# 0x002A/MuCHSALSA

Hardware: AMD Instinct MI355X
Metric: overlap-pairs/s (higher is better)
Workload: dtype int32+f64; 1 GPU; 100k synthetic Nanopore x10 kb, 500k unitig anchors, 10x coverage (BASELINE.json configs[2]); rows=5059558, reads=100000, anchors=499992, edges=981460, edgematches_rank0=25532466, orders_rank0=1029308, parallelism=one job on one GPU, edges_proven_clean_rank0=5372

## Files before the change

### muchsalsa_amd/csrc/msgpu_api.hip

```cpp
#include <hip/hip_runtime.h>

#include <chrono>
#include <cmath>
#include <cstdarg>
#include <cstdio>
#include <cstdlib>
#include <cstring>
#include <condition_variable>
#include <deque>
#include <mutex>
#include <new>
#include <thread>
#include <vector>
#include <algorithm>
#include <sys/mman.h>
#include <unistd.h>

#include "asm_internal.h"
#include "host_pool.h"
#include "msgpu.h"
#include "msgpu_internal.h"

using namespace msgpu;

// ... 74 lines not shown
    if (header_of(p)->registered || !have_device()) return p;
    block_unmap(p);
  }
  void *q = nullptr;
  if (hipHostMalloc(&q, PB_HEADER + (bytes ? bytes : 1), hipHostMallocDefault) != hipSuccess || !q) {
    (void)hipGetLastError();
    return nullptr;
  }
  *static_cast<BlockHeader *>(q) = BlockHeader{PB_MAGIC, q, 0, 0, 0, 1};
  return static_cast<char *>(q) + PB_HEADER;
}
void pinned_block_free(void *p) noexcept {
  if (p) block_unmap(p);
}

void *host_table_alloc(size_t bytes) {
  void *p = block_map(bytes ? bytes : 1);
  if (!p) throw std::bad_alloc();
  return p;
}
void host_table_free(void *q) noexcept {
  if (q) block_unmap(q);
}
void host_table_pin(void *q) noexcept {
  if (q) block_register(q);
}
}


namespace {

struct DevBuf {
  void  *p   = nullptr;
  size_t cap = 0;
  size_t off  = 0;
  size_t hint = 0;
  static inline thread_local double grow_by = 1.0;
  double own_grow_by = 0.0;
  hipError_t ensure(size_t bytes) {
    if (off + bytes <= cap) return hipSuccess;
    const size_t need = off + bytes;
    size_t       want = need + need / 8 + 256;
    const double by = own_grow_by > grow_by ? own_grow_by : grow_by;
    if (by > 1.0) want = off + static_cast<size_t>(double(want - off) * by);
    if (hint > want) want = hint;
    static const bool dbg_alloc = std::getenv("MSGPU_ALLOC_DEBUG") != nullptr;
    if (dbg_alloc) fprintf(stderr, "[alloc] %zu -> %zu bytes (need %zu, kept %zu, hint %zu, grow_by %.2f)\n", cap, want, need, off, hint, grow_by);
    void      *np = nullptr;
    hipError_t e;
    if (p && !off) {
      e   = hipFree(p);
      p   = nullptr;
      cap = 0;
      if (e != hipSuccess) return e;
    }
    e = hipMalloc(&np, want);
    if (e != hipSuccess) return e;
    static const bool poison = std::getenv("MSGPU_POISON") != nullptr;
    if (poison) {
      e = hipMemset(np, 0xA5, want);
      if (e == hipSuccess) e = hipDeviceSynchronize();
      if (e != hipSuccess) {
        (void)hipFree(np);
        return e;
      }
    }
    if (p) {
      e = hipDeviceSynchronize();
      if (e == hipSuccess) e = hipMemcpy(np, p, off, hipMemcpyDeviceToDevice);
      if (e == hipSuccess) e = hipDeviceSynchronize();
      if (e != hipSuccess) {
        (void)hipFree(np);
        return e;
      }
      (void)hipFree(p);
    }
    p   = np;
    cap = want;
    return hipSuccess;
  }
  void release() {
    if (p) (void)hipFree(p);
    p   = nullptr;
    cap = 0;
    off = hint = 0;
  }
  template <class T> T *as() const { return reinterpret_cast<T *>(static_cast<char *>(p) + off); }
  void  *at() const { return static_cast<char *>(p) + off; }
  size_t room() const { return cap > off ? cap - off : 0; }
};

enum State { ST_CREATED = 0, ST_LOADED = 1, ST_EDGES = 2, ST_CHAINED = 3,
             ST_RESULT = 4  };

}

struct msgpu_ctx {
  int          device     = 0;
  hipStream_t  stream     = nullptr;
  hipStream_t  own_stream = nullptr;
  msgpu_params p;
  char         err[512]   = {0};
  State        state      = ST_CREATED;
  uint32_t     shard = 0, nshards = 1;
  uint32_t     win_lo = 0, win_hi = 0xffffffffu;
  uint64_t     base_edges = 0, base_ems = 0, base_orders = 0, base_ids = 0;
  uint64_t    *h_scalars = nullptr;
  uint64_t    *h_scalars_dev = nullptr;
  bool         stage_events = true;
  bool         chain_zeroed = false;
  bool         no_prologue = false;
  bool         prologue_ok = false;
  bool         scalars_clean = false;
  bool         bin_clean = false;
  size_t       bin_zero_words = 0;
  uint32_t     prologue_shard = 0, prologue_nshards = 1;
  uint64_t     prologue_own = 0;
  bool         full_scan_ok = false;
  uint64_t     index_total = 0, own_accum = 0;
  bool         nlists_clean = false;
  bool         cand_zeroed = false;
  uint64_t     prologue_bound = 0;
  uint32_t     prologue_lists[4] = {0, 0, 0, 0};
  uint64_t     readback_seq = 0;
  uint64_t     lost_publications = 0;
  bool         readback_mapped = false;
  hipEvent_t   ev_readback = nullptr;
  hipEvent_t   ev_order = nullptr;
  uint32_t     decl_V = 0, decl_A = 0;
  bool                                  has_deadline = false;
  std::chrono::steady_clock::time_point deadline{};

  uint64_t n_rows = 0, n_alive = 0;
  uint32_t V = 0, A = 0;
  const msgpu_row *d_rows = nullptr;

  uint64_t n_edges = 0, n_ems = 0, n_orders = 0, n_ids = 0, n_visit = 0, total_bound = 0;
  uint32_t n_list[4] = {0, 0, 0, 0};

  DevBuf rows_in, rows_pk, cnt_read, read_off, cursor, bkt_key, bkt_dead, by_read, read_cnt, alive_rank,
      anchor_cnt, anchor_off, anchor_first, anchor_off_gen, bkt2_idx, bkt2_line, by_anchor, read_len, read_first, scalars,
      scan_tmp, vis16, spos2, visits, bin_cursor, bin_start;
  DevBuf bound, cand_off, cand_j, cand_t, scr_v2, scr_start, n_cand, n_edge, lists, edges, edge_cand;
  DevBuf big_key, big_t, big_r2s, big_pfx, pair_tab, chain_chunks, big_off, cand_sums, bucket_visits;
  hipStream_t side_stream = nullptr, side_stream2 = nullptr;
  hipEvent_t  ev_side[2]  = {nullptr, nullptr}, ev_side2 = nullptr;
  uint64_t    n_big_edges = 0, n_big_ems = 0;
  bool   fast_path = true;
  bool   chain_band = true;
  bool   sub_wave  = true;
  bool   use_fork  = true;
  bool   use_prologue = true;
  bool   chain_serial = false;
  uint32_t n_cls[4] = {0, 0, 0, 0};
  uint64_t n_edges_fast = 0;
  uint64_t chain_E = 0;
  DevBuf ems, order_scr, ids_scr, edge_norders, edge_nids, orders, ids, big_list, cls_list, big_elems,
      big_paths;
  DevBuf g_deg, g_off, g_adj, g_cand, g_sane, g_out;
  DevBuf sel_idx, sel_cnt, sel_off, sel_ems;

  DevBuf      alt_edges, alt_ems, alt_orders, alt_ids;
  hipStream_t copy_stream = nullptr;
  hipEvent_t  ev_done[2] = {nullptr, nullptr}, ev_copied[2] = {nullptr, nullptr}, ev_wall[2] = {nullptr, nullptr};
  struct HostBuf {
    void  *p   = nullptr;
    size_t cap = 0;
  } h_edges, h_ems, h_orders, h_ids, h_read_len, h_read_first, h_sel_off, h_sel_ems, h_wire[2];
  hipEvent_t ev_part[2][3] = {{nullptr, nullptr, nullptr}, {nullptr, nullptr, nullptr}};
  std::mutex              gate_m;
  std::condition_variable gate_cv;
  uint64_t                chain_launches = 0;
  DevBuf win_cuts;
  DevBuf wire_dev[2];
  bool   wire_copy = true;

  hipEvent_t ev[10] = {nullptr};
  static constexpr int CK_RING = 256;
  hipEvent_t ck_ev[CK_RING][2] = {};
  uint32_t   ck_head = 0, ck_count = 0;
  bool       have_index_t = false, have_cand_t = false, have_chain_t = false, index_fast = false;
  bool   have_stage_t = false;
  uint32_t index_path = 0;
  bool     index_binned = false;
  bool     use_bin = true;
};

namespace {

int fail(msgpu_ctx *c, int code, const char *fmt, ...) {
  va_list ap;
  va_start(ap, fmt);
  vsnprintf(c->err, sizeof(c->err), fmt, ap);
  va_end(ap);
  return code;
}

#define HIPCHK(c, expr)                                                                                                \
  do {                                                                                                                 \
    hipError_t _e = (expr);                                                                                            \
    if (_e != hipSuccess)                                                                                              \
      return fail((c), _e == hipErrorOutOfMemory ? MSGPU_E_NOMEM : MSGPU_E_HIP, "%s failed: %s (%s:%d)", #expr,        \
                  hipGetErrorString(_e), __FILE__, __LINE__);                                                          \
  } while (0)

#define ENSURE(c, buf, bytes) HIPCHK(c, (c)->buf.ensure(bytes))

template <class T> T *scalar(msgpu_ctx *c, int slot) { return reinterpret_cast<T *>(c->scalars.as<uint64_t>() + slot); }
template <class T> const T *host_scalar(const msgpu_ctx *c, int slot) { return reinterpret_cast<const T *>(c->h_scalars + slot); }
static uint32_t cand_chunks(uint32_t V) { return (V + CAND_CHUNK - 1) / CAND_CHUNK; }
static size_t   cand_sums_bytes(uint32_t V) { return static_cast<size_t>(cand_chunks(V) + 1) * (16 + 256); }
static unsigned long long *cand_chunk_sums(msgpu_ctx *c) { return c->cand_sums.as<unsigned long long>(); }
static uint32_t *cand_hist(msgpu_ctx *c, uint32_t V) { return reinterpret_cast<uint32_t *>(c->cand_sums.as<unsigned long long>() + 2 * static_cast<size_t>(cand_chunks(V) + 1)); }
static CandZero cand_zero(msgpu_ctx *c, uint32_t V) {
  static_assert(SC_BIGCUR == SC_BIGSTATS + 2 && SC_CLS == SC_BIGCUR + 2 && SC_HEADS == SC_CLS + 2, "adjacent scalar slots");
  CandZero z;
  z.n_cand         = c->n_cand.as<uint32_t>();
  z.n_edge         = c->n_edge.as<uint32_t>();
  z.scalar_words   = scalar<uint32_t>(c, SC_BIGSTATS);
  z.n_scalar_words = 12;
  return z;
}

bool past_deadline(const msgpu_ctx *c) { return c->has_deadline && std::chrono::steady_clock::now() >= c->deadline; }
int host_sync(msgpu_ctx *c, hipStream_t st, hipEvent_t ev = nullptr) {
  if (!c->has_deadline) {
    if (ev) HIPCHK(c, hipEventSynchronize(ev));
    else HIPCHK(c, hipStreamSynchronize(st));
    return MSGPU_OK;
  }
  for (uint32_t spins = 0;; ++spins) {
    const hipError_t q = ev ? hipEventQuery(ev) : hipStreamQuery(st);
    if (q == hipSuccess) return MSGPU_OK;
    if (q != hipErrorNotReady) return fail(c, MSGPU_E_HIP, "%s failed: %s", ev ? "hipEventQuery" : "hipStreamQuery", hipGetErrorString(q));
    if (past_deadline(c))
      return fail(c, MSGPU_E_TIMEOUT, "the context's stream did not drain before the deadline (msgpu_set_deadline): work is still queued");
    if (spins < 2000) __builtin_ia32_pause();
    else std::this_thread::sleep_for(std::chrono::microseconds(50));
  }
}

HostPublish arm_readback(msgpu_ctx *c) {
  return c->readback_mapped ? HostPublish{c->h_scalars_dev, ++c->readback_seq} : HostPublish{nullptr, 0};
}
int wait_scalars(msgpu_ctx *c) {
  if (c->readback_mapped) {
    const uint64_t     seq  = c->readback_seq;
    volatile uint64_t *flag = c->h_scalars + SC_COUNT;
    for (uint64_t spins = 1;; ++spins) {
      if (__atomic_load_n(flag, __ATOMIC_ACQUIRE) == seq) return MSGPU_OK;
      __builtin_ia32_pause();
      if ((spins & 0xffff) == 0) {
        const hipError_t q = hipStreamQuery(c->stream);
        if (q == hipSuccess) {
          if (__atomic_load_n(flag, __ATOMIC_ACQUIRE) == seq) return MSGPU_OK;
          break;
        }
        if (q != hipErrorNotReady) break;
        if (past_deadline(c))
          return fail(c, MSGPU_E_TIMEOUT, "table sizes did not come back before the deadline (msgpu_set_deadline): the stream is "
                                          "held up by work queued in front of ours");
      }
    }
    ++c->lost_publications;
    HIPCHK(c, hipMemcpyAsync(c->h_scalars, c->scalars.p, SC_COUNT * sizeof(uint64_t), hipMemcpyDeviceToHost, c->stream));
    return host_sync(c, c->stream);
  }
  return host_sync(c, nullptr, c->ev_readback);
}
int close_readback(msgpu_ctx *c) {
  if (!c->readback_mapped) {
    HIPCHK(c, hipMemcpyAsync(c->h_scalars, c->scalars.p, SC_COUNT * sizeof(uint64_t), hipMemcpyDeviceToHost, c->stream));
    HIPCHK(c, hipEventRecord(c->ev_readback, c->stream));
  }
  return wait_scalars(c);
}
int read_scalars(msgpu_ctx *c, hipEvent_t mark = nullptr) {
  const HostPublish p = arm_readback(c);
  if (p.seq) launch_publish_scalars(c->stream, c->scalars.as<uint64_t>(), p);
  if (mark) HIPCHK(c, hipEventRecord(mark, c->stream));
  return close_readback(c);
}

void release_all(msgpu_ctx *c) {
  DevBuf *all[] = {&c->sel_idx, &c->sel_cnt, &c->sel_off, &c->sel_ems, &c->g_deg, &c->g_off, &c->g_adj, &c->g_cand, &c->g_sane, &c->g_out, &c->rows_in, &c->rows_pk, &c->cnt_read, &c->read_off, &c->cursor, &c->bkt_key,
                   &c->bkt_dead, &c->by_read, &c->read_cnt, &c->alive_rank, &c->anchor_cnt, &c->anchor_off,
                   &c->anchor_first, &c->anchor_off_gen,
                   &c->bkt2_idx, &c->bkt2_line, &c->by_anchor, &c->read_len, &c->read_first, &c->scalars, &c->scan_tmp,
                   &c->bound, &c->cand_off, &c->cand_j, &c->cand_t, &c->scr_v2, &c->scr_start, &c->n_cand, &c->n_edge,
                   &c->lists, &c->edges, &c->edge_cand,
                   &c->big_key, &c->big_t, &c->big_r2s, &c->big_pfx, &c->pair_tab, &c->chain_chunks, &c->big_off, &c->cand_sums, &c->bucket_visits, &c->ems, &c->order_scr, &c->ids_scr,
                   &c->edge_norders, &c->edge_nids, &c->orders, &c->ids, &c->big_list, &c->cls_list, &c->big_elems, &c->big_paths, &c->alt_edges, &c->alt_ems, &c->alt_orders, &c->alt_ids, &c->vis16, &c->visits,
                   &c->spos2, &c->bin_cursor, &c->bin_start, &c->wire_dev[0], &c->wire_dev[1], &c->win_cuts};
  for (DevBuf *b : all) b->release();
}

int build_index_once(msgpu_ctx *c, bool force_generic, bool two_pass, bool bin, uint32_t *ix_flags_out) {
  hipStream_t st = c->stream;
  const uint64_t n = c->n_rows;
  {
    const void *before = c->scalars.p;
    ENSURE(c, scalars, SC_COUNT * sizeof(uint64_t));
    if (c->scalars.p != before) c->scalars_clean = false;
  }
  bool scalars_zeroed = false;
  auto zero_scalars = [&]() -> int {
    if (scalars_zeroed) return MSGPU_OK;
    HIPCHK(c, hipMemsetAsync(c->scalars.p, 0, SC_COUNT * sizeof(uint64_t), st));
    scalars_zeroed  = true;
    c->nlists_clean = true;
    return MSGPU_OK;
  };

  if (c->decl_V && c->decl_A) {
    c->V = c->decl_V;
    c->A = c->decl_A;
  } else {
    if (int rc = zero_scalars()) return rc;
    launch_max_ids(st, c->d_rows, n, scalar<uint32_t>(c, SC_MAXIDS));
    if (int rc = read_scalars(c)) return rc;
    c->V = host_scalar<uint32_t>(c, SC_MAXIDS)[0];
    c->A = host_scalar<uint32_t>(c, SC_MAXIDS)[1];
  }
  const uint32_t V = c->V, A = c->A;

  const size_t nz = n ? n : 1;
  const size_t mva = size_t(V > A ? V : A) + 2;
  constexpr uint32_t BUCKET_CAP = 128;
  const uint32_t reads_per_pass = BIN_NB_MAX << BIN_RPB_SHIFT;
  const uint32_t bpasses = (bin && !force_generic && !two_pass && n && V) ? static_cast<uint32_t>((size_t(V) + reads_per_pass - 1) / reads_per_pass) : 0;
  uint32_t       bcap    = (bpasses && bpasses <= BIN_PASSES_MAX) ? bin_capacity(n, V) : 0;
  if (bcap && !index_sort_bin_prepare(bcap)) bcap = 0;
  const uint32_t bshift  = bcap ? BIN_RPB_SHIFT : 0;
  const uint32_t nb      = bshift ? static_cast<uint32_t>((size_t(std::min(V, reads_per_pass)) + (1u << bshift) - 1) >> bshift) : 0;
  const uint32_t     cap = (!bshift && !two_pass && V && size_t(V) * BUCKET_CAP * sizeof(IRow) <= (size_t(4) << 30)) ? BUCKET_CAP : 0;
  ENSURE(c, cnt_read, (size_t(V) + 1) * 4);
  ENSURE(c, read_off, (size_t(V) + 2) * 4);
  ENSURE(c, cursor, mva * 4);
  if (bshift) {
    const void *before = c->bin_cursor.p;
    ENSURE(c, bin_cursor, (size_t(bpasses) * (nb + 1) + 1) * 4);
    if (c->bin_cursor.p != before) {
      c->bin_clean      = false;
      c->bin_zero_words = 0;
    }
    if (size_t(bpasses) * (nb + 1) + 1 > c->bin_zero_words) c->bin_clean = false;
    ENSURE(c, bin_start, (size_t(nb) + 2) * 4);
    ENSURE(c, bucket_visits, ((size_t(V) >> BIN_RPB_SHIFT) + 2) * 4);
  }
  const bool fused_readback = bshift != 0 && c->readback_mapped;
  if (!(fused_readback && c->scalars_clean))
    if (int rc = zero_scalars()) return rc;
  c->scalars_clean = false;
  ENSURE(c, bkt_key, (bshift ? size_t(nb) * bcap * 2 : cap ? size_t(V) * cap : nz) * sizeof(IRow));
  ENSURE(c, bkt_dead, nz);
  ENSURE(c, by_read, nz * sizeof(IRow));
  ENSURE(c, read_cnt, (size_t(V) + 1) * 4);
  ENSURE(c, alive_rank, nz * 4);
  ENSURE(c, anchor_cnt, (size_t(A) + 1) * 4);
  ENSURE(c, anchor_first, (size_t(A) + 2) * 4);
  ENSURE(c, anchor_off_gen, (size_t(A) + 2) * 4);
  ENSURE(c, anchor_off, (size_t(A) + 2) * 4);
  ENSURE(c, bkt2_idx, nz * 4);
  ENSURE(c, bkt2_line, nz * 4);
  ENSURE(c, by_anchor, nz * sizeof(IRow));
  ENSURE(c, vis16, nz * 16);
  ENSURE(c, spos2, (bshift ? 1 : cap ? size_t(V) * cap : nz) * 8);
  ENSURE(c, visits, (size_t(V) + 1) * 4);
  ENSURE(c, read_len, (size_t(V) + 1) * 4);
  ENSURE(c, read_first, (size_t(V) + 1) * 4);
  {
    uint64_t m = n;
    if (V > m) m = V;
    if (A > m) m = A;
    ENSURE(c, scan_tmp, 3 * (size_t(scan_blocks(m)) + 1) * 8);
  }

  c->prologue_ok           = false;
  const bool want_prologue = c->use_prologue && !force_generic && !c->no_prologue && V != 0 && (c->nshards == 1 || bshift) && c->win_lo == 0 && c->win_hi >= V;
  if (want_prologue) {
    ENSURE(c, n_cand, (size_t(V) + 1) * 4);
    ENSURE(c, n_edge, (size_t(V) + 1) * 4);
    ENSURE(c, cand_sums, cand_sums_bytes(V));
  }
  size_t zero_words_known = 0;
  {
    uint32_t *const zero[8]   = {bshift ? c->bin_cursor.as<uint32_t>() : c->cnt_read.as<uint32_t>(), c->cursor.as<uint32_t>(),
                                 c->read_cnt.as<uint32_t>(), c->anchor_cnt.as<uint32_t>(), nullptr, nullptr, nullptr, nullptr};
    const uint32_t  n_zero[8] = {bshift ? bpasses * (nb + 1) + 1 : V + 1, static_cast<uint32_t>(mva), V + 1, A + 1, 0, 0, 0, 0};
    uint32_t *const ones[2]   = {c->anchor_first.as<uint32_t>(), nullptr};
    const uint32_t  n_ones[2] = {A + 2, 0};
    if (!bshift) launch_index_init8(st, zero, n_zero, ones, n_ones);
    else if (!c->bin_clean) {
      c->bin_zero_words     = std::max<size_t>(c->bin_zero_words, n_zero[0]);
      uint32_t *const z4[4] = {zero[0], nullptr, nullptr, nullptr};
      const uint32_t  n4[4] = {n_zero[0], 0, 0, 0};
      uint32_t *const o2[2] = {nullptr, nullptr};
      const uint32_t  no2[2] = {0, 0};
      launch_index_init(st, z4, n4, o2, no2);
    }
    c->bin_clean = false;
    if (bshift) {
      zero_words_known  = c->bin_zero_words;
      c->bin_zero_words = 0;
    }
  }
  uint32_t *d_flags = scalar<uint32_t>(c, SC_IXFLAGS);
  if (force_generic) {
    const uint32_t f = IXF_FORCE;
    HIPCHK(c, hipMemcpyAsync(d_flags, &f, 4, hipMemcpyHostToDevice, st));
  }

  if (bshift) {
    uint32_t *row_base = c->bin_cursor.as<uint32_t>() + size_t(bpasses) * (nb + 1);
    for (uint32_t p = 0; p < bpasses; ++p) {
      const uint32_t rd_lo = p * reads_per_pass;
      const uint32_t nb_p  = static_cast<uint32_t>((size_t(std::min(V - rd_lo, reads_per_pass)) + (1u << bshift) - 1) >> bshift);
      uint32_t      *cur   = c->bin_cursor.as<uint32_t>() + size_t(p) * (nb + 1);
      BinTail        tail;
      tail.bin_start    = c->bin_start.as<uint32_t>();
      tail.row_base     = row_base;
      tail.read_off_end = p + 1 == bpasses ? c->read_off.as<uint32_t>() + V : nullptr;
      tail.done_heads   = scalar<unsigned long long>(c, SC_HEADS);
      launch_index_bin(st, c->d_rows, n, V, A, d_flags, scalar<uint32_t>(c, SC_ERR), c->anchor_first.as<uint32_t>(), cur,
                       c->bkt_key.as<uint4>(), rd_lo, nb_p, bcap, tail);
      launch_index_sort_bin(st, cur, c->bin_start.as<uint32_t>(), V, rd_lo, nb_p, bcap, c->bkt_key.as<uint4>(),
                            c->by_read.as<IRow>(), c->by_anchor.as<IRow>(), c->vis16.as<uint4>(), c->read_off.as<uint32_t>(),
                            c->read_cnt.as<uint32_t>(), c->read_len.as<int32_t>(), c->read_first.as<uint32_t>(),
                            c->visits.as<uint32_t>(), c->d_rows, d_flags, scalar<uint32_t>(c, SC_ERR), c->bucket_visits.as<uint32_t>());
    }
  } else {
  launch_index_pass1(st, c->d_rows, n, c->cnt_read.as<uint32_t>(), c->anchor_first.as<uint32_t>(), V, A, d_flags,
                     scalar<uint32_t>(c, SC_ERR), c->bkt_key.as<IRow>(), cap, c->spos2.as<uint2>());
  exclusive_scan<uint32_t>(st, c->cnt_read.as<uint32_t>(), V, c->read_off.as<uint32_t>(), c->scan_tmp.as<uint32_t>(),
                           scalar<uint32_t>(c, SC_TOTAL_A));
  if (!cap) launch_scatter_read(st, c->d_rows, n, c->read_off.as<uint32_t>(), c->cursor.as<uint32_t>(), c->bkt_key.as<IRow>());
  launch_sort_read(st, c->read_off.as<uint32_t>(), c->cnt_read.as<uint32_t>(), V, c->bkt_key.as<IRow>(),
                   c->by_read.as<IRow>(), c->read_cnt.as<uint32_t>(),
                   c->alive_rank.as<uint32_t>(), c->anchor_cnt.as<uint32_t>(), c->bkt_dead.as<uint8_t>(), d_flags,
                   c->by_anchor.as<IRow>(), cap, c->d_rows, c->read_len.as<int32_t>(), c->read_first.as<uint32_t>(),
                   scalar<uint32_t>(c, SC_ERR), c->spos2.as<uint2>(), c->vis16.as<uint4>(), c->visits.as<uint32_t>());
  }
  if (bshift) {
    ENSURE(c, cand_off, (size_t(V) + 2) * 8);
    ENSURE(c, lists, (size_t(V) + 1) * (3 * sizeof(CandDesc) + 4));
// ... 69 lines not shown
  c->own_accum    = fused_readback ? 0 : *host_scalar<uint64_t>(c, SC_OWN);
  if (fused_readback && ixf == 0 && err == 0) {
    c->scalars_clean = c->bin_clean = true;
    c->bin_zero_words = zero_words_known;
  }
  if (want_prologue && ixf == 0 && err == 0) {
    c->prologue_ok      = true;
    c->cand_zeroed      = true;
    c->prologue_bound   = *host_scalar<uint64_t>(c, SC_TOTAL_A);
    c->prologue_shard   = bshift ? c->shard : 0;
    c->prologue_nshards = bshift ? c->nshards : 1;
    c->prologue_own     = (bshift && c->nshards > 1) ? *host_scalar<uint64_t>(c, SC_OWN) : c->prologue_bound;
    for (int k = 0; k < 4; ++k) c->prologue_lists[k] = host_scalar<uint32_t>(c, SC_NLISTS)[k];
  }
  uint32_t       n_alive = *host_scalar<uint32_t>(c, SC_NALIVE);
  if (err & 2u)
    return fail(c, MSGPU_E_IDS, "a row has an id outside the declared id space (%u reads, %u anchors)", V, A);
  c->index_binned = bshift != 0;
  if (bshift && ixf != 0) {
    c->prologue_ok = c->cand_zeroed = false;
    *ix_flags_out  = ixf | IXF_BINFAIL;
    return MSGPU_OK;
  }
  if (ixf & IXF_OVERFLOW) {
    *ix_flags_out = ixf;
    return MSGPU_OK;
  }
  if ((ixf & ~IXF_DUPS) != 0 && !(err & 1u)) {
    exclusive_scan<uint32_t>(st, c->anchor_cnt.as<uint32_t>(), A, c->anchor_off_gen.as<uint32_t>(),
                             c->scan_tmp.as<uint32_t>(), scalar<uint32_t>(c, SC_NALIVE));
    launch_select_anchor_off(st, d_flags, c->anchor_first.as<uint32_t>(), c->anchor_off_gen.as<uint32_t>(), A,
                             c->anchor_off.as<uint32_t>(), scalar<uint32_t>(c, SC_NALIVE), static_cast<uint32_t>(n));
    HIPCHK(c, hipMemsetAsync(c->cursor.p, 0, mva * 4, st));
    launch_scatter_anchor(st, c->d_rows, n, c->alive_rank.as<uint32_t>(), c->anchor_off.as<uint32_t>(),
                          c->cursor.as<uint32_t>(), c->bkt2_idx.as<uint32_t>(), c->bkt2_line.as<uint32_t>(), d_flags);
    launch_rank_anchor(st, c->anchor_off.as<uint32_t>(), n, scalar<uint32_t>(c, SC_NALIVE), c->bkt2_idx.as<uint32_t>(),
                       c->bkt2_line.as<uint32_t>(), c->d_rows, c->alive_rank.as<uint32_t>(), c->by_anchor.as<IRow>(),
                       d_flags, c->read_off.as<uint32_t>(), c->by_read.as<IRow>(), c->vis16.as<uint4>());
    HIPCHK(c, hipGetLastError());
    if (int rc = read_scalars(c, c->ev[1])) return rc;
    n_alive = *host_scalar<uint32_t>(c, SC_NALIVE);
  }
  c->n_alive    = n_alive;
  *ix_flags_out = ixf;
  if (err & 1u)
    return fail(c, MSGPU_E_IDS,
                "read ids are not dense Registry ids in first-line order (Registry.cpp:36-45): use msgpu_parse_paf ids");
  return MSGPU_OK;
}

int build_index(msgpu_ctx *c) {
  if (c->stage_events) HIPCHK(c, hipEventRecord(c->ev[0], c->stream));
  uint32_t ixf = 0;
  bool     two_pass = false;
  int      rc  = build_index_once(c, false, two_pass, c->use_bin, &ixf);
  if (rc != MSGPU_OK) return rc;
  const bool binned = c->use_bin && !(ixf & IXF_BINFAIL) && c->index_binned;
  if (ixf & IXF_BINFAIL) {
    ixf = 0;
    rc  = build_index_once(c, false, two_pass, false, &ixf);
    if (rc != MSGPU_OK) return rc;
  }
  if (ixf & IXF_OVERFLOW) {
    two_pass = true;
    rc       = build_index_once(c, false, two_pass, false, &ixf);
    if (rc != MSGPU_OK) return rc;
  }
  if ((ixf & IXF_DUPS) && (ixf & ~IXF_DUPS) == 0) {
    rc = build_index_once(c, true, two_pass, false, &ixf);
    if (rc != MSGPU_OK) return rc;
  }
  c->index_fast   = (ixf & ~IXF_DUPS) == 0;
  c->index_path   = (binned ? MSGPU_INDEX_BIN : two_pass ? MSGPU_INDEX_TWO_PASS : MSGPU_INDEX_ATOMIC) | (c->index_fast ? 0u : MSGPU_INDEX_GENERIC);
  c->have_index_t = c->stage_events;
  c->state        = ST_LOADED;
  return MSGPU_OK;
}

}

extern "C" {

void msgpu_default_params(msgpu_params *p) {
  if (!p) return;
  p->min_matches = 400;
  p->th_length   = 500;
  p->th_matches  = 500;
  p->th_overlap  = 100;
  p->wiggle_room = 300;
  p->ratio_pct   = 15;
  p->alt_frac    = 0.75;
}

const char *msgpu_strerror(int code) {
  switch (code) {
  case MSGPU_OK: return "ok";
  case MSGPU_E_IO: return "can't open blast file";
  case MSGPU_E_FORMAT: return "invalid BLAST file";
  case MSGPU_E_NUMBER: return "invalid integer field in BLAST file";
  case MSGPU_E_NOMEM: return "out of memory";
  case MSGPU_E_ARG: return "invalid argument (unexpected nullptr)";
  case MSGPU_E_HIP: return "HIP runtime error";
  case MSGPU_E_STATE: return "entry points called out of order";
  case MSGPU_E_IDS: return "read ids are not in Registry (first-line) order";
  case MSGPU_E_NODEVICE: return "no HIP device (libmsgpu has no CPU fallback)";
  case MSGPU_E_LAYOUT: return "path cannot be assembled (the reference would terminate or hang on it)";
  case MSGPU_E_TIMEOUT: return "a deadline passed while device work was still queued";
  default: return "unknown error";
  }
}

int msgpu_create(int device, const msgpu_params *params, msgpu_ctx **out) {
  if (!out) return MSGPU_E_ARG;
  *out = nullptr;
  int        ndev = 0;
  hipError_t e    = hipGetDeviceCount(&ndev);
  if (e != hipSuccess || ndev <= 0) return MSGPU_E_NODEVICE;
  if (device < 0 || device >= ndev) return MSGPU_E_ARG;
  msgpu_ctx *c = new (std::nothrow) msgpu_ctx();
  if (!c) return MSGPU_E_NOMEM;
  c->device = device;
  if (params)
    c->p = *params;
  else
    msgpu_default_params(&c->p);
  if (hipSetDevice(device) != hipSuccess || hipStreamCreateWithFlags(&c->own_stream, hipStreamNonBlocking) != hipSuccess) {
    delete c;
    return MSGPU_E_HIP;
  }
  c->stream = c->own_stream;
  if (hipHostMalloc(reinterpret_cast<void **>(&c->h_scalars), (SC_COUNT + 1) * sizeof(uint64_t),
                    hipHostMallocMapped | hipHostMallocCoherent) != hipSuccess) {
    c->h_scalars = nullptr;
    msgpu_destroy(c);
    return MSGPU_E_NOMEM;
  }
  memset(c->h_scalars, 0, (SC_COUNT + 1) * sizeof(uint64_t));
  if (hipHostGetDevicePointer(reinterpret_cast<void **>(&c->h_scalars_dev), c->h_scalars, 0) != hipSuccess) c->h_scalars_dev = nullptr;
  c->readback_mapped = c->h_scalars_dev && !getenv("MSGPU_SYNC_READBACK");
  {
    const char *nf = getenv("MSGPU_NO_FASTPATH");
    c->fast_path   = !(nf && nf[0] == '1');
    const char *nb = getenv("MSGPU_NO_BAND");
    c->chain_band  = c->fast_path && !(nb && nb[0] == '1');
    const char *ns = getenv("MSGPU_NO_SUBWAVE");
    c->sub_wave    = !(ns && ns[0] == '1');
    const char *nw = getenv("MSGPU_NO_WIRE_COPY");
    c->wire_copy   = !(nw && nw[0] == '1');
    const char *nbin = getenv("MSGPU_NO_BIN");
    c->use_bin       = !(nbin && nbin[0] == '1');
    c->use_prologue = !getenv("MSGPU_NO_PROLOGUE");
    c->use_fork     = !getenv("MSGPU_NO_FORK");
    c->chain_serial = getenv("MSGPU_CHAIN_SERIAL") != nullptr;
  }
  for (auto &ev : c->ev)
    if (hipEventCreate(&ev) != hipSuccess) {
      msgpu_destroy(c);
      return MSGPU_E_HIP;
    }
  int prio_least = 0, prio_greatest = 0;
  if (hipDeviceGetStreamPriorityRange(&prio_least, &prio_greatest) != hipSuccess) prio_least = prio_greatest = 0;
  if (hipStreamCreateWithPriority(&c->side_stream, hipStreamNonBlocking, prio_greatest) != hipSuccess ||
      hipStreamCreateWithPriority(&c->side_stream2, hipStreamNonBlocking, prio_greatest) != hipSuccess ||
      hipEventCreateWithFlags(&c->ev_side2, hipEventDisableTiming) != hipSuccess ||
      hipEventCreateWithFlags(&c->ev_part[0][0], hipEventDisableTiming) != hipSuccess ||
      hipEventCreateWithFlags(&c->ev_part[0][1], hipEventDisableTiming) != hipSuccess ||
      hipEventCreateWithFlags(&c->ev_part[0][2], hipEventDisableTiming) != hipSuccess ||
      hipEventCreateWithFlags(&c->ev_part[1][0], hipEventDisableTiming) != hipSuccess ||
      hipEventCreateWithFlags(&c->ev_part[1][1], hipEventDisableTiming) != hipSuccess ||
      hipEventCreateWithFlags(&c->ev_part[1][2], hipEventDisableTiming) != hipSuccess ||
      hipEventCreateWithFlags(&c->ev_side[0], hipEventDisableTiming) != hipSuccess ||
      hipEventCreateWithFlags(&c->ev_side[1], hipEventDisableTiming) != hipSuccess ||
      hipEventCreateWithFlags(&c->ev_readback, hipEventDisableTiming) != hipSuccess ||
      hipEventCreateWithFlags(&c->ev_order, hipEventDisableTiming) != hipSuccess) {
    msgpu_destroy(c);
    return MSGPU_E_HIP;
  }
  if (hipStreamCreateWithFlags(&c->copy_stream, hipStreamNonBlocking) != hipSuccess) {
    msgpu_destroy(c);
    return MSGPU_E_HIP;
  }
  for (int k = 0; k < 2; ++k)
    if (hipEventCreateWithFlags(&c->ev_done[k], hipEventDisableTiming) != hipSuccess ||
        hipEventCreateWithFlags(&c->ev_copied[k], hipEventDisableTiming) != hipSuccess) {
      msgpu_destroy(c);
      return MSGPU_E_HIP;
    }
  *out = c;
  return MSGPU_OK;
}

void msgpu_destroy(msgpu_ctx *c) {
  if (!c) return;
  (void)hipSetDevice(c->device);
  if (c->stream) (void)hipStreamSynchronize(c->stream);
  release_all(c);
  for (auto &ev : c->ev)
    if (ev) (void)hipEventDestroy(ev);
  for (auto &ev : c->ev_side)
    if (ev) (void)hipEventDestroy(ev);
  if (c->ev_readback) (void)hipEventDestroy(c->ev_readback);
  if (c->ev_order) (void)hipEventDestroy(c->ev_order);
  if (c->ev_side2) (void)hipEventDestroy(c->ev_side2);
  for (auto &per_set : c->ev_part)
    for (hipEvent_t e : per_set)
      if (e) (void)hipEventDestroy(e);
  if (c->side_stream2) {
    (void)hipStreamSynchronize(c->side_stream2);
    (void)hipStreamDestroy(c->side_stream2);
  }
  for (auto &pair : c->ck_ev)
    for (auto &ev : pair)
      if (ev) (void)hipEventDestroy(ev);
  if (c->side_stream) {
    (void)hipStreamSynchronize(c->side_stream);
    (void)hipStreamDestroy(c->side_stream);
  }
  if (c->copy_stream) {
    (void)hipStreamSynchronize(c->copy_stream);
    (void)hipStreamDestroy(c->copy_stream);
  }
  for (int k = 0; k < 2; ++k) {
    if (c->ev_done[k]) (void)hipEventDestroy(c->ev_done[k]);
    if (c->ev_copied[k]) (void)hipEventDestroy(c->ev_copied[k]);
  }
  for (msgpu_ctx::HostBuf *h : {&c->h_edges, &c->h_ems, &c->h_orders, &c->h_ids, &c->h_read_len, &c->h_read_first, &c->h_sel_off,
                               &c->h_sel_ems, &c->h_wire[0], &c->h_wire[1]})
    if (h->p) pinned_block_free(h->p);
  if (c->own_stream) (void)hipStreamDestroy(c->own_stream);
  if (c->h_scalars) (void)hipHostFree(c->h_scalars);
  delete c;
}

const char *msgpu_last_error(const msgpu_ctx *c) { return c ? c->err : "null context"; }

int msgpu_set_stream(msgpu_ctx *c, void *hip_stream) {
  if (!c) return MSGPU_E_ARG;
  HIPCHK(c, hipStreamSynchronize(c->stream));
  c->stream = hip_stream ? static_cast<hipStream_t>(hip_stream) : c->own_stream;
  return MSGPU_OK;
}

void *msgpu_get_stream(const msgpu_ctx *c) { return c ? static_cast<void *>(c->stream) : nullptr; }

int msgpu_stream_wait(msgpu_ctx *c, void *hip_stream) {
  if (!c) return MSGPU_E_ARG;
  hipStream_t other = static_cast<hipStream_t>(hip_stream);
  if (other == c->stream) return MSGPU_OK;
  HIPCHK(c, hipSetDevice(c->device));
  HIPCHK(c, hipEventRecord(c->ev_order, other));
  HIPCHK(c, hipStreamWaitEvent(c->stream, c->ev_order, 0));
  return MSGPU_OK;
}
int msgpu_stream_release(msgpu_ctx *c, void *hip_stream) {
  if (!c) return MSGPU_E_ARG;
  hipStream_t other = static_cast<hipStream_t>(hip_stream);
  if (other == c->stream) return MSGPU_OK;
  HIPCHK(c, hipSetDevice(c->device));
  HIPCHK(c, hipEventRecord(c->ev_order, c->stream));
  HIPCHK(c, hipStreamWaitEvent(other, c->ev_order, 0));
  return MSGPU_OK;
}

int msgpu_set_shard(msgpu_ctx *c, uint32_t shard, uint32_t n_shards) {
  if (!c) return MSGPU_E_ARG;
  if (n_shards == 0 || shard >= n_shards) return fail(c, MSGPU_E_ARG, "shard %u of %u is out of range", shard, n_shards);
  c->shard   = shard;
  c->nshards = n_shards;
  if (c->state > ST_LOADED) c->state = ST_LOADED;
  return MSGPU_OK;
}

int msgpu_set_id_space(msgpu_ctx *c, uint32_t n_reads, uint32_t n_anchors) {
  if (!c) return MSGPU_E_ARG;
  if ((n_reads == 0) != (n_anchors == 0)) return fail(c, MSGPU_E_ARG, "declare both id counts, or 0 and 0 to find them");
  c->decl_V = n_reads;
  c->decl_A = n_anchors;
  return MSGPU_OK;
}

int msgpu_load_rows(msgpu_ctx *c, const msgpu_row *rows, size_t n_rows) {
  if (!c) return MSGPU_E_ARG;
  if (n_rows && !rows) return fail(c, MSGPU_E_ARG, "Unexpected nullptr.");
  if (n_rows > (1ull << 30)) return fail(c, MSGPU_E_ARG, "row table too large (%zu rows, at most 2^30)", n_rows);
  HIPCHK(c, hipSetDevice(c->device));
  c->state = ST_CREATED;
  ENSURE(c, rows_in, (n_rows ? n_rows : 1) * sizeof(msgpu_row));
  if (n_rows)
    HIPCHK(c, hipMemcpyAsync(c->rows_in.p, rows, n_rows * sizeof(msgpu_row), hipMemcpyHostToDevice, c->stream));
  c->d_rows = c->rows_in.as<msgpu_row>();
  c->n_rows = n_rows;
  return build_index(c);
}

int msgpu_load_rows_packed(msgpu_ctx *c, const msgpu_packed_rows *p) {
  if (!c) return MSGPU_E_ARG;
  if (!p || (p->n_rows && (!p->rows || !p->run_start || !p->run_delta || !p->n_runs)) || (p->n_reads && !p->read_len))
    return fail(c, MSGPU_E_ARG, "Unexpected nullptr.");
  if (p->n_rows > (1ull << 30)) return fail(c, MSGPU_E_ARG, "row table too large (%llu rows, at most 2^30)", (unsigned long long)p->n_rows);
  HIPCHK(c, hipSetDevice(c->device));
  c->state = ST_CREATED;
  const size_t n = static_cast<size_t>(p->n_rows);
  const size_t off_len = (n * sizeof(msgpu_row28) + 255) / 256 * 256, off_rs = off_len + (size_t(p->n_reads) * 4 + 255) / 256 * 256,
               off_rd = off_rs + (size_t(p->n_runs) * 4 + 255) / 256 * 256, total = off_rd + size_t(p->n_runs) * 4 + 256;
  ENSURE(c, rows_pk, total);
  ENSURE(c, rows_in, (n ? n : 1) * sizeof(msgpu_row));
// ... 3 lines not shown
    if (p->n_reads) HIPCHK(c, hipMemcpyAsync(d + off_len, p->read_len, size_t(p->n_reads) * 4, hipMemcpyHostToDevice, c->stream));
    HIPCHK(c, hipMemcpyAsync(d + off_rs, p->run_start, size_t(p->n_runs) * 4, hipMemcpyHostToDevice, c->stream));
    HIPCHK(c, hipMemcpyAsync(d + off_rd, p->run_delta, size_t(p->n_runs) * 4, hipMemcpyHostToDevice, c->stream));
    launch_expand_rows(c->stream, d, n, reinterpret_cast<const int32_t *>(d + off_len), p->n_reads, reinterpret_cast<const uint32_t *>(d + off_rs),
                       reinterpret_cast<const uint32_t *>(d + off_rd), p->n_runs, c->rows_in.as<msgpu_row>(),
                       reinterpret_cast<uint32_t *>(d + off_rd + size_t(p->n_runs) * 4));
    HIPCHK(c, hipGetLastError());
  }
  c->d_rows = c->rows_in.as<msgpu_row>();
  c->n_rows = n;
  return build_index(c);
}

int msgpu_load_rows_device(msgpu_ctx *c, const void *d_rows, size_t n_rows) {
  if (!c) return MSGPU_E_ARG;
  if (n_rows && !d_rows) return fail(c, MSGPU_E_ARG, "Unexpected nullptr.");
  if (n_rows > (1ull << 30)) return fail(c, MSGPU_E_ARG, "row table too large (%zu rows, at most 2^30)", n_rows);
  HIPCHK(c, hipSetDevice(c->device));
  c->state  = ST_CREATED;
  c->d_rows = static_cast<const msgpu_row *>(d_rows);
  c->n_rows = n_rows;
  return build_index(c);
}

static size_t chunk_words(uint64_t n_edges) { return 2 * static_cast<size_t>(n_edges / COMPACT_CHUNK + 2); }

int msgpu_calculate_edges(msgpu_ctx *c) {
  if (!c) return MSGPU_E_ARG;
  if (c->state < ST_LOADED) return fail(c, MSGPU_E_STATE, "msgpu_calculate_edges before msgpu_load_rows");
  HIPCHK(c, hipSetDevice(c->device));
  hipStream_t    st = c->stream;
  const uint32_t V  = c->V;
  c->state          = ST_LOADED;
  if (c->stage_events) HIPCHK(c, hipEventRecord(c->ev[2], st));

  ENSURE(c, bound, (size_t(V) + 1) * 4);
  ENSURE(c, cand_off, (size_t(V) + 2) * 8);
  ENSURE(c, lists, (size_t(V) + 1) * (3 * sizeof(CandDesc) + 4));
  ENSURE(c, n_cand, (size_t(V) + 1) * 4);
  ENSURE(c, n_edge, (size_t(V) + 1) * 4);
  ENSURE(c, cand_sums, cand_sums_bytes(V));
  CandDesc *l0 = c->lists.as<CandDesc>(), *l1 = l0 + V + 1, *l2 = l1 + V + 1;
  uint32_t *l3 = reinterpret_cast<uint32_t *>(l2 + V + 1);

  const bool all_reads = c->index_fast && c->nshards == 1 && c->win_lo == 0 && c->win_hi >= V;
  const bool use_prologue = c->index_fast && c->win_lo == 0 && c->win_hi >= V && c->prologue_ok && c->prologue_shard == c->shard &&
                            c->prologue_nshards == c->nshards;
  const bool zeroed    = use_prologue && c->cand_zeroed;
  c->cand_zeroed       = false;
  const uint32_t *bound     = all_reads ? c->visits.as<uint32_t>() : c->bound.as<uint32_t>();
  uint64_t total_bound, own_bound;
  if (use_prologue) {
    total_bound = c->prologue_bound;
    own_bound   = c->prologue_own;
    for (int k = 0; k < 4; ++k) c->n_list[k] = c->prologue_lists[k];
    if (!zeroed) {
      const CandZero  z         = cand_zero(c, V);
      uint32_t *const zero[4]   = {z.n_cand, z.n_edge, z.scalar_words, nullptr};
      const uint32_t  n_zero[4] = {V + 1, V + 1, z.n_scalar_words, 0};
      uint32_t *const ones[2]   = {nullptr, nullptr};
      const uint32_t  n_ones[2] = {0, 0};
      launch_index_init(st, zero, n_zero, ones, n_ones);
    }
  } else if (c->full_scan_ok && c->index_fast && c->nshards == 1) {
    if (!c->nlists_clean) HIPCHK(c, hipMemsetAsync(scalar<uint32_t>(c, SC_NLISTS), 0, 16, st));
    c->nlists_clean = false;
    launch_classify_reads(st, c->read_off.as<uint32_t>(), c->read_cnt.as<uint32_t>(), c->visits.as<uint32_t>(),
                          c->cand_off.as<uint64_t>(), V, 0, 1, c->win_lo, c->win_hi, l0, l1, l2, l3,
                          scalar<uint32_t>(c, SC_NLISTS), cand_zero(c, V), scalar<unsigned long long>(c, SC_OWN));
    HIPCHK(c, hipGetLastError());
    if (int rc = read_scalars(c)) return rc;
    total_bound  = c->index_total;
    const uint64_t own_now = *host_scalar<uint64_t>(c, SC_OWN);
    own_bound    = own_now - c->own_accum;
    c->own_accum = own_now;
    for (int k = 0; k < 4; ++k) c->n_list[k] = host_scalar<uint32_t>(c, SC_NLISTS)[k];
  } else {
    if (!c->nlists_clean) HIPCHK(c, hipMemsetAsync(scalar<uint32_t>(c, SC_NLISTS), 0, 16, st));
    c->full_scan_ok = false;
    if (!all_reads)
      launch_bound(st, c->read_off.as<uint32_t>(), c->read_cnt.as<uint32_t>(), c->vis16.as<uint4>(), V, c->shard,
                   c->nshards, c->win_lo, c->win_hi, c->bound.as<uint32_t>());
    exclusive_scan<uint64_t>(st, bound, V, c->cand_off.as<uint64_t>(), c->scan_tmp.as<uint64_t>(),
                             scalar<uint64_t>(c, SC_TOTAL_A));
    c->nlists_clean = false;
    launch_classify_reads(st, c->read_off.as<uint32_t>(), c->read_cnt.as<uint32_t>(), bound,
                          c->cand_off.as<uint64_t>(), V, c->shard, c->nshards, c->win_lo, c->win_hi, l0, l1, l2, l3,
                          scalar<uint32_t>(c, SC_NLISTS), cand_zero(c, V));
    HIPCHK(c, hipGetLastError());
    if (int rc = read_scalars(c)) return rc;
    total_bound = own_bound = *host_scalar<uint64_t>(c, SC_TOTAL_A);
    for (int k = 0; k < 4; ++k) c->n_list[k] = host_scalar<uint32_t>(c, SC_NLISTS)[k];
  }
  c->total_bound = own_bound;

  const size_t tb = total_bound ? total_bound : 1;
  ENSURE(c, cand_j, tb * 4);
  ENSURE(c, cand_t, tb * 4);
  ENSURE(c, scr_v2, tb * 4);
  ENSURE(c, scr_start, tb * 4);

  CandArgs a;
  a.read_off       = c->read_off.as<uint32_t>();
  a.read_cnt       = c->read_cnt.as<uint32_t>();
  a.anchor_off     = c->anchor_off.as<uint32_t>();
  a.by_read        = c->by_read.as<IRow>();
  a.by_anchor      = c->by_anchor.as<IRow>();
  a.vis            = c->vis16.as<uint4>();
  a.cand_off       = c->cand_off.as<uint64_t>();
  a.cand_j         = c->cand_j.as<uint32_t>();
  a.cand_t         = c->cand_t.as<uint32_t>();
  a.edge_scr_v2    = c->scr_v2.as<uint32_t>();
  a.edge_scr_start = c->scr_start.as<uint32_t>();
  a.n_cand         = c->n_cand.as<uint32_t>();
  a.n_edge         = c->n_edge.as<uint32_t>();
  a.th_overlap     = c->p.th_overlap;
  a.big_stats      = scalar<unsigned long long>(c, SC_BIGSTATS);
  const bool fork = (c->n_list[1] || c->n_list[2]) && c->n_list[0] && c->use_fork;
  if (fork) {
    HIPCHK(c, hipEventRecord(c->ev_side[0], st));
    if (c->n_list[2]) {
      HIPCHK(c, hipStreamWaitEvent(c->side_stream, c->ev_side[0], 0));
      launch_candidates(c->side_stream, a, 2, l2, c->n_list[2]);
    }
    launch_candidates(st, a, 0, l0, c->n_list[0]);
    if (c->n_list[1]) {
      HIPCHK(c, hipStreamWaitEvent(c->side_stream2, c->ev_side[0], 0));
      launch_candidates(c->side_stream2, a, 1, l1, c->n_list[1]);
      HIPCHK(c, hipEventRecord(c->ev_side2, c->side_stream2));
      HIPCHK(c, hipStreamWaitEvent(st, c->ev_side2, 0));
    }
    if (c->n_list[2]) {
      HIPCHK(c, hipEventRecord(c->ev_side[1], c->side_stream));
      HIPCHK(c, hipStreamWaitEvent(st, c->ev_side[1], 0));
    }
  } else {
    launch_candidates(st, a, 2, l2, c->n_list[2]);
    launch_candidates(st, a, 1, l1, c->n_list[1]);
    launch_candidates(st, a, 0, l0, c->n_list[0]);
  }
  if (c->n_list[3]) {
    ENSURE(c, big_key, tb * 8);
    ENSURE(c, big_t, tb * 4);
    ENSURE(c, big_r2s, tb * 4);
    ENSURE(c, big_pfx, (c->n_rows ? c->n_rows : 1) * 4);
    launch_candidates_big(st, a, l3, c->n_list[3], c->big_key.as<uint64_t>(), c->big_t.as<uint32_t>(),
                          c->big_r2s.as<uint32_t>(), c->big_pfx.as<uint32_t>());
  }
  HIPCHK(c, hipGetLastError());
  auto capacities = [&](uint64_t *cap_edges, uint64_t *cap_big) {
    uint64_t ce = c->edges.room() / sizeof(msgpu_edge);
    if (c->edge_cand.cap / 8 < ce) ce = c->edge_cand.cap / 8;
    if (c->cls_list.cap / 4 < ce) ce = c->cls_list.cap / 4;
    uint64_t cb = c->big_list.cap / 4;
    if (c->big_off.cap / 8 < cb) cb = c->big_off.cap / 8;
    if (c->chain_chunks.cap / 8 < chunk_words(ce)) ce = 0;
    *cap_edges = ce;
    *cap_big   = cb;
  };
  auto emit = [&](uint64_t cap_edges, uint64_t cap_big, bool publish) {
    EmitArgs k;
    k.n_edge         = c->n_edge.as<uint32_t>();
    k.n_cand         = c->n_cand.as<uint32_t>();
    k.cand_off       = c->cand_off.as<uint64_t>();
    k.edge_scr_v2    = c->scr_v2.as<uint32_t>();
    k.edge_scr_start = c->scr_start.as<uint32_t>();
    k.V              = V;
    k.hist           = cand_hist(c, V);
    k.chunk_sums     = cand_chunk_sums(c);
    k.n_chunks       = cand_chunks(V);
    k.edges          = c->edges.as<msgpu_edge>();
    k.edge_cand      = c->edge_cand.as<uint64_t>();
    k.list           = c->cls_list.as<uint32_t>();
    k.big_list       = c->big_list.as<uint32_t>();
    k.big_off        = c->big_off.as<uint64_t>();
    k.big_cursor     = scalar<unsigned long long>(c, SC_BIGCUR);
    k.big_stats      = scalar<unsigned long long>(c, SC_BIGSTATS);
    k.cap_edges      = cap_edges;
    k.cap_big        = cap_big;
    k.chain_chunk_sums    = c->chain_chunks.as<unsigned long long>();
    k.n_chain_chunk_words = cap_edges ? static_cast<uint32_t>(chunk_words(cap_edges)) : 0u;
    k.scalars        = c->scalars.as<uint64_t>();
    k.pub            = publish ? arm_readback(c) : HostPublish{nullptr, 0};
    k.nlists         = scalar<unsigned long long>(c, SC_NLISTS);
    launch_emit_edges(st, k, publish);
  };
  uint64_t cap_edges = 0, cap_big = 0;
  capacities(&cap_edges, &cap_big);
  emit(cap_edges, cap_big, true);
  c->nlists_clean = true;
  HIPCHK(c, hipGetLastError());
  if (int rc = close_readback(c)) return rc;
  const uint64_t *tot = host_scalar<uint64_t>(c, SC_TOTAL_A), *big = host_scalar<uint64_t>(c, SC_BIGSTATS);
  c->n_big_edges = big[0];
  c->n_big_ems   = big[1];
  for (int k = 0; k < 4; ++k) c->n_cls[k] = host_scalar<uint32_t>(c, SC_CLS)[k];
  c->n_ems   = tot[0];
  c->n_edges = tot[1];
  c->n_visit = c->total_bound;
  if (c->n_edges >= 0xfffffff0ull) return fail(c, MSGPU_E_ARG, "edge table too large (%llu)", (unsigned long long)c->n_edges);
  if (c->n_edges > cap_edges || c->n_big_edges >= cap_big) {
    ENSURE(c, edges, (c->n_edges ? c->n_edges : 1) * sizeof(msgpu_edge));
    ENSURE(c, edge_cand, (c->n_edges ? c->n_edges : 1) * 8);
    ENSURE(c, cls_list, (c->n_edges + 1) * 4);
    ENSURE(c, big_list, (c->n_big_edges + 1) * 4);
    ENSURE(c, big_off, (c->n_big_edges + 1) * 8);
    ENSURE(c, chain_chunks, chunk_words(c->edges.room() / sizeof(msgpu_edge)) * 8);
    capacities(&cap_edges, &cap_big);
    emit(cap_edges, cap_big, false);
  }
  c->chain_zeroed = true;
  HIPCHK(c, hipGetLastError());
  if (c->stage_events) HIPCHK(c, hipEventRecord(c->ev[3], st));
  c->have_cand_t = c->stage_events;
  c->n_orders    = 0;
  c->n_ids       = 0;
  c->state       = ST_EDGES;
  return MSGPU_OK;
}

int msgpu_chaining_and_overlaps(msgpu_ctx *c) {
  if (!c) return MSGPU_E_ARG;
  if (c->state < ST_EDGES || c->state == ST_RESULT)
    return fail(c, MSGPU_E_STATE, "msgpu_chaining_and_overlaps before msgpu_calculate_edges");
  HIPCHK(c, hipSetDevice(c->device));
  hipStream_t    st = c->stream;
  const uint64_t E = c->n_edges, M = c->n_ems;
  for (int k = 0; k < 2; ++k)
    if (!c->ck_ev[c->ck_head][k]) HIPCHK(c, hipEventCreate(&c->ck_ev[c->ck_head][k]));
  const hipEvent_t ck_begin = c->ck_ev[c->ck_head][0], ck_end = c->ck_ev[c->ck_head][1];
  if (c->stage_events) HIPCHK(c, hipEventRecord(c->ev[4], st));

  ENSURE(c, ems, (M ? M : 1) * sizeof(msgpu_edgematch));
  ENSURE(c, order_scr, (M ? M : 1) * sizeof(msgpu_order));
  ENSURE(c, ids_scr, (M ? M : 1) * 4);
  ENSURE(c, edge_norders, (E + 4) * 4);
  ENSURE(c, edge_nids, (E + 4) * 4);
  ENSURE(c, chain_chunks, chunk_words(E) * 8);

  ChainArgs a;
  a.edges        = c->edges.as<msgpu_edge>();
  a.edge_cand    = c->edge_cand.as<uint64_t>();
  a.n_edges      = E;
  a.cand_j       = c->cand_j.as<uint32_t>();
  a.cand_t       = c->cand_t.as<uint32_t>();
  a.read_off     = c->read_off.as<uint32_t>();
  a.read_cnt     = c->read_cnt.as<uint32_t>();
  a.read_len     = c->read_len.as<int32_t>();
  a.by_read      = c->by_read.as<IRow>();
  a.by_anchor    = c->by_anchor.as<IRow>();
  a.ems          = c->ems.as<msgpu_edgematch>();
  a.order_scr    = c->order_scr.as<msgpu_order>();
  a.ids_scr      = c->ids_scr.as<uint32_t>();
  a.edge_norders = c->edge_norders.as<uint32_t>();
  a.edge_nids    = c->edge_nids.as<uint32_t>();
  a.err          = scalar<uint32_t>(c, SC_ERR);
  if (!c->pair_tab.p) {
    ENSURE(c, pair_tab, PAIR_TAB_WORDS * sizeof(uint32_t));
    launch_fill_pair_tab(st, c->pair_tab.as<uint32_t>());
  }
  a.pair_tab     = c->pair_tab.as<uint32_t>();
  a.pair_tab64   = c->pair_tab.as<uint32_t>() + 4 * PAIR_TAB_STRIDE;
  a.pair_tab_sub = c->pair_tab.as<uint32_t>() + 4 * PAIR_TAB_STRIDE + 2 * PAIR_TAB_STRIDE;
  if (!c->chain_zeroed)
    HIPCHK(c, hipMemsetAsync(c->chain_chunks.p, 0, chunk_words(E) * 8, st));
  c->chain_zeroed = false;
  a.chunk_sums   = c->chain_chunks.as<unsigned long long>();
  a.fast_path    = (c->fast_path ? CHAIN_FAST_SHORTCUT : 0) | (c->chain_band ? CHAIN_FAST_BAND : 0);
  c->chain_E     = E;
  a.fast_margin  = static_cast<long long>(std::min<uint64_t>(c->p.wiggle_room, uint64_t(1) << 40)) - 3;
  a.wiggle       = static_cast<double>(c->p.wiggle_room);
  a.ratio_pct    = c->p.ratio_pct;
  a.alt_frac     = c->p.alt_frac;
  a.out_edge_base = static_cast<uint32_t>(c->base_edges);

  const uint32_t n_big = static_cast<uint32_t>(c->n_big_edges);
  if (n_big) {
    ENSURE(c, big_elems, (c->n_big_ems ? c->n_big_ems : 1) * big_elem_bytes());
    ENSURE(c, big_paths, (c->n_big_ems ? c->n_big_ems : 1) * 2 * big_path_bytes());
  }
  if (n_big) HIPCHK(c, hipEventRecord(c->ev_side[0], st));
  auto launch_big = [&]() -> int {
    if (!n_big) return MSGPU_OK;
    HIPCHK(c, hipStreamWaitEvent(c->side_stream, c->ev_side[0], 0));
    launch_chain_big(c->side_stream, a, c->big_list.as<uint32_t>(), c->big_off.as<uint64_t>(), n_big,
                     c->big_elems.p, c->big_paths.p);
    HIPCHK(c, hipEventRecord(c->ev_side[1], c->side_stream));
    return MSGPU_OK;
  };
  {
    std::lock_guard<std::mutex> g(c->gate_m);
    ++c->chain_launches;
  }
  c->gate_cv.notify_all();
  if (int rc = launch_big()) return rc;
  HIPCHK(c, hipEventRecord(ck_begin, st));
  if (c->sub_wave && E) {
    const uint32_t *list = c->cls_list.as<uint32_t>();
    const uint32_t *l64 = list, *l32 = l64 + c->n_cls[2], *l16 = l32 + c->n_cls[1], *l8 = l16 + c->n_cls[0];
    const bool serial = c->chain_serial;
    const bool any_sub = c->n_cls[0] || c->n_cls[1] || c->n_cls[3];
    const bool beside  = !serial && any_sub && c->n_cls[2];
    if (beside) HIPCHK(c, hipStreamWaitEvent(c->side_stream2, ck_begin, 0));
    launch_chain(st, a, l64, c->n_cls[2]);
    if (serial) {
      launch_chain_sub(st, a, 32, l32, c->n_cls[1]);
      launch_chain_sub(st, a, 16, l16, c->n_cls[0]);
      launch_chain_sub(st, a, 8, l8, c->n_cls[3]);
    } else if (any_sub) {
      launch_chain_sub_all(beside ? c->side_stream2 : st, a, l32, c->n_cls[1], l16, c->n_cls[0], l8, c->n_cls[3]);
    }
    if (beside) {
      HIPCHK(c, hipEventRecord(c->ev_side2, c->side_stream2));
      HIPCHK(c, hipStreamWaitEvent(st, c->ev_side2, 0));
    }
  } else {
    launch_chain(st, a, nullptr, 0);
  }
  HIPCHK(c, hipEventRecord(ck_end, st));
  c->ck_head = (c->ck_head + 1) % msgpu_ctx::CK_RING;
  if (c->ck_count < msgpu_ctx::CK_RING) ++c->ck_count;
  HIPCHK(c, hipGetLastError());
  if (n_big) HIPCHK(c, hipStreamWaitEvent(st, c->ev_side[1], 0));

  if (c->stage_events) HIPCHK(c, hipEventRecord(c->ev[7], st));
  auto compact = [&](bool publish) {
    CompactArgs k;
    k.edges        = c->edges.as<msgpu_edge>();
    k.n_edges      = E;
    k.edge_norders = c->edge_norders.as<uint32_t>();
    k.edge_nids    = c->edge_nids.as<uint32_t>();
    k.chunk_sums   = c->chain_chunks.as<unsigned long long>();
    k.n_chunks     = static_cast<uint32_t>((E + COMPACT_CHUNK - 1) / COMPACT_CHUNK);
    k.scalars      = c->scalars.as<uint64_t>();
    k.pub          = publish ? arm_readback(c) : HostPublish{nullptr, 0};
    k.order_scr    = c->order_scr.as<msgpu_order>();
    k.ids_scr      = c->ids_scr.as<uint32_t>();
    k.orders       = c->orders.as<msgpu_order>();
    k.ids          = c->ids.as<uint32_t>();
    k.out_em_base    = c->base_ems;
    k.out_order_base = c->base_orders;
    k.out_ids_base   = c->base_ids;
    k.out_edge_base  = static_cast<uint32_t>(c->base_edges);
    k.cap_orders     = c->orders.room() / sizeof(msgpu_order);
    k.cap_ids        = c->ids.room() / 4;
    launch_compact(st, k);
  };
  const uint64_t cap_orders = c->orders.room() / sizeof(msgpu_order), cap_ids = c->ids.room() / 4;
  compact(true);
  HIPCHK(c, hipGetLastError());
  if (int rc = close_readback(c)) return rc;
  c->n_edges_fast     = *host_scalar<uint64_t>(c, SC_TOTAL_C);
  const uint64_t *tot = host_scalar<uint64_t>(c, SC_TOTAL_A);
  c->n_orders = tot[0];
  c->n_ids    = tot[1];
  if (c->n_orders > cap_orders || c->n_ids > cap_ids) {
    ENSURE(c, orders, (c->n_orders ? c->n_orders : 1) * sizeof(msgpu_order));
    ENSURE(c, ids, (c->n_ids ? c->n_ids : 1) * 4);
    compact(false);
  }
  HIPCHK(c, hipGetLastError());
  if (c->stage_events) HIPCHK(c, hipEventRecord(c->ev[8], st));
  c->have_chain_t = true;
  c->have_stage_t = c->stage_events;
  c->state        = ST_CHAINED;
  return MSGPU_OK;
}

int msgpu_set_stage_events(msgpu_ctx *c, int on) {
  if (!c) return MSGPU_E_ARG;
  c->stage_events = on != 0;
  return MSGPU_OK;
}

int msgpu_get_counts(msgpu_ctx *c, msgpu_counts *out) {
  if (!c || !out) return MSGPU_E_ARG;
  memset(out, 0, sizeof(*out));
  out->n_rows_in       = c->n_rows;
  out->n_rows_alive    = c->n_alive;
  out->n_reads         = c->V;
  out->n_anchors       = c->A;
  out->n_edges         = c->state >= ST_EDGES ? c->n_edges : 0;
  out->n_ems           = c->state >= ST_EDGES ? c->n_ems : 0;
  out->n_orders        = c->state >= ST_CHAINED ? c->n_orders : 0;
  out->n_ids           = c->state >= ST_CHAINED ? c->n_ids : 0;
  out->n_pairs_scanned = c->state >= ST_EDGES ? c->n_visit : 0;
  out->n_edges_fastpath = c->state >= ST_CHAINED ? c->n_edges_fast : 0;
  out->n_lost_publications = c->lost_publications;
  out->index_path          = c->index_path;
  return MSGPU_OK;
}

int msgpu_chain_band_width(void) { return MSGPU_CHAIN_BAND; }

int msgpu_get_chain_band_counts(msgpu_ctx *c, uint64_t *n_banded, uint64_t *n_fallback) {
  if (!c || !n_banded || !n_fallback) return MSGPU_E_ARG;
  *n_banded = *n_fallback = 0;
  if (c->state < ST_CHAINED || !c->chain_chunks.p) return MSGPU_OK;
  HIPCHK(c, hipSetDevice(c->device));
  const size_t n_chunks = static_cast<size_t>((c->chain_E + COMPACT_CHUNK - 1) / COMPACT_CHUNK);
  const size_t fb_word  = 2 * static_cast<size_t>(c->chain_E / COMPACT_CHUNK + 1);
  std::vector<unsigned long long> w(fb_word + 1);
  HIPCHK(c, hipStreamSynchronize(c->stream));
  HIPCHK(c, hipMemcpy(w.data(), c->chain_chunks.p, w.size() * 8, hipMemcpyDeviceToHost));
  for (size_t k = 0; k < n_chunks; ++k) *n_banded += (w[2 * k] >> 16) & 0xffffull;
  *n_fallback = w[fb_word];
  return MSGPU_OK;
}

int msgpu_get_timings(msgpu_ctx *c, msgpu_timings *out) {
  if (!c || !out) return MSGPU_E_ARG;
  memset(out, 0, sizeof(*out));
  HIPCHK(c, hipStreamSynchronize(c->stream));
  if (c->have_index_t) HIPCHK(c, hipEventElapsedTime(&out->index_ms, c->ev[0], c->ev[1]));
  if (c->have_cand_t) HIPCHK(c, hipEventElapsedTime(&out->candidates_ms, c->ev[2], c->ev[3]));
  if (c->have_chain_t) {
    if (c->have_stage_t) {
      HIPCHK(c, hipEventElapsedTime(&out->chain_ms, c->ev[4], c->ev[7]));
      HIPCHK(c, hipEventElapsedTime(&out->compact_ms, c->ev[7], c->ev[8]));
    }
    double   sum = 0;
    uint32_t n   = 0;
    for (uint32_t i = 0; i < c->ck_count; ++i) {
      const uint32_t slot = (c->ck_head + msgpu_ctx::CK_RING - 1 - i) % msgpu_ctx::CK_RING;
      float          ms   = 0;
      HIPCHK(c, hipEventElapsedTime(&ms, c->ck_ev[slot][0], c->ck_ev[slot][1]));
      sum += ms;
      ++n;
    }
    out->chain_kernel_ms       = n ? static_cast<float>(sum / n) : 0.f;
    out->chain_kernel_launches = n;
    c->ck_count                = 0;
  }
  return MSGPU_OK;
}

static int copy_tables(msgpu_ctx *c, void *edges, void *ems, void *orders, void *ids, hipMemcpyKind kind) {
  if (!c) return MSGPU_E_ARG;
  if (c->state < ST_EDGES) return fail(c, MSGPU_E_STATE, "no tables yet");
  if ((ems || orders || ids) && c->state < ST_CHAINED)
    return fail(c, MSGPU_E_STATE, "EdgeMatch/order tables exist only after msgpu_chaining_and_overlaps");
  HIPCHK(c, hipSetDevice(c->device));
  hipStream_t st = c->stream;
  if (edges && c->n_edges) HIPCHK(c, hipMemcpyAsync(edges, c->edges.at(), c->n_edges * sizeof(msgpu_edge), kind, st));
  if (ems && c->n_ems) HIPCHK(c, hipMemcpyAsync(ems, c->ems.at(), c->n_ems * sizeof(msgpu_edgematch), kind, st));
  if (orders && c->n_orders) HIPCHK(c, hipMemcpyAsync(orders, c->orders.at(), c->n_orders * sizeof(msgpu_order), kind, st));
  if (ids && c->n_ids) HIPCHK(c, hipMemcpyAsync(ids, c->ids.at(), c->n_ids * 4, kind, st));
  if (kind == hipMemcpyDeviceToHost) HIPCHK(c, hipStreamSynchronize(st));
  return MSGPU_OK;
}

int msgpu_copy_tables(msgpu_ctx *c, msgpu_edge *edges, msgpu_edgematch *ems, msgpu_order *orders, uint32_t *ids) {
  return copy_tables(c, edges, ems, orders, ids, hipMemcpyDeviceToHost);
}
int msgpu_copy_tables_device(msgpu_ctx *c, void *d_edges, void *d_ems, void *d_orders, void *d_ids) {
  return copy_tables(c, d_edges, d_ems, d_orders, d_ids, hipMemcpyDeviceToDevice);
}

int msgpu_copy_reads(msgpu_ctx *c, int32_t *read_len, uint32_t *read_first_line) {
  if (!c) return MSGPU_E_ARG;
  if (c->state < ST_LOADED) return fail(c, MSGPU_E_STATE, "no rows loaded");
  HIPCHK(c, hipSetDevice(c->device));
  if (read_len && c->V)
// ... 679 lines not shown
```

### muchsalsa_amd/csrc/msgpu_internal.h

```cpp
#ifndef MSGPU_INTERNAL_H
#define MSGPU_INTERNAL_H

#include <hip/hip_runtime.h>
#include <stdint.h>

#include "msgpu.h"

namespace msgpu {

struct IRow {
  int32_t  n_lo, n_hi, i_lo, i_hi;
  uint32_t score, line, other, pf;
};
static_assert(sizeof(IRow) == 32, "IRow must be 32 bytes");
constexpr uint32_t PF_POS_MASK = 0x3fffffffu;
constexpr uint32_t PF_DIR      = 1u << 30;
constexpr uint32_t PF_PRIM     = 1u << 31;

enum { SC_MAXIDS = 0 , SC_ERR = 1, SC_TOTAL_A = 2, SC_TOTAL_B = 3, SC_TOTAL_C = 4, SC_NLISTS = 5 ,
       SC_NBIG = 7, SC_NALIVE = 8, SC_IXFLAGS = 9, SC_BIGSTATS = 10 , SC_BIGCUR = 12 ,
       SC_CLS = 14 ,
       SC_HEADS = 16 , SC_DONE = 17 ,
       SC_OWN = 18 , SC_COUNT = 19 };
static_assert(SC_COUNT <= 64, "one wavefront publishes the whole scalar block (publish_to_host)");
struct HostPublish {
  uint64_t *host;
  uint64_t  seq;
};

struct CandDesc {
  uint32_t r, rb, n1, bound;
  uint64_t co, pad;
};
static_assert(sizeof(CandDesc) == 32, "CandDesc must be 32 bytes");

struct CandArgs {
  const uint32_t *read_off, *read_cnt, *anchor_off;
  const IRow     *by_read, *by_anchor;
  const uint4    *vis;
  const uint64_t *cand_off;
  uint32_t       *cand_j;
  uint32_t       *cand_t;
  uint32_t       *edge_scr_v2;
  uint32_t       *edge_scr_start;
  uint32_t       *n_cand, *n_edge;
  unsigned long long *big_stats;
  uint32_t        th_overlap;
};
constexpr uint32_t CAND_CHUNK = 256;
struct CandZero {
  uint32_t *n_cand, *n_edge;
  uint32_t *scalar_words;
  uint32_t  n_scalar_words;
};
struct EmitArgs {
  const uint32_t *n_edge, *n_cand;
  const uint64_t *cand_off;
  const uint32_t *edge_scr_v2, *edge_scr_start;
  uint32_t        V;
  const uint32_t *hist;
  const unsigned long long *chunk_sums;
  uint32_t        n_chunks;
  msgpu_edge     *edges;
  uint64_t       *edge_cand;
  uint32_t       *list;
  uint32_t       *big_list;
  uint64_t       *big_off;
  unsigned long long *big_cursor;
  const unsigned long long *big_stats;
  uint64_t        cap_edges, cap_big;
  unsigned long long *chain_chunk_sums;
  uint32_t        n_chain_chunk_words;
  uint64_t       *scalars;
  HostPublish     pub;
  unsigned long long *nlists;
};

struct ChainArgs {
  msgpu_edge      *edges;
  const uint64_t  *edge_cand;
  uint64_t         n_edges;
  const uint32_t  *cand_j, *cand_t;
  const uint32_t  *read_off, *read_cnt;
  const int32_t   *read_len;
  const IRow      *by_read, *by_anchor;
  msgpu_edgematch *ems;
  msgpu_order     *order_scr;
  uint32_t        *ids_scr;
  uint32_t        *edge_norders, *edge_nids;
  uint32_t        *err;
  const uint32_t  *pair_tab;
  const uint32_t  *pair_tab64;
  const uint32_t  *pair_tab_sub;
  unsigned long long *chunk_sums;
  int              fast_path;
  long long        fast_margin;
  double           wiggle, ratio_pct, alt_frac;
  uint32_t         out_edge_base;
};

constexpr uint32_t COMPACT_CHUNK = 1024;
struct CompactArgs {
  msgpu_edge        *edges;
  uint64_t           n_edges;
  const uint32_t    *edge_norders, *edge_nids;
  const unsigned long long *chunk_sums;
  uint32_t           n_chunks;
  uint64_t          *scalars;
  HostPublish        pub;
  const msgpu_order *order_scr;
  const uint32_t    *ids_scr;
  msgpu_order       *orders;
  uint32_t          *ids;
  uint64_t           out_em_base, out_order_base, out_ids_base;
  uint32_t           out_edge_base;
  uint64_t           cap_orders, cap_ids;
};

constexpr uint32_t MAX_WORLD = 64;
struct MergeBase {
  uint64_t edges, orders, ids;
  uint32_t read_id, anchor_id;
};
struct MergeArgs {
  const uint8_t *gathered;
  uint64_t       slab_bytes, off_edges, off_orders, off_ids;
  uint32_t       world;
  MergeBase      base[MAX_WORLD + 1];
  msgpu_edge    *edges;
  msgpu_order   *orders;
  uint32_t      *ids;
};

struct PackWireArgs {
  const msgpu_edge  *edges;
  const msgpu_order *orders;
  const uint32_t    *ids;
  uint64_t           n_edges, n_orders, n_ids;
  uint8_t           *w_edges, *w_orders;
  uint32_t          *w_ids;
  uint64_t           base_ems = 0, base_orders = 0, base_ids = 0;
  uint32_t           base_edges = 0;
};
inline uint64_t wire_edges_bytes(uint64_t n) { return 17 * n + 8; }
inline uint64_t wire_orders_bytes(uint64_t n) { return 33 * n + 4; }
inline uint64_t wire_ids_bytes(uint64_t n, uint32_t id_bytes) { return id_bytes == 3 ? (3 * n + 3) / 4 * 4 : 4 * n; }
struct WindowCutArgs {
  uint32_t n;
  float    frac[255];
};
void launch_window_cuts(hipStream_t st, const uint64_t *cum, uint32_t V, const WindowCutArgs &a, uint64_t *out);
void launch_pack_wire(hipStream_t st, const PackWireArgs &a);
void unpack_wire_host(const uint8_t *w_edges, const uint8_t *w_orders, const uint32_t *w_ids, uint32_t id_bytes, uint64_t n_edges,
                      uint64_t n_orders, uint64_t n_ids, uint64_t base_edges, uint64_t base_ems, uint64_t base_orders,
                      uint64_t base_ids, msgpu_edge *edges, msgpu_order *orders, uint32_t *ids, unsigned threads, unsigned tables = 7);
void launch_merge_wire(hipStream_t st, const MergeArgs &a, bool ids3);

template <class T> void exclusive_scan(hipStream_t st, const uint32_t *in, uint64_t n, T *out, T *block_sums, T *d_total);
uint32_t scan_blocks(uint64_t n);

void launch_max_ids(hipStream_t st, const msgpu_row *rows, uint64_t n, uint32_t *max_ids);
void launch_expand_rows(hipStream_t st, const void *pk, uint64_t n, const int32_t *read_len, uint32_t n_reads, const uint32_t *run_start,
                        const uint32_t *run_delta, uint32_t n_runs, msgpu_row *out, uint32_t *err);
constexpr uint32_t IXF_UNSORTED = 1u;
constexpr uint32_t IXF_SPARSE   = 2u;
constexpr uint32_t IXF_DUPS     = 4u;
constexpr uint32_t IXF_FORCE    = 8u;
constexpr uint32_t IXF_OVERFLOW = 16u;
constexpr uint32_t IXF_BIGSCAF  = 32u;
constexpr uint32_t IXF_BINFAIL  = 64u;
constexpr uint32_t BIN_NB_MAX    = 8192;
constexpr uint32_t BIN_RPB_SHIFT = 4;
constexpr uint32_t BIN_PASSES_MAX = 8;
struct BinTail {
  uint32_t *bin_start;
  uint32_t *row_base;
  uint32_t *read_off_end;
  unsigned long long *done_heads;
};
struct IndexEpilogueArgs {
  const uint32_t *read_first;
  uint32_t        V, A, n_rows;
  uint32_t       *err, *flags;
  const uint32_t *anchor_first, *anchor_off_gen;
  uint32_t       *anchor_off, *n_alive;
  uint32_t       *heads, *row_base;
  const uint32_t *visits, *bucket_visits;
  uint32_t        n_buckets;
  uint64_t       *cand_off;
  uint64_t       *total;
  int             classify;
  const uint32_t *read_off, *read_cnt;
  uint32_t        shard, nshards;
  CandDesc       *list0, *list1, *list2;
  uint32_t       *list3, *n_lists;
  unsigned long long *own_total;
  CandZero        z;
  uint32_t       *done;
  uint64_t       *scalars;
  HostPublish     pub;
  uint64_t        zero_mask;
};
void launch_index_epilogue(hipStream_t st, const IndexEpilogueArgs &a);
uint32_t bin_capacity(uint64_t n, uint32_t V);
bool index_sort_bin_prepare(uint32_t cap);
void launch_index_bin(hipStream_t st, const msgpu_row *rows, uint64_t n, uint32_t V, uint32_t A, uint32_t *flags, uint32_t *err,
                      uint32_t *anchor_first, uint32_t *cursor, uint4 *bin_rec, uint32_t rd_lo, uint32_t nb, uint32_t cap,
                      const BinTail &tail);
void launch_index_sort_bin(hipStream_t st, uint32_t *cursor, const uint32_t *bin_start, uint32_t V, uint32_t rd_lo, uint32_t nb,
                           uint32_t cap, const uint4 *bin_rec, IRow *by_read, IRow *by_anchor, uint4 *vis, uint32_t *read_off,
                           uint32_t *read_cnt, int32_t *read_len, uint32_t *read_first, uint32_t *visits, const msgpu_row *rows,
                           uint32_t *flags, uint32_t *err, uint32_t *bucket_visits);
void launch_publish_scalars(hipStream_t st, const uint64_t *src, const HostPublish &p);
void launch_index_init(hipStream_t st, uint32_t *const zero[4], const uint32_t n_zero[4], uint32_t *const ones[2],
                       const uint32_t n_ones[2]);
void launch_index_init8(hipStream_t st, uint32_t *const zero[8], const uint32_t n_zero[8], uint32_t *const ones[2],
                        const uint32_t n_ones[2]);
void launch_index_pass1(hipStream_t st, const msgpu_row *rows, uint64_t n, uint32_t *cnt_read, uint32_t *anchor_first,
                        uint32_t V, uint32_t A, uint32_t *flags, uint32_t *err, IRow *bkt_row, uint32_t cap, uint2 *spos);
void launch_scatter_read(hipStream_t st, const msgpu_row *rows, uint64_t n, const uint32_t *read_off, uint32_t *cursor,
                         IRow *bkt_row);
void launch_sort_read(hipStream_t st, const uint32_t *read_off, const uint32_t *cnt_read, uint32_t V, const IRow *bkt_row,
                      IRow *by_read, uint32_t *read_cnt, uint32_t *alive_rank,
                      uint32_t *anchor_cnt, uint8_t *bkt_dead, uint32_t *flags, IRow *by_anchor, uint32_t cap,
                      const msgpu_row *rows, int32_t *read_len, uint32_t *read_first, uint32_t *err,
                      const uint2 *spos, uint4 *vis, uint32_t *visits);
void launch_index_finish(hipStream_t st, const uint32_t *read_first, uint32_t V, uint32_t *err, const uint32_t *flags,
                         const uint32_t *fast_off, const uint32_t *gen_off, uint32_t A, uint32_t *anchor_off, uint32_t *d_n_alive,
                         uint32_t n_rows);
void launch_select_anchor_off(hipStream_t st, const uint32_t *flags, const uint32_t *fast_off, const uint32_t *gen_off,
                              uint32_t A, uint32_t *anchor_off, uint32_t *d_n_alive, uint32_t n_rows);
void launch_scatter_anchor(hipStream_t st, const msgpu_row *rows, uint64_t n, const uint32_t *alive_rank,
                           const uint32_t *anchor_off, uint32_t *cursor, uint32_t *bkt_idx, uint32_t *bkt_line,
                           const uint32_t *flags);
void launch_rank_anchor(hipStream_t st, const uint32_t *anchor_off, uint64_t n_rows, const uint32_t *d_n_alive,
                        const uint32_t *bkt_idx, const uint32_t *bkt_line, const msgpu_row *rows,
                        const uint32_t *alive_rank, IRow *by_anchor, const uint32_t *flags, const uint32_t *read_off,
                        IRow *by_read, uint4 *vis);
void launch_bound(hipStream_t st, const uint32_t *read_off, const uint32_t *read_cnt, const uint4 *vis, uint32_t V,
                  uint32_t shard, uint32_t nshards, uint32_t lo, uint32_t hi, uint32_t *bound);
void launch_classify_reads(hipStream_t st, const uint32_t *read_off, const uint32_t *read_cnt, const uint32_t *bound,
                           const uint64_t *cand_off, uint32_t V, uint32_t shard, uint32_t nshards, uint32_t lo,
                           uint32_t hi, CandDesc *l0, CandDesc *l1, CandDesc *l2, uint32_t *l3, uint32_t *n_lists, const CandZero &z,
                           unsigned long long *own_total = nullptr);
void launch_candidates(hipStream_t st, const CandArgs &a, int cls, const CandDesc *list, uint32_t n_list);
void launch_candidates_big(hipStream_t st, const CandArgs &a, const uint32_t *list, uint32_t n_list, uint64_t *big_key,
                           uint32_t *big_t, uint32_t *big_r2s, uint32_t *big_pfx);
void launch_emit_edges(hipStream_t st, const EmitArgs &a, bool reduce);
constexpr uint32_t PAIR_TAB_STRIDE = 2016 + 128;
#ifndef MSGPU_CHAIN_BAND
#define MSGPU_CHAIN_BAND 12
#endif
static_assert(MSGPU_CHAIN_BAND >= 1 && MSGPU_CHAIN_BAND <= 62, "band width");
constexpr int chain_band_pairs(int n) { return MSGPU_CHAIN_BAND * (MSGPU_CHAIN_BAND + 1) / 2 + (n - 1 - MSGPU_CHAIN_BAND) * MSGPU_CHAIN_BAND; }
static_assert(chain_band_pairs(64) <= 2016, "the band table fits the stride of the others");
constexpr uint32_t PAIR_TAB_BAND64_OFF = 4 * PAIR_TAB_STRIDE + 2 * PAIR_TAB_STRIDE + 3 * 2 * PAIR_TAB_STRIDE;
constexpr uint32_t PAIR_TAB_WORDS      = PAIR_TAB_BAND64_OFF + 2 * PAIR_TAB_STRIDE;
constexpr int CHAIN_FAST_SHORTCUT = 1, CHAIN_FAST_BAND = 2;
void launch_fill_pair_tab(hipStream_t st, uint32_t *tab);
void launch_chain(hipStream_t st, const ChainArgs &a, const uint32_t *list, uint32_t n_list);
void launch_chain_sub(hipStream_t st, const ChainArgs &a, int width, const uint32_t *list, uint32_t n_list);
struct ChainSubLists {
  const uint32_t *list32, *list16, *list8;
  uint32_t        n32, n16, n8, nb32, nb16;
};
void launch_chain_sub_all(hipStream_t st, const ChainArgs &a, const uint32_t *l32, uint32_t n32, const uint32_t *l16, uint32_t n16,
                          const uint32_t *l8, uint32_t n8);
size_t big_elem_bytes();
size_t big_path_bytes();
void launch_chain_big(hipStream_t st, const ChainArgs &a, const uint32_t *big_list, const uint64_t *big_off,
                      uint32_t n_big, void *elems, void *paths);
void launch_merge_gathered(hipStream_t st, const MergeArgs &a);
void launch_degree(hipStream_t st, const msgpu_edge *edges, uint64_t n_edges, uint32_t *deg);
void launch_fill_adj(hipStream_t st, const msgpu_edge *edges, uint64_t n_edges, const uint64_t *adj_off,
                     uint32_t *cursor, uint32_t *adj);
void launch_mark_contained(hipStream_t st, const msgpu_order *orders, uint64_t n_orders, uint32_t *cand,
                           uint32_t *n_cand);
void launch_check_contraction(hipStream_t st, const msgpu_edge *edges, uint64_t n_edges, const msgpu_order *orders,
                              const uint64_t *adj_off, const uint32_t *adj, const uint32_t *cand,
                              const uint32_t *n_cand, uint64_t n_orders, double wiggle, uint8_t *sane);
void launch_pick_contraction(hipStream_t st, const msgpu_edge *edges, uint64_t n_edges, const uint8_t *sane,
                             int64_t *out);
void launch_compact(hipStream_t st, const CompactArgs &a);
void launch_em_counts(hipStream_t st, const msgpu_edge *edges, const uint32_t *sel, uint64_t n, uint32_t *cnt);
void launch_em_gather(hipStream_t st, const msgpu_edge *edges, const msgpu_edgematch *ems, const uint32_t *sel, uint64_t n,
                      const uint64_t *off, msgpu_edgematch *out);

const uint8_t *seq_store_bases(const msgpu_seqctx *c, int kind, uint64_t *n_bases);
void launch_edit_distance_pairs(hipStream_t st, const uint8_t *d_a, const uint8_t *d_b, const msgpu_align_pair *d_pairs, uint32_t n,
                                uint32_t band, uint32_t *d_out);
enum { ES_CNT_LDS = 0, ES_CNT_SLAB, ES_CNT_D0, ES_CNT_CAPPED, ES_CNT_MAXD, ES_CNT_BROKEN, ES_CNT_COUNT = 8 };
void       launch_edit_script_lengths(hipStream_t st, const uint32_t *d_dist, uint32_t n, uint32_t band, uint32_t *d_len);
uint32_t   edit_script_slots();
uint64_t   edit_script_slab_words(uint32_t slots, uint32_t band);
uint32_t   edit_script_lds_max_d();
hipError_t launch_edit_script_pairs(hipStream_t st, const uint8_t *d_a, const uint8_t *d_b, const msgpu_align_pair *d_pairs, uint32_t n,
                                    uint32_t band, const uint32_t *d_dist, const uint64_t *d_off, uint32_t *d_list, uint32_t *d_cnt,
                                    uint32_t *d_slab, uint32_t slots, uint32_t *d_words);

}

#endif
```

### muchsalsa_amd/csrc/msgpu_kernels.hip

```cpp
#include <hip/hip_runtime.h>
#include <stdint.h>
#include <stdlib.h>

#include <type_traits>
#include <utility>

#include "msgpu.h"
#include "msgpu_internal.h"
#include "msgpu_device.h"

namespace msgpu {


constexpr int SCAN_ITEMS = 8;
uint32_t      scan_blocks(uint64_t n);

template <class T> __global__ __launch_bounds__(256) void k_scan_reduce(const uint32_t *in, uint64_t n, T *block_sums) {
  __shared__ T s[4];
  uint64_t     base = static_cast<uint64_t>(blockIdx.x) * 256 * SCAN_ITEMS;
  T            sum  = 0;
  for (int i = 0; i < SCAN_ITEMS; ++i) {
    uint64_t idx = base + static_cast<uint64_t>(i) * 256 + threadIdx.x;
    if (idx < n) sum += in[idx];
  }
// ... 1133 lines not shown
    nc_r             = r < a.V ? a.n_cand[r] : 0u;
  }
  for (uint32_t i = blockIdx.x * 1024 + threadIdx.x; i < a.n_chain_chunk_words; i += gridDim.x * 1024) a.chain_chunk_sums[i] = 0;
  unsigned long long t[4] = {0, 0, 0, 0};
  for (uint32_t c = threadIdx.x; c < a.n_chunks; c += 1024) {
    const unsigned long long nc = a.chunk_sums[2 * c], ne = a.chunk_sums[2 * c + 1];
    if (c < chunk) {
      t[0] += nc;
      t[1] += ne;
    }
    t[2] += nc;
    t[3] += ne;
  }
#pragma unroll
  for (int k = 0; k < 4; ++k) {
    for (int d = 32; d > 0; d >>= 1) t[k] += __shfl_xor(t[k], d);
    if (lane == 0) s_red[wave][k] = t[k];
  }
  {
    uint32_t hb = 0, ht = 0;
    for (uint32_t c0 = wave; c0 < a.n_chunks; c0 += 64) {
      uint32_t v[4];
#pragma unroll
      for (int u = 0; u < 4; ++u) {
        const uint32_t c = c0 + 16 * u;
        v[u]             = c < a.n_chunks ? a.hist[static_cast<size_t>(c) * 64 + lane] : 0u;
      }
#pragma unroll
      for (int u = 0; u < 4; ++u) {
        hb += c0 + 16 * u < chunk ? v[u] : 0u;
        ht += v[u];
      }
    }
    s_hb[wave][lane] = hb;
    s_ht[wave][lane] = ht;
  }
  __syncthreads();
  if (wave == 1) {
#pragma unroll
    for (int k = 0; k < 4; ++k) {
      unsigned long long v = lane < 16 ? s_red[lane][k] : 0ull;
      for (int d = 8; d > 0; d >>= 1) v += __shfl_xor(v, d);
      if (lane == 0) s_tot[k] = v;
    }
  }
  uint32_t c8 = 0, c16 = 0, c32 = 0, c64 = 0;
  if (wave == 0) {
    uint32_t before = 0, total = 0;
#pragma unroll
    for (int w = 0; w < 16; ++w) {
      before += s_hb[w][lane];
      total += s_ht[w][lane];
    }
    uint32_t inc = total;
    for (int d = 1; d < 64; d <<= 1) {
      const uint32_t o = __shfl_down(inc, d);
      if (lane + d < 64) inc += o;
    }
    s_pos[lane] = inc - total + before;
    c8 = lane < 8 ? total : 0, c16 = (lane >= 8 && lane < 16) ? total : 0, c32 = (lane >= 16 && lane < 32) ? total : 0, c64 = lane >= 32 ? total : 0;
    for (int d = 32; d > 0; d >>= 1) {
      c8 += __shfl_xor(c8, d);
      c16 += __shfl_xor(c16, d);
      c32 += __shfl_xor(c32, d);
      c64 += __shfl_xor(c64, d);
    }
  }
  __syncthreads();
  const unsigned long long base_m = s_tot[0], base_e = s_tot[1], tot_m = s_tot[2], tot_e = s_tot[3];
  if (chunk == 0 && threadIdx.x < 64) {
    const unsigned long long cls_lo = static_cast<unsigned long long>(c16) | (static_cast<unsigned long long>(c32) << 32);
    const unsigned long long cls_hi = static_cast<unsigned long long>(c64) | (static_cast<unsigned long long>(c8) << 32);
    if (lane == 0) {
      a.scalars[SC_TOTAL_A] = tot_m;
      a.scalars[SC_TOTAL_B] = tot_e;
      a.scalars[SC_CLS]     = cls_lo;
      a.scalars[SC_CLS + 1] = cls_hi;
    }
    publish_to_host(a.pub, lane, lane == SC_TOTAL_A ? tot_m : lane == SC_TOTAL_B ? tot_e : lane == SC_CLS ? cls_lo : lane == SC_CLS + 1 ? cls_hi
                                 : lane < SC_COUNT ? a.scalars[lane] : 0ull);
    if (lane == 0 && a.nlists) a.nlists[0] = a.nlists[1] = 0;
  }
  if (tot_e > a.cap_edges || a.big_stats[0] >= a.cap_big) return;
  uint32_t ie = 0, im = 0;
  if (threadIdx.x < CAND_CHUNK) {
    ie               = wave_incl_scan(ne_r);
    im               = wave_incl_scan(nc_r);
    if (lane == 63) {
      s_w[0][wave] = ie;
      s_w[1][wave] = im;
    }
  }
  __syncthreads();
  if (threadIdx.x < CAND_CHUNK) {
    uint32_t be = ie - ne_r, bm = im - nc_r;
    for (int w = 0; w < wave; ++w) {
      be += s_w[0][w];
      bm += s_w[1][w];
    }
    s_ne[threadIdx.x] = ne_r;
    s_nc[threadIdx.x] = nc_r;
    s_eb[threadIdx.x] = be;
    s_mb[threadIdx.x] = bm;
  }
  __syncthreads();
  constexpr int ROUNDS = CAND_CHUNK / 64;
  const int     sub = threadIdx.x & 15;
  uint32_t      ne_r4[ROUNDS], nc_r4[ROUNDS], st_r[ROUNDS], en_r[ROUNDS], v2_r[ROUNDS];
  uint64_t      co_r[ROUNDS];
#pragma unroll
  for (int round = 0; round < ROUNDS; ++round) {
    const uint32_t lr = round * 64 + (threadIdx.x >> 4), r = chunk * CAND_CHUNK + lr;
    ne_r4[round] = s_ne[lr];
    nc_r4[round] = s_nc[lr];
    co_r[round]  = ne_r4[round] ? a.cand_off[r] : 0ull;
  }
#pragma unroll
  for (int round = 0; round < ROUNDS; ++round) {
    const uint32_t e = sub;
    st_r[round] = en_r[round] = v2_r[round] = 0;
    if (e < ne_r4[round]) {
      st_r[round] = a.edge_scr_start[co_r[round] + e];
      en_r[round] = (e + 1 < ne_r4[round]) ? a.edge_scr_start[co_r[round] + e + 1] : nc_r4[round];
      v2_r[round] = a.edge_scr_v2[co_r[round] + e];
    }
  }
#pragma unroll
  for (int round = 0; round < ROUNDS; ++round) {
    const uint32_t lr = round * 64 + (threadIdx.x >> 4), r = chunk * CAND_CHUNK + lr;
    const uint32_t ne = ne_r4[round];
    if (ne == 0) continue;
    const uint32_t nc = nc_r4[round];
    const uint64_t eb = base_e + s_eb[lr], mb = base_m + s_mb[lr], co = co_r[round];
    for (uint32_t e = sub; e < ne; e += 16) {
      const bool     first = e == static_cast<uint32_t>(sub);
      const uint32_t st = first ? st_r[round] : a.edge_scr_start[co + e];
      const uint32_t en = first ? en_r[round] : ((e + 1 < ne) ? a.edge_scr_start[co + e + 1] : nc);
      msgpu_edge     ed;
      ed.v1        = r;
      ed.v2        = first ? v2_r[round] : a.edge_scr_v2[co + e];
      ed.em_off    = mb + st;
      ed.order_off = 0;
      ed.em_cnt    = en - st;
      ed.order_cnt = 0;
      ed.shadow    = 0;
      ed.pad       = 0;
      a.edges[eb + e]     = ed;
      a.edge_cand[eb + e] = co + st;
      if (ed.em_cnt > 64) {
        const unsigned long long i = atomicAdd(&a.big_cursor[0], 1ull);
        a.big_list[i] = static_cast<uint32_t>(eb + e);
        a.big_off[i]  = atomicAdd(&a.big_cursor[1], static_cast<unsigned long long>(ed.em_cnt));
      } else if (ed.em_cnt) {
        a.list[atomicAdd(&s_pos[ed.em_cnt - 1], 1u)] = static_cast<uint32_t>(eb + e);
      }
    }
  }
}
void launch_emit_edges(hipStream_t st, const EmitArgs &a, bool reduce) {
  if (reduce && a.n_chunks)
    hipLaunchKernelGGL(k_cand_reduce, dim3(a.n_chunks), dim3(1024), 0, st, a.n_edge, a.n_cand, a.cand_off, a.edge_scr_start, a.V,
                       const_cast<unsigned long long *>(a.chunk_sums), const_cast<uint32_t *>(a.hist));
  hipLaunchKernelGGL(k_emit_edges, dim3(a.n_chunks ? a.n_chunks : 1), dim3(1024), 0, st, a);
}


__device__ __forceinline__ void chunk_add(unsigned long long *chunk_sums, uint64_t e, bool clean, uint32_t n_orders, uint32_t n_ids, bool banded = false) {
  static_assert(COMPACT_CHUNK < (1u << 16), "two 16-bit edge counts in the low half of a chunk sum");
  unsigned long long *c = chunk_sums + 2 * (e / COMPACT_CHUNK);
  __hip_atomic_fetch_add(c, (clean ? 1ull : 0ull) | (banded ? 1ull << 16 : 0ull) | (static_cast<unsigned long long>(n_orders) << 32), __ATOMIC_RELAXED, __HIP_MEMORY_SCOPE_AGENT);
  __hip_atomic_fetch_add(c + 1, static_cast<unsigned long long>(n_ids), __ATOMIC_RELAXED, __HIP_MEMORY_SCOPE_AGENT);
}
__device__ __forceinline__ void band_fallback_add(unsigned long long *chunk_sums, uint64_t n_edges) {
  __hip_atomic_fetch_add(chunk_sums + 2 * (n_edges / COMPACT_CHUNK + 1), 1ull, __ATOMIC_RELAXED, __HIP_MEMORY_SCOPE_AGENT);
}

struct PathRec {
  uint64_t mask;
  uint64_t score;
  uint32_t primary;
  uint32_t pad;
};

struct __attribute__((aligned(16))) ChainElem {
  double clo1, chi1;
  double clo2, chi2;
  int    rlo1, rhi1, rlo2, rhi2;
};

struct NanoMasks {
  unsigned long long pos, neg, ovl, abort_;
};
template <bool WF, int SORTED >
__device__ __forceinline__ NanoMasks nano_check(double k_clo, double k_chi, double l_clo, double l_chi, int k_rlo,
                                                int k_rhi, int l_rlo, int l_rhi, double &d) {
  typedef unsigned long long M;
  const bool lt_lo_b = k_clo < l_clo;
  const M    lt_lo = __ballot(lt_lo_b), lt_hi = __ballot(k_chi < l_chi);
  const M    gt_lo = __ballot(k_clo > l_clo), gt_hi = __ballot(k_chi > l_chi);
  NanoMasks  f;
  const double x = k_chi - l_clo;
  const double y = l_chi - k_clo;
  double       t = lt_lo_b ? x : y;
  if (WF) {
    f.ovl = __ballot(t >= 0.0);
    d     = fabs(t) + 1;
  } else {
    f.ovl = __ballot(k_clo <= l_chi) & __ballot(l_clo <= k_chi);
    t     = __builtin_amdgcn_inverse_ballot_w64(f.ovl) ? t : -t;
    d = t + 1;
  }
  if (WF) {
    f.pos = lt_lo & lt_hi;
    f.neg = gt_lo & gt_hi;
  } else {
    f.pos = lt_lo & (lt_hi | ~f.ovl);
    f.neg = (f.ovl & gt_lo & gt_hi) | ~(f.ovl | lt_lo);
  }
  if (SORTED == 1) {
    const M rovl = __ballot(l_rlo <= k_rhi);
    const M u2   = __ballot(k_rlo < l_rlo) & __ballot(k_rhi < l_rhi);
    f.abort_     = rovl & (f.neg | (f.pos & ~u2));
  } else if (SORTED == 2) {
    const M rovl = __ballot(k_rlo <= l_rhi);
    const M um2  = __ballot(k_rlo > l_rlo) & __ballot(k_rhi > l_rhi);
    f.abort_     = rovl & (f.pos | (f.neg & ~um2));
  } else {
    const M rovl = __ballot(k_rlo <= l_rhi) & __ballot(l_rlo <= k_rhi);
    const M u2   = __ballot(k_rlo < l_rlo) & __ballot(k_rhi < l_rhi);
    const M um2  = __ballot(k_rlo > l_rlo) & __ballot(k_rhi > l_rhi);
    f.abort_     = rovl & ((f.neg & ~um2) | (f.pos & ~u2));
  }
  return f;
}

__device__ __forceinline__ int paths_of_direction(unsigned long long act, bool direction, int lane, double pop,
                                                  uint64_t pm, bool em_prim, uint32_t j1, uint32_t q2, uint32_t n1,
                                                  uint32_t n2, double alt_frac, PathRec *paths) {
  if (act == 0) return 0;
  const bool mine = (act >> lane) & 1ull;
  const double best = group_max_f64<64>(mine ? pop : -1.0);
  double maxv;
  int    maxi;
  if (best > 0.0) {
    maxv = best;
    maxi = __builtin_ctzll(__ballot(mine && pop == best));
  } else {
    maxv = 0.0;
    maxi = __builtin_ctzll(act);
  }
  maxi = __builtin_amdgcn_readfirstlane(maxi);
  const unsigned long long prim_lanes = __ballot(mine && em_prim);
  int                      np         = 0;
  const uint64_t           m          = rl_u64(pm, maxi);
  bool                     hp         = (m & prim_lanes) != 0;
  hp |= __popcll(m) > 2;
  if (lane == 0) {
    paths[0].mask    = m;
    paths[0].score   = static_cast<uint64_t>(maxv);
    paths[0].primary = hp;
  }
  np = 1;
  const double       thr  = maxv * alt_frac;
  uint64_t           used = m;
  unsigned long long cand = __ballot(mine && pop > thr);
  while (true) {
    cand &= __ballot((pm & used) == 0);
    if (!cand) break;
    const int      p  = __builtin_ctzll(cand);
    const uint64_t mp = rl_u64(pm, p);
    const double   sp = rl_f64(pop, p);
    if (lane == 0) {
      paths[np].mask    = mp;
      paths[np].score   = static_cast<uint64_t>(sp);
      paths[np].primary = (mp & prim_lanes) != 0;
    }
    ++np;
    used |= mp;
    cand &= ~(1ull << p);
  }
  if (np == 1 && hp) {
    const int first = __builtin_ctzll(m), last = 63 - __builtin_clzll(m);
    const uint32_t qe = direction ? q2 : (n2 - 1 - q2);
    const uint32_t jf = rl_u32(j1, first), jl = rl_u32(j1, last), qf = rl_u32(qe, first), ql = rl_u32(qe, last);
    bool           demote;
    if ((jf != 0 && qf != 0) || (jl != n1 - 1 && ql != n2 - 1)) {
      demote = true;
    } else {
      const bool     on   = (m >> lane) & 1ull;
      const uint64_t below = m & ((1ull << lane) - 1);
      const int      prev  = below ? 63 - __builtin_clzll(below) : lane;
      const uint32_t pj = __shfl(j1, prev), pq = __shfl(qe, prev);
      const bool     firstt = below == 0;
      const uint32_t i_t    = firstt ? 0u : pj + 1u;
      const uint32_t jj_t   = firstt ? 0u : pq + 1u;
      const bool     viol   = on && qe < jj_t;
      const unsigned long long vmask = __ballot(viol);
      const int      fv   = vmask ? __builtin_ctzll(vmask) : 64;
      const bool     i1   = j1 > i_t;
      const bool     i2   = lane < fv ? (qe > jj_t) : (lane == fv ? (n2 > jj_t) : false);
      demote              = __ballot(on && i1 && i2) != 0;
    }
    if (demote && lane == 0) paths[0].primary = 0;
  }
  return np;
}

// ... 371 lines not shown
      } else if (L1 < L2 && R1 > R2) {
        have = true;
        fl   = 0;
        lo   = L2 - L1;
        ro   = R1 - R2;
      }
      if (!have) continue;
      const uint32_t cnt = static_cast<uint32_t>(__popcll(mask));
      if ((mask >> lane) & 1ull) {
        const uint32_t pos = static_cast<uint32_t>(__popcll(mask & ((1ull << lane) - 1)));
        a.ids_scr[ed.em_off + n_ids + pos] = anchor;
      }
      if (lane == 0) {
        msgpu_order o;
        o.edge_idx     = static_cast<uint32_t>(e);
        o.flags        = fl | (dir ? MSGPU_ORD_DIR : 0u) | (pv[pi].primary ? MSGPU_ORD_PRIMARY : 0u);
        o.left_offset  = lo;
        o.right_offset = ro;
        o.score        = pv[pi].score;
        o.ids_off      = n_ids;
        o.ids_cnt      = cnt;
        o.start        = (fl & MSGPU_ORD_START_V1) ? v1 : v2;
        o.end          = (fl & MSGPU_ORD_START_V1) ? v2 : v1;
        o.base         = v1;
        o.pad[0]       = 0;
        o.pad[1]       = 0;
        a.order_scr[ed.em_off + n_orders] = o;
      }
      ++n_orders;
      n_ids += cnt;
    }
  }
  if (lane == 0) {
    a.edge_norders[e] = n_orders;
    a.edge_nids[e]    = n_ids;
    a.edges[e].shadow = shadow ? 1 : 0;
    chunk_add(a.chunk_sums, e, clean, n_orders, n_ids, banded);
  }
}


struct __attribute__((aligned(16))) SubPath {
  uint32_t mask, primary;
  uint64_t score;
};

__device__ __forceinline__ double shfl_f64(double v, int src) {
  const long long b  = __double_as_longlong(v);
  const uint32_t  lo = __shfl(static_cast<uint32_t>(b), src), hi = __shfl(static_cast<uint32_t>(b >> 32), src);
  return __longlong_as_double(static_cast<long long>((static_cast<unsigned long long>(hi) << 32) | lo));
}

template <int W> __device__ __forceinline__ uint32_t group_bits(unsigned long long m, int gbase) {
  return static_cast<uint32_t>(m >> gbase) & (W == 32 ? 0xffffffffu : ((1u << W) - 1u));
}

template <int W> __device__ __forceinline__ int longest_prefix(unsigned long long m) {
#pragma unroll
  for (int d = 32; d >= W; d >>= 1) m |= m >> d;
  return __popc(static_cast<uint32_t>(m) & (W == 32 ? 0xffffffffu : ((1u << W) - 1u)));
}

template <int K> __device__ __forceinline__ uint32_t row_bcast(uint32_t v) {
  static_assert(K >= 0 && K < 16, "row lane");
  return static_cast<uint32_t>(__builtin_amdgcn_mov_dpp(static_cast<int>(v), 0x150 + K, 0xf, 0xf, false));
}

template <int W, int K> __device__ __forceinline__ uint32_t group_bcast(uint32_t v) {
  static_assert(K >= 0 && K < W, "group lane");
  if constexpr (W == 16) {
    return row_bcast<K>(v);
  } else if constexpr (W == 8) {
    const int lo = __builtin_amdgcn_mov_dpp(static_cast<int>(v), 0x150 + K, 0xf, 0x3, false);
    return static_cast<uint32_t>(__builtin_amdgcn_update_dpp(lo, static_cast<int>(v), 0x150 + 8 + K, 0xf, 0xc, false));
  } else if constexpr (K < 16) {
    const int r = static_cast<int>(row_bcast<K>(v));
    return static_cast<uint32_t>(__builtin_amdgcn_update_dpp(r, r, 0x142, 0xa, 0xf, false));
  } else {
    const uint32_t r  = row_bcast<K - 16>(v);
    const uint32_t ro = static_cast<uint32_t>(__builtin_amdgcn_mov_dpp(static_cast<int>(v), 0x150 + K - 16, 0xa, 0xf, false));
    return __builtin_amdgcn_permlane16_swap(r, ro, false, false)[1];
  }
}
template <int W, int K> __device__ __forceinline__ double group_bcast_f64(double v) {
  const unsigned long long b  = __builtin_bit_cast(unsigned long long, v);
  const uint32_t           lo = group_bcast<W, K>(static_cast<uint32_t>(b));
  const uint32_t           hi = group_bcast<W, K>(static_cast<uint32_t>(b >> 32));
  return __builtin_bit_cast(double, (static_cast<unsigned long long>(hi) << 32) | lo);
}

template <typename F, int... K> __device__ __forceinline__ void unroll_while(F &&f, std::integer_sequence<int, K...>) {
  (void)(f(std::integral_constant<int, K>{}) && ...);
}

template <int W>
__device__ __forceinline__ uint32_t paths_of_direction_sub(uint32_t act, bool direction, int sl, int gbase, double pop,
                                                           uint32_t pm, bool em_prim, uint32_t j1, uint32_t q2,
                                                           uint32_t n1, uint32_t n2, double alt_frac, SubPath *paths) {
  const bool live = act != 0;
  const bool mine = (act >> sl) & 1u;
  const double best = group_max_f64<W>(mine ? pop : -1.0);
  double maxv = 0.0;
  int    maxi = live ? __builtin_ctz(act) : 0;
  if (best > 0.0) {
    maxv = best;
    const uint32_t at = group_bits<W>(__ballot(mine && pop == best), gbase);
    maxi = at ? __builtin_ctz(at) : 0;
  }
  const uint32_t prim_lanes = group_bits<W>(__ballot(mine && em_prim), gbase);
  const uint32_t m          = __shfl(pm, gbase + maxi);
  const bool     hp         = ((m & prim_lanes) != 0) | (__popc(m) > 2);
  if (live && sl == 0) paths[0] = SubPath{m, hp ? 1u : 0u, static_cast<uint64_t>(maxv)};
  uint32_t np = live ? 1u : 0u;
  const double thr  = maxv * alt_frac;
  uint32_t     used = m;
  uint32_t     cand = group_bits<W>(__ballot(mine && pop > thr), gbase);
  while (true) {
    cand &= group_bits<W>(__ballot((pm & used) == 0), gbase);
    if (__ballot(cand != 0) == 0) break;
    const bool     has = cand != 0;
    const int      p   = has ? __builtin_ctz(cand) : 0;
    const uint32_t mp  = __shfl(pm, gbase + p);
    const double   sp  = shfl_f64(pop, gbase + p);
    if (has && sl == 0) paths[np] = SubPath{mp, (mp & prim_lanes) != 0 ? 1u : 0u, static_cast<uint64_t>(sp)};
    if (has) {
      ++np;
      used |= mp;
      cand &= ~(1u << p);
    }
  }
  const bool     single = live && np == 1 && hp;
  const uint32_t ms     = m ? m : 1u;
  const int      first = __builtin_ctz(ms), last = 31 - __builtin_clz(ms);
  const uint32_t qe = direction ? q2 : (n2 - 1 - q2);
  const uint32_t jf = __shfl(j1, gbase + first), jl = __shfl(j1, gbase + last);
  const uint32_t qf = __shfl(qe, gbase + first), ql = __shfl(qe, gbase + last);
  const bool     ends   = (jf != 0 && qf != 0) || (jl != n1 - 1 && ql != n2 - 1);
  const bool     on     = (m >> sl) & 1u;
  const uint32_t below  = m & ((1u << sl) - 1u);
  const int      prev   = below ? 31 - __builtin_clz(below) : sl;
  const uint32_t pj = __shfl(j1, gbase + prev), pq = __shfl(qe, gbase + prev);
  const bool     firstt = below == 0;
  const uint32_t i_t = firstt ? 0u : pj + 1u, jj_t = firstt ? 0u : pq + 1u;
  const bool     viol  = on && qe < jj_t;
  const uint32_t vmask = group_bits<W>(__ballot(viol), gbase);
  const int      fv    = vmask ? __builtin_ctz(vmask) : 64;
  const bool     i1    = j1 > i_t;
  const bool     i2    = sl < fv ? (qe > jj_t) : (sl == fv ? (n2 > jj_t) : false);
  const bool     inter = group_bits<W>(__ballot(on && i1 && i2), gbase) != 0;
  if (single && (ends || inter) && sl == 0) paths[0].primary = 0;
  return np;
}

template <int W>
__device__ __forceinline__ void chain_sub_body(const ChainArgs &a, const uint32_t *list, uint32_t n_list, uint32_t block,
                                               unsigned char (*s_wavebuf)[sizeof(ChainElem) * 64], uint32_t (*s_cm)[64],
                                               double (*s_keep)[64][4], uint32_t (*s_anchor)[64]) {
  constexpr int G = 64 / W;
  static_assert(W == 8 || W == 16 || W == 32, "group width");
  static_assert(sizeof(ChainElem) * 64 >= sizeof(SubPath) * 2 * 64, "the path lists overlay the element table");
  const int      wave = threadIdx.x >> 6, lane = threadIdx.x & 63;
  const int      g = lane / W, sl = lane % W, gbase = g * W;
  const uint32_t slot    = (block * 4 + wave) * G + g;
  const bool     valid_g = slot < n_list;
  if (__ballot(valid_g) == 0) return;
  const uint32_t   e  = valid_g ? list[slot] : list[0];
  const msgpu_edge ed = a.edges[e];
  const uint32_t   n  = (valid_g && ed.em_cnt <= static_cast<uint32_t>(W)) ? ed.em_cnt : 0u;
  const uint64_t   cp = a.edge_cand[e];
  const bool       act = sl < static_cast<int>(n);
  const uint32_t   v1 = ed.v1, v2 = ed.v2;
  const uint32_t   n1 = a.read_cnt[v1], n2 = a.read_cnt[v2];
  const int        len1 = a.read_len[v1], len2 = a.read_len[v2];
  ChainElem       *el = reinterpret_cast<ChainElem *>(s_wavebuf[wave]);
  uint32_t        *cm = s_cm[wave];

  uint32_t  j1 = 0, q2 = 0, anchor = 0;
  double    clo1 = 0, clo2 = 0, ovr1 = 0, ovr2 = 0, em_score = 0;
  bool      em_dir = false, em_prim = false;
  ChainElem x{};
  cm[lane] = 0;
  if (act) {
    j1               = a.cand_j[cp + sl];
    const uint32_t t = a.cand_t[cp + sl];
    const IRow m1 = load_irow(&a.by_read[a.read_off[v1] + j1]);
    const IRow m2 = load_irow(&a.by_anchor[t]);
    anchor        = m1.other;
    q2            = m2.pf & PF_POS_MASK;
    const int  ov_lo = max(m1.i_lo, m2.i_lo), ov_hi = min(m1.i_hi, m2.i_hi);
    const bool d1 = (m1.pf & PF_DIR) != 0, d2 = (m2.pf & PF_DIR) != 0;
    em_dir           = d1 == d2;
    em_prim          = (m1.pf & PF_PRIM) && (m2.pf & PF_PRIM);
    const bool   o1  = m1.line > m2.line;
    const IRow  &om = o1 ? m1 : m2, &im = o1 ? m2 : m1;
    const double ol  = static_cast<double>(om.i_hi - om.i_lo + 1);
    const double il  = static_cast<double>(im.i_hi - im.i_lo + 1);
    const double cl  = static_cast<double>(ov_hi - ov_lo + 1);
    const double os  = static_cast<double>(om.score) * cl / ol;
    const double is_ = static_cast<double>(im.score) * cl / il;
    em_score         = os + is_;
    {
      uint4 *q = reinterpret_cast<uint4 *>(&a.ems[ed.em_off + sl]);
      q[0]     = make_uint4(static_cast<uint32_t>(ov_lo), static_cast<uint32_t>(ov_hi),
                            static_cast<uint32_t>(__double_as_longlong(em_score)),
                            static_cast<uint32_t>(__double_as_longlong(em_score) >> 32));
      q[1]     = make_uint4(anchor, om.line, (em_dir ? 1u : 0u) | (em_prim ? 2u : 0u), e + a.out_edge_base);
    }
    {
      const double rr1 = static_cast<double>(m1.i_hi - m1.i_lo + 1) / static_cast<double>(m1.n_hi - m1.n_lo + 1);
      const double rr2 = static_cast<double>(m2.i_hi - m2.i_lo + 1) / static_cast<double>(m2.n_hi - m2.n_lo + 1);
      const bool   l1  = m1.i_lo < m2.i_lo, l2 = m2.i_lo < m1.i_lo;
      const bool   h1  = m1.i_hi > m2.i_hi, h2 = m2.i_hi > m1.i_hi;
      const double qL  = static_cast<double>(l1 ? m2.i_lo - m1.i_lo : m1.i_lo - m2.i_lo) / (l1 ? rr1 : rr2);
      const double qR  = static_cast<double>(h1 ? m1.i_hi - m2.i_hi : m2.i_hi - m1.i_hi) / (h1 ? rr1 : rr2);
      double ncl1 = l1 ? qL : 0.0, ncr1 = h1 ? qR : 0.0, ncl2 = l2 ? qL : 0.0, ncr2 = h2 ? qR : 0.0;
      if (!d1) {
        const double tmp = ncl1;
        ncl1             = ncr1;
        ncr1             = tmp;
      }
      if (!d2) {
        const double tmp = ncl2;
        ncl2             = ncr2;
        ncr2             = tmp;
      }
      x.rlo1 = m1.n_lo;
      x.rhi1 = m1.n_hi;
      x.clo1 = static_cast<double>(m1.n_lo) + ncl1;
      x.chi1 = static_cast<double>(m1.n_hi) - ncr1;
      ovr1   = static_cast<double>(len1 - m1.n_hi) + ncr1;
      x.rlo2 = m2.n_lo;
      x.rhi2 = m2.n_hi;
      x.clo2 = static_cast<double>(m2.n_lo) + ncl2;
      x.chi2 = static_cast<double>(m2.n_hi) - ncr2;
      ovr2   = static_cast<double>(len2 - m2.n_hi) + ncr2;
    }
    clo1     = x.clo1;
    clo2     = x.clo2;
    el[lane] = x;
  }
  {
    double *kp = s_keep[wave][lane];
    kp[0] = clo1, kp[1] = clo2, kp[2] = ovr1, kp[3] = ovr2;
    s_anchor[wave][lane] = anchor;
  }
  const uint32_t m_plus  = group_bits<W>(__ballot(act && em_dir), gbase);
  const uint32_t m_minus = group_bits<W>(__ballot(act && !em_dir), gbase);
  __builtin_amdgcn_fence(__ATOMIC_RELEASE, "wavefront");
  __builtin_amdgcn_wave_barrier();

  bool clean = false;
  {
    const bool      try_clean = (m_plus == 0 || m_minus == 0) && n >= 2 && (a.fast_path & CHAIN_FAST_SHORTCUT);
    const bool      plus      = m_minus == 0;
    const ChainElem Pv        = el[sl > 0 ? lane - 1 : lane];
    bool            good      = true;
    if (act && sl > 0) {
      good = (Pv.clo1 < x.clo1) & (Pv.chi1 < x.chi1) & (Pv.rlo1 < x.rlo1) & (Pv.rhi1 < x.rhi1);
      good &= plus ? ((Pv.clo2 < x.clo2) & (Pv.chi2 < x.chi2) & (Pv.rlo2 < x.rlo2) & (Pv.rhi2 < x.rhi2))
                   : ((Pv.clo2 > x.clo2) & (Pv.chi2 > x.chi2) & (Pv.rlo2 > x.rlo2) & (Pv.rhi2 > x.rhi2));
    }
    const double av = plus ? x.clo1 - x.clo2 : x.clo1 + x.chi2;
    const double bv = plus ? x.chi1 - x.chi2 : x.chi1 + x.clo2;
    good &= (av > -1.0e9) & (av < 1.0e9) & (bv > -1.0e9) & (bv < 1.0e9) & (em_score > 1.0e-6);
    const bool maybe = try_clean && group_bits<W>(__ballot(act && !good), gbase) == 0;
    if (__ballot(maybe)) {
      int a_hi = act ? static_cast<int>(ceil(av)) : -2147483647 - 1;
      int a_lo = act ? static_cast<int>(floor(av)) : 2147483647;
      int b_hi = act ? static_cast<int>(ceil(bv)) : -2147483647 - 1;
      int b_lo = act ? static_cast<int>(floor(bv)) : 2147483647;
#pragma unroll
      for (int d = W / 2; d > 0; d >>= 1) {
        a_hi = max(a_hi, __shfl_xor(a_hi, d));
        a_lo = min(a_lo, __shfl_xor(a_lo, d));
        b_hi = max(b_hi, __shfl_xor(b_hi, d));
        b_lo = min(b_lo, __shfl_xor(b_lo, d));
      }
      clean = maybe && static_cast<long long>(a_hi) - b_lo <= a.fast_margin && static_cast<long long>(b_hi) - a_lo <= a.fast_margin;
    }
  }

  const int P = clean ? 0 : static_cast<int>(n * (n - 1) / 2);
  const int nP   = longest_prefix<W>(__ballot(act && !clean));
  const int Pmax = nP * (nP - 1) / 2;
  const bool               one_dir = __ballot(m_plus != 0 && m_minus != 0) == 0;
  const unsigned long long KD_one  = __ballot(m_minus == 0);
  static_assert(sizeof(ChainElem) == 48, "the pair table holds byte offsets of 48-byte elements");
  const __amdgpu_buffer_rsrc_t tab_rsrc = __builtin_amdgcn_make_buffer_rsrc(
      const_cast<uint32_t *>(a.pair_tab_sub) + (W == 32 ? 0 : W == 16 ? 1 : 2) * PAIR_TAB_STRIDE * 2, 0, PAIR_TAB_STRIDE * 8, 0x00020000);
  const uint32_t tab_lane = static_cast<uint32_t>(sl) * 8u;
  auto           load_pairs = [&](int p0) __attribute__((always_inline)) -> uint2 {
    typedef int v2i __attribute__((ext_vector_type(2)));
    const v2i   v = __builtin_amdgcn_raw_buffer_load_b64(tab_rsrc, tab_lane, p0 * 8, 0);
    return make_uint2(static_cast<uint32_t>(v.x), static_cast<uint32_t>(v.y));
  };
  const int            Pl  = P - sl;
  const unsigned char *elg = reinterpret_cast<const unsigned char *>(el + gbase);
  unsigned char       *cmg = reinterpret_cast<unsigned char *>(cm + gbase);
  double          wiggle  = a.wiggle;
  asm volatile("" : "+v"(wiggle));
  bool wf_lane = true;
  if (act) {
    const int prev_rlo1 = el[sl > 0 ? lane - 1 : lane].rlo1;
    wf_lane = (x.clo1 <= x.chi1) & (x.clo2 <= x.chi2) & (x.rlo1 <= x.rhi1) & (sl == 0 || prev_rlo1 <= x.rlo1);
  }
  const bool wf = __ballot(!wf_lane) == 0;
  auto sweep_step = [&](int p0, const uint2 kl, auto wft, auto dirt) __attribute__((always_inline)) {
    typedef decltype(wft)  WFT;
    typedef decltype(dirt) DIRT;
    constexpr int          DIR = DIRT::value;
    unsigned long long     bits;
    const bool             in_range = p0 < Pl;
    {
      typedef unsigned long long M;
      M valid = __ballot(in_range), KD = KD_one;
      if (DIR == 2) {
        const int  k = static_cast<int>(kl.y & 0xffu), l = static_cast<int>(kl.y >> 18);
        const bool kd = (m_plus >> k) & 1u, ld = (m_plus >> l) & 1u;
        valid &= __ballot(kd == ld);
        KD    = __ballot(kd);
      }
      const ChainElem K = *reinterpret_cast<const ChainElem *>(elg + (kl.x & 0xffffu));
      const ChainElem L = *reinterpret_cast<const ChainElem *>(elg + (kl.x >> 16));
      double          d1, d2;
      const NanoMasks f1 = nano_check<WFT::value, WFT::value>(K.clo1, K.chi1, L.clo1, L.chi1, K.rlo1, K.rhi1, L.rlo1, L.rhi1, d1);
      const NanoMasks f2 = nano_check<WFT::value, false>(K.clo2, K.chi2, L.clo2, L.chi2, K.rlo2, K.rhi2, L.rlo2, L.rhi2, d2);
      M p2, n2m;
      if (DIR == 0) {
        p2  = f2.pos;
        n2m = f2.neg;
      } else if (DIR == 1) {
        p2  = f2.neg;
        n2m = f2.pos;
      } else {
        const M fl = KD & (f2.pos ^ f2.neg);
        p2         = f2.neg ^ fl;
        n2m        = f2.pos ^ fl;
      }
      const M codir = (f1.pos & p2) | (f1.neg & n2m);
      const M mixed = f1.ovl ^ f2.ovl;
      M       cl    = codir & ~(f1.abort_ | f2.abort_);
      cl &= valid;
      const double df = fabs(d1 - d2);
      const M near_ = __ballot(df <= wiggle), sum_ok = __ballot(d1 + d2 <= wiggle);
      M       ok    = cl & ((near_ & ~mixed) | (sum_ok & mixed));
      const M need_div = cl & ~(mixed | near_);
      if (need_div) {
        bool pass = false;
        if (__builtin_amdgcn_inverse_ballot_w64(need_div)) pass = df * 100 / fmax(d1, d2) <= a.ratio_pct;
        ok |= __ballot(pass);
      }
      bits = ok;
    }
    const uint32_t run = (kl.y >> 8) & 0xffu;
    if (run != 0 && in_range) {
      uint32_t *row = reinterpret_cast<uint32_t *>(cmg + (kl.y >> 16));
      __hip_atomic_fetch_or(row, __builtin_amdgcn_ubfe(static_cast<uint32_t>(bits >> lane), 0u, run) << (kl.y & 31u),
                            __ATOMIC_RELAXED, __HIP_MEMORY_SCOPE_WORKGROUP);
    }
  };
  auto sweep = [&](auto wft, auto dirt) __attribute__((always_inline)) {
    uint2 ka = load_pairs(0);
    for (int p0 = 0; p0 < Pmax; p0 += 2 * W) {
      const uint2 kb = load_pairs(p0 + W);
      sweep_step(p0, ka, wft, dirt);
      if (p0 + W >= Pmax) break;
      ka = load_pairs(p0 + 2 * W);
      sweep_step(p0 + W, kb, wft, dirt);
    }
  };
  auto sweep_dir = [&](auto wft) __attribute__((always_inline)) {
    if (!one_dir) sweep(wft, std::integral_constant<int, 2>{});
    else if (KD_one == ~0ull) sweep(wft, std::integral_constant<int, 0>{});
    else if (KD_one == 0) sweep(wft, std::integral_constant<int, 1>{});
    else sweep(wft, std::integral_constant<int, 3>{});
  };
  if (wf) sweep_dir(std::true_type{});
  else sweep_dir(std::false_type{});
  __builtin_amdgcn_fence(__ATOMIC_RELEASE, "wavefront");
  __builtin_amdgcn_wave_barrier();
  const uint32_t mycm = clean ? (act ? (1u << sl) - 1u : 0u) : cm[lane];

  const int nmax = longest_prefix<W>(__ballot(act));
  double    pop  = em_score;
  uint32_t  pm   = 1u << sl;
  {
    uint32_t pred = static_cast<uint32_t>(sl);
    uint32_t rev  = __builtin_bitreverse32(mycm);
    auto     dp_step = [&](double cand, int k) __attribute__((always_inline)) {
      unsigned long long comp, saved;
      asm volatile("v_add_co_u32 %0, %1, %0, %0" : "+v"(rev), "=s"(comp));
      const unsigned long long upd = comp & __ballot(cand > pop);
      asm volatile("s_and_saveexec_b64 %[sv], %[m]\n\t"
                   "v_mov_b64 %[pop], %[cand]\n\t"
                   "v_mov_b32 %[pred], %[k]\n\t"
                   "s_mov_b64 exec, %[sv]"
                   : [pop] "+v"(pop), [pred] "+v"(pred), [sv] "=&s"(saved)
                   : [m] "s"(upd), [cand] "v"(cand), [k] "s"(k)
                   : "scc");
    };
    unroll_while(
        [&](auto kc) __attribute__((always_inline)) {
          constexpr int k = decltype(kc)::value;
          if (k + 1 >= nmax) return false;
          dp_step(group_bcast_f64<W, k>(pop) + em_score, k);
          return true;
        },
        std::make_integer_sequence<int, W - 1>{});
    uint32_t ptr = pred;
    for (int span = 1; span < nmax; span <<= 1) {
      if constexpr (W == 32) {
        const uint32_t o  = __shfl(pm, gbase + static_cast<int>(ptr));
        const uint32_t p2 = __shfl(ptr, gbase + static_cast<int>(ptr));
        pm |= o;
        ptr = p2;
      } else {
        const uint32_t o = __shfl(pm | (ptr << 16), gbase + static_cast<int>(ptr));
        pm |= o & 0xffffu;
        ptr = o >> 16;
      }
    }
  }

  SubPath *pmn = reinterpret_cast<SubPath *>(s_wavebuf[wave]) + gbase, *ppl = pmn + 64;
  uint32_t n_m = 0, n_p = 0;
#pragma clang loop unroll(disable)
  for (int trip = 0; trip < 2; ++trip) {
    const bool     dir  = trip != 0 || m_minus == 0;
    const uint32_t actd = trip == 0 ? (m_minus ? m_minus : m_plus) : (m_minus ? m_plus : 0u);
    const uint32_t np   = paths_of_direction_sub<W>(actd, dir, sl, gbase, pop, pm, em_prim, j1, q2, n1, n2, a.alt_frac, dir ? ppl : pmn);
    if (actd) (dir ? n_p : n_m) = np;
    if (__ballot(m_minus != 0 && m_plus != 0) == 0) break;
  }
  __builtin_amdgcn_fence(__ATOMIC_RELEASE, "wavefront");
  __builtin_amdgcn_wave_barrier();

  bool     k_m = false, k_p = false;
  uint32_t prim_m = 0, prim_p = 0, len_m = 0, len_p = 0;
  if (sl < static_cast<int>(n_m)) {
    prim_m = pmn[sl].primary;
    len_m  = static_cast<uint32_t>(__popc(pmn[sl].mask));
    k_m    = true;
  }
  if (sl < static_cast<int>(n_p)) {
    prim_p = ppl[sl].primary;
    len_p  = static_cast<uint32_t>(__popc(ppl[sl].mask));
    k_p    = true;
  }
  const bool has_primary = group_bits<W>(__ballot((k_m && prim_m) || (k_p && prim_p)), gbase) != 0;
  if (has_primary) {
    k_m = k_m && prim_m;
    k_p = k_p && prim_p;
  }
  const bool has_multi = group_bits<W>(__ballot((k_m && len_m > 1) || (k_p && len_p > 1)), gbase) != 0;
  if (has_multi) {
    k_m = k_m && len_m > 1;
    k_p = k_p && len_p > 1;
  }
  const uint32_t keep_m = group_bits<W>(__ballot(k_m), gbase), keep_p = group_bits<W>(__ballot(k_p), gbase);
  const int      combined = __popc(keep_m) + __popc(keep_p);
  bool           shadow   = true;
  if (combined == 1) shadow = !(keep_m ? pmn[__builtin_ctz(keep_m)].primary : ppl[__builtin_ctz(keep_p)].primary);

  uint32_t n_orders = 0, n_ids = 0;
  {
    uint32_t km = keep_m, kp = keep_p;
    while (__ballot((km | kp) != 0)) {
      const bool     dir  = km == 0;
      const uint32_t keep = dir ? kp : km;
      const bool     has  = keep != 0;
      const int      pi   = has ? __builtin_ctz(keep) : 0;
      km &= km - 1u;
      kp = dir ? (keep & (keep - 1u)) : kp;
      const SubPath  rec  = (dir ? ppl : pmn)[pi];
      const uint32_t mask = (has && rec.mask) ? rec.mask : 1u;
      const int      f = __builtin_ctz(mask), l = 31 - __builtin_clz(mask);
      const double  *kf = s_keep[wave][gbase + f], *kl = s_keep[wave][gbase + l];
      const double   L1 = kf[0], R1 = kl[2];
      const double   L2 = dir ? kf[1] : kf[3], R2 = dir ? kl[3] : kl[1];
      bool     have = false;
      uint32_t fl   = 0;
      double   lo = 0, ro = 0;
      if (L1 <= L2 && R1 <= R2) {
        have = true;
        fl   = MSGPU_ORD_START_V1 | MSGPU_ORD_CONTAINED;
        lo   = L2 - L1;
        ro   = R2 - R1;
      } else if (L1 >= L2 && R1 >= R2) {
        have = true;
        fl   = MSGPU_ORD_CONTAINED;
        lo   = L1 - L2;
        ro   = R1 - R2;
      } else if (L1 > L2 && R1 < R2) {
        have = true;
        fl   = MSGPU_ORD_START_V1;
        lo   = L1 - L2;
        ro   = R2 - R1;
      } else if (L1 < L2 && R1 > R2) {
        have = true;
        fl   = 0;
        lo   = L2 - L1;
        ro   = R1 - R2;
      }
      const bool emit = has && have;
      if (emit) {
        const uint32_t cnt = static_cast<uint32_t>(__popc(mask));
        if ((mask >> sl) & 1u) a.ids_scr[ed.em_off + n_ids + static_cast<uint32_t>(__popc(mask & ((1u << sl) - 1u)))] = s_anchor[wave][lane];
        if (sl == 0) {
          msgpu_order o;
          o.edge_idx     = e;
          o.flags        = fl | (dir ? MSGPU_ORD_DIR : 0u) | (rec.primary ? MSGPU_ORD_PRIMARY : 0u);
          o.left_offset  = lo;
          o.right_offset = ro;
          o.score        = rec.score;
          o.ids_off      = n_ids;
          o.ids_cnt      = cnt;
          o.start        = (fl & MSGPU_ORD_START_V1) ? v1 : v2;
          o.end          = (fl & MSGPU_ORD_START_V1) ? v2 : v1;
          o.base         = v1;
          o.pad[0]       = 0;
          o.pad[1]       = 0;
          a.order_scr[ed.em_off + n_orders] = o;
        }
        ++n_orders;
        n_ids += cnt;
      }
    }
  }
  if (n && sl == 0) {
    a.edge_norders[e] = n_orders;
    a.edge_nids[e]    = n_ids;
    a.edges[e].shadow = shadow ? 1 : 0;
    chunk_add(a.chunk_sums, e, clean, n_orders, n_ids);
  }
}

template <int W>
__global__ __launch_bounds__(256) __attribute__((amdgpu_waves_per_eu(W == 32 ? 7 : 6, W == 32 ? 7 : 6))) void k_chain_sub(ChainArgs a, const uint32_t *list, uint32_t n_list) {
  __shared__ __attribute__((aligned(16))) unsigned char s_wavebuf[4][sizeof(ChainElem) * 64];
  __shared__ uint32_t                                  s_cm[4][64];
  __shared__ __attribute__((aligned(16))) double       s_keep[4][64][4];
  __shared__ uint32_t                                  s_anchor[4][64];
  chain_sub_body<W>(a, list, n_list, blockIdx.x, s_wavebuf, s_cm, s_keep, s_anchor);
}
#ifndef MSGPU_SUB_WAVES
#define MSGPU_SUB_WAVES 7
#endif
__global__ __launch_bounds__(256) __attribute__((amdgpu_waves_per_eu(MSGPU_SUB_WAVES, MSGPU_SUB_WAVES))) void k_chain_sub_all(ChainArgs a, ChainSubLists l) {
  __shared__ __attribute__((aligned(16))) unsigned char s_wavebuf[4][sizeof(ChainElem) * 64];
  __shared__ uint32_t                                  s_cm[4][64];
  __shared__ __attribute__((aligned(16))) double       s_keep[4][64][4];
  __shared__ uint32_t                                  s_anchor[4][64];
  uint32_t b = blockIdx.x;
  if (b < l.nb32) {
    chain_sub_body<32>(a, l.list32, l.n32, b, s_wavebuf, s_cm, s_keep, s_anchor);
  } else if ((b -= l.nb32) < l.nb16) {
    chain_sub_body<16>(a, l.list16, l.n16, b, s_wavebuf, s_cm, s_keep, s_anchor);
  } else {
    chain_sub_body<8>(a, l.list8, l.n8, b - l.nb16, s_wavebuf, s_cm, s_keep, s_anchor);
  }
}
template __global__ void k_chain_sub<8>(ChainArgs, const uint32_t *, uint32_t);
template __global__ void k_chain_sub<16>(ChainArgs, const uint32_t *, uint32_t);
template __global__ void k_chain_sub<32>(ChainArgs, const uint32_t *, uint32_t);


struct BigElem {
  int      rlo1, rhi1, rlo2, rhi2;
  double   clo1, chi1, clo2, chi2, ovr1, ovr2, score;
  uint32_t anchor, j1, q2, flags;
  double   pop;
  uint32_t pred, used;
};

struct BigPath {
  uint32_t end, first, len, primary;
  uint64_t score;
};

struct BigHot {
  int    rlo1, rhi1, rlo2, rhi2;
  double clo1, chi1, clo2, chi2;
};
template <class EK, class EL>
__device__ __forceinline__ bool big_compat(const EK &K, const EL &L, bool direction, double wiggle, double ratio_pct) {
  int    o1 = 0, o2 = 0;
  double d1 = 0, d2 = 0;
  bool   abort_ = false;
  {
    if (K.clo1 <= L.chi1 && L.clo1 <= K.chi1) {
      if (K.clo1 < L.clo1 && K.chi1 < L.chi1) {
        o1 = 2;
        d1 = K.chi1 - L.clo1 + 1;
      }
      if (K.clo1 > L.clo1 && K.chi1 > L.chi1) {
        o1 = -2;
        d1 = L.chi1 - K.clo1 + 1;
      }
    } else if (K.clo1 < L.clo1) {
      o1 = 1;
      d1 = L.clo1 - K.chi1 + 1;
    } else {
      o1 = -1;
      d1 = K.clo1 - L.chi1 + 1;
    }
    int uco = 0;
    if (K.rlo1 <= L.rhi1 && L.rlo1 <= K.rhi1) {
      if (K.rlo1 < L.rlo1 && K.rhi1 < L.rhi1) uco = 2;
      if (K.rlo1 > L.rlo1 && K.rhi1 > L.rhi1) uco = -2;
      if ((o1 < 0 && uco >= 0) || (o1 > 0 && uco <= 0)) abort_ = true;
    }
  }
  {
    if (K.clo2 <= L.chi2 && L.clo2 <= K.chi2) {
      if (K.clo2 < L.clo2 && K.chi2 < L.chi2) {
        o2 = 2;
        d2 = K.chi2 - L.clo2 + 1;
      }
      if (K.clo2 > L.clo2 && K.chi2 > L.chi2) {
        o2 = -2;
        d2 = L.chi2 - K.clo2 + 1;
      }
    } else if (K.clo2 < L.clo2) {
      o2 = 1;
      d2 = L.clo2 - K.chi2 + 1;
    } else {
      o2 = -1;
      d2 = K.clo2 - L.chi2 + 1;
    }
    int uco = 0;
    if (K.rlo2 <= L.rhi2 && L.rlo2 <= K.rhi2) {
      if (K.rlo2 < L.rlo2 && K.rhi2 < L.rhi2) uco = 2;
      if (K.rlo2 > L.rlo2 && K.rhi2 > L.rhi2) uco = -2;
      if ((o2 < 0 && uco >= 0) || (o2 > 0 && uco <= 0)) abort_ = true;
    }
  }
  if (abort_) return false;
  if (!direction) o2 = -o2;
  if (o1 == o2 && o1 != 0) {
    const double mx = std_max(d1, d2);
    const double df = mx - std_min(d1, d2);
    return (df <= wiggle) || (df * 100 / mx <= ratio_pct);
  }
  if ((o1 < 0 && o2 < 0) || (o1 > 0 && o2 > 0)) return d1 + d2 <= wiggle;
  return false;
}

constexpr uint32_t BIG_REG_CAP = 256;
__global__ __launch_bounds__(64) void k_chain_big(ChainArgs a, const uint32_t *big_list, const uint64_t *big_off,
                                                  uint32_t n_big, BigElem *elems,
                                                  BigPath *paths ) {
  if (blockIdx.x >= n_big) return;
  const int        lane = threadIdx.x;
  const uint64_t   e    = big_list[blockIdx.x];
  const msgpu_edge ed   = a.edges[e];
  const uint32_t   n    = ed.em_cnt;
  const uint64_t   cp   = a.edge_cand[e];
  const uint32_t   v1 = ed.v1, v2 = ed.v2;
  const uint32_t   n1 = a.read_cnt[v1], n2 = a.read_cnt[v2];
  const int        len1 = a.read_len[v1], len2 = a.read_len[v2];
  BigElem         *E  = elems + big_off[blockIdx.x];
  BigPath         *Pm = paths + 2 * big_off[blockIdx.x], *Pp = Pm + n;
  __shared__ double   s_pop[BIG_REG_CAP];
  __shared__ uint32_t s_pred[BIG_REG_CAP], s_used[BIG_REG_CAP], s_flags[BIG_REG_CAP];
  const bool fast = n <= BIG_REG_CAP;
  auto POP   = [&](uint32_t i) -> double & { return fast ? s_pop[i] : E[i].pop; };
  auto PRED  = [&](uint32_t i) -> uint32_t & { return fast ? s_pred[i] : E[i].pred; };
  auto USED  = [&](uint32_t i) -> uint32_t & { return fast ? s_used[i] : E[i].used; };
  auto FLAGS = [&](uint32_t i) -> uint32_t { return fast ? s_flags[i] : E[i].flags; };

  for (uint32_t i = lane; i < n; i += 64) {
    const uint32_t j1 = a.cand_j[cp + i], t = a.cand_t[cp + i];
    const IRow     m1 = load_irow(&a.by_read[a.read_off[v1] + j1]);
    const IRow     m2 = load_irow(&a.by_anchor[t]);
    const int      ov_lo = max(m1.i_lo, m2.i_lo), ov_hi = min(m1.i_hi, m2.i_hi);
    const bool     d1 = (m1.pf & PF_DIR) != 0, d2 = (m2.pf & PF_DIR) != 0;
    const bool     em_dir = d1 == d2, em_prim = (m1.pf & PF_PRIM) && (m2.pf & PF_PRIM);
    const bool     o1 = m1.line > m2.line;
    const IRow    &om = o1 ? m1 : m2, &im = o1 ? m2 : m1;
    const double   ol = static_cast<double>(om.i_hi - om.i_lo + 1);
    const double   il = static_cast<double>(im.i_hi - im.i_lo + 1);
    const double   cl = static_cast<double>(ov_hi - ov_lo + 1);
    const double   os = static_cast<double>(om.score) * cl / ol;
    const double   is_ = static_cast<double>(im.score) * cl / il;
    BigElem        x;
    x.score  = os + is_;
    x.anchor = m1.other;
    x.j1     = j1;
    x.q2     = m2.pf & PF_POS_MASK;
    x.flags  = (em_dir ? 1u : 0u) | (em_prim ? 2u : 0u);
    msgpu_edgematch em;
    em.ov_lo     = ov_lo;
    em.ov_hi     = ov_hi;
    em.score     = x.score;
    em.anchor_id = x.anchor;
    em.line      = om.line;
    em.flags     = x.flags;
    em.edge_idx  = static_cast<uint32_t>(e) + a.out_edge_base;
    a.ems[ed.em_off + i] = em;
    {
      const double rr  = static_cast<double>(m1.i_hi - m1.i_lo + 1) / static_cast<double>(m1.n_hi - m1.n_lo + 1);
      double       ncl = static_cast<double>(ov_lo - m1.i_lo) / rr;
      double       ncr = static_cast<double>(m1.i_hi - ov_hi) / rr;
      if (!d1) {
        double tmp = ncl;
        ncl        = ncr;
        ncr        = tmp;
      }
      x.rlo1 = m1.n_lo;
      x.rhi1 = m1.n_hi;
      x.clo1 = static_cast<double>(m1.n_lo) + ncl;
      x.chi1 = static_cast<double>(m1.n_hi) - ncr;
      x.ovr1 = static_cast<double>(len1 - m1.n_hi) + ncr;
// ... 147 lines not shown
          bool     disjoint = true;
          uint32_t len = 0, first = p;
          bool     prim = false;
          for (uint32_t c = p; c != 0xffffffffu; c = PRED(c)) {
            if (USED(c)) {
              disjoint = false;
              break;
            }
            prim |= (FLAGS(c) & 2u) != 0;
            first = c;
            ++len;
          }
          if (!disjoint) continue;
          for (uint32_t c = p; c != 0xffffffffu; c = PRED(c)) USED(c) = 1;
          P[np].end     = p;
          P[np].first   = first;
          P[np].len     = len;
          P[np].primary = prim ? 1u : 0u;
          P[np].score   = static_cast<uint64_t>(POP(p));
          ++np;
        }
        if (np == 1 && P[0].primary) {
          const uint32_t f = P[0].first, l = P[0].end;
          auto           qe = [&](uint32_t i) { return direction ? E[i].q2 : (n2 - 1 - E[i].q2); };
          bool           demote;
          if ((E[f].j1 != 0 && qe(f) != 0) || (E[l].j1 != n1 - 1 && qe(l) != n2 - 1)) {
            demote = true;
          } else {
            uint32_t *tmp = a.ids_scr + ed.em_off;
            uint32_t  len = P[0].len, w = len;
            for (uint32_t c = l; c != 0xffffffffu; c = PRED(c)) tmp[--w] = c;
            long long i = 0, jj = 0;
            bool      is_shadow = false;
            for (uint32_t t = 0; t < len && !is_shadow; ++t) {
              const uint32_t  c  = tmp[t];
              const long long rs = static_cast<long long>(E[c].j1);
              bool            inter = rs > i;
              i                     = rs + 1;
              long long re          = static_cast<long long>(qe(c));
              if (re < jj) re = static_cast<long long>(n2);
              inter &= re > jj;
              jj        = re + 1;
              is_shadow = inter;
            }
            demote = is_shadow;
          }
          if (demote) P[0].primary = 0;
        }
      }
    }
    np_dir[pass] = np;
    __threadfence_block();
    __syncthreads();
  }

  if (lane == 0) {
    const uint32_t n_m = np_dir[0], n_p = np_dir[1];
    bool           has_primary = false;
    for (uint32_t i = 0; i < n_p; ++i) has_primary |= Pp[i].primary != 0;
    for (uint32_t i = 0; i < n_m; ++i) has_primary |= Pm[i].primary != 0;
    auto keep1 = [&](const BigPath &p) { return !has_primary || p.primary; };
    bool has_multi = false;
    for (uint32_t i = 0; i < n_p; ++i) has_multi |= keep1(Pp[i]) && Pp[i].len > 1;
    for (uint32_t i = 0; i < n_m; ++i) has_multi |= keep1(Pm[i]) && Pm[i].len > 1;
    auto     keep = [&](const BigPath &p) { return keep1(p) && (!has_multi || p.len > 1); };
    uint32_t combined = 0;
    for (uint32_t i = 0; i < n_m; ++i) combined += keep(Pm[i]) ? 1u : 0u;
    for (uint32_t i = 0; i < n_p; ++i) combined += keep(Pp[i]) ? 1u : 0u;
    bool shadow;
    if (combined > 1) {
      shadow = true;
    } else {
      const BigPath *first = nullptr;
      for (uint32_t i = 0; i < n_m && !first; ++i)
        if (keep(Pm[i])) first = &Pm[i];
      for (uint32_t i = 0; i < n_p && !first; ++i)
        if (keep(Pp[i])) first = &Pp[i];
      shadow = first ? !first->primary : false;
    }
    uint32_t n_orders = 0, n_ids = 0;
    for (int pass = 0; pass < 2; ++pass) {
      const BigPath *pv  = pass == 0 ? Pm : Pp;
      const uint32_t npv = pass == 0 ? n_m : n_p;
      const bool     dir = pass == 1;
      for (uint32_t pi = 0; pi < npv; ++pi) {
        if (!keep(pv[pi])) continue;
        const uint32_t f = pv[pi].first, l = pv[pi].end;
        const double   L1 = E[f].clo1, R1 = E[l].ovr1;
        double         L2 = E[f].clo2, R2 = E[l].ovr2;
        if (!dir) {
          L2 = E[f].ovr2;
          R2 = E[l].clo2;
        }
        bool     have = false;
        uint32_t fl   = 0;
        double   lo = 0, ro = 0;
        if (L1 <= L2 && R1 <= R2) {
          have = true;
          fl   = MSGPU_ORD_START_V1 | MSGPU_ORD_CONTAINED;
          lo   = L2 - L1;
          ro   = R2 - R1;
        } else if (L1 >= L2 && R1 >= R2) {
          have = true;
          fl   = MSGPU_ORD_CONTAINED;
          lo   = L1 - L2;
          ro   = R1 - R2;
        } else if (L1 > L2 && R1 < R2) {
          have = true;
          fl   = MSGPU_ORD_START_V1;
          lo   = L1 - L2;
          ro   = R2 - R1;
        } else if (L1 < L2 && R1 > R2) {
          have = true;
          fl   = 0;
          lo   = L2 - L1;
          ro   = R1 - R2;
        }
        if (!have) continue;
        const uint32_t cnt = pv[pi].len;
        uint32_t       w   = cnt;
        for (uint32_t c = l; c != 0xffffffffu; c = PRED(c)) a.ids_scr[ed.em_off + n_ids + --w] = E[c].anchor;
        msgpu_order o;
        o.edge_idx     = static_cast<uint32_t>(e);
        o.flags        = fl | (dir ? MSGPU_ORD_DIR : 0u) | (pv[pi].primary ? MSGPU_ORD_PRIMARY : 0u);
        o.left_offset  = lo;
        o.right_offset = ro;
        o.score        = pv[pi].score;
        o.ids_off      = n_ids;
        o.ids_cnt      = cnt;
        o.start        = (fl & MSGPU_ORD_START_V1) ? v1 : v2;
        o.end          = (fl & MSGPU_ORD_START_V1) ? v2 : v1;
        o.base         = v1;
        o.pad[0]       = 0;
        o.pad[1]       = 0;
        a.order_scr[ed.em_off + n_orders] = o;
        ++n_orders;
        n_ids += cnt;
      }
    }
    a.edge_norders[e] = n_orders;
    a.edge_nids[e]    = n_ids;
    a.edges[e].shadow = shadow ? 1 : 0;
    chunk_add(a.chunk_sums, e, false, n_orders, n_ids);
  }
}

__device__ __forceinline__ void tab64_entry(uint32_t *tab, int p, int k, int l, int run) {
  (void)run;
  tab[4 * PAIR_TAB_STRIDE + 2 * p]     = static_cast<uint32_t>(k * 48);
  tab[4 * PAIR_TAB_STRIDE + 2 * p + 1] = static_cast<uint32_t>(l * 48);
}
__device__ __forceinline__ void tabsub_entry(uint32_t *tab, int t, int p, int k, int l, int run) {
  uint32_t *e = tab + 4 * PAIR_TAB_STRIDE + 2 * PAIR_TAB_STRIDE + (static_cast<size_t>(t - 1) * PAIR_TAB_STRIDE + p) * 2;
  e[0]        = static_cast<uint32_t>(k * 48) | (static_cast<uint32_t>(l * 48) << 16);
  e[1]        = static_cast<uint32_t>(k) | (static_cast<uint32_t>(run) << 8) | (static_cast<uint32_t>(l * 4) << 16);
}
__device__ __forceinline__ void band64_entry(uint32_t *tab, int p) {
  constexpr int B = MSGPU_CHAIN_BAND, TRI = B * (B + 1) / 2;
  int k = 0, l = 1;
  if (p < TRI) {
    l = static_cast<int>((1.0f + __fsqrt_rn(1.0f + 8.0f * static_cast<float>(p))) * 0.5f);
    if (l * (l - 1) / 2 > p) --l;
    if ((l + 1) * l / 2 <= p) ++l;
    k = p - l * (l - 1) / 2;
  } else {
    const int q = p - TRI;
    l = B + 1 + q / B;
    k = l - B + q % B;
    if (l >= 64) {
      k = 0;
      l = 1;
    }
  }
  tab[PAIR_TAB_BAND64_OFF + 2 * p]     = static_cast<uint32_t>(k * 48);
  tab[PAIR_TAB_BAND64_OFF + 2 * p + 1] = static_cast<uint32_t>(l * 48);
}
__global__ __launch_bounds__(256) void k_fill_pair_tab(uint32_t *tab) {
  const int i = blockIdx.x * 256 + threadIdx.x;
  if (i >= 4 * static_cast<int>(PAIR_TAB_STRIDE)) return;
  const int t = i / static_cast<int>(PAIR_TAB_STRIDE), p = i % static_cast<int>(PAIR_TAB_STRIDE), W = 64 >> t;
  if (t == 0) band64_entry(tab, p);
  if (p >= 2016) {
    tab[i] = 1u << 8;
    if (t == 0) tab64_entry(tab, p, 0, 1, 0);
    else tabsub_entry(tab, t, p, 0, 1, 0);
    return;
  }
  int l = static_cast<int>((1.0f + __fsqrt_rn(1.0f + 8.0f * static_cast<float>(p))) * 0.5f);
  if (l * (l - 1) / 2 > p) --l;
  if ((l + 1) * l / 2 <= p) ++l;
  const int k = p - l * (l - 1) / 2, lane = p % W;
  const int run = (k == 0 || lane == 0) ? min(l - k, W - lane) : 0;
  tab[i] = static_cast<uint32_t>(k | (l << 8) | (run << 16)) | (static_cast<uint32_t>(64 - run - k) << 24);
  if (t == 0) tab64_entry(tab, p, k, l, run);
  else tabsub_entry(tab, t, p, k, l, run);
}

__global__ __launch_bounds__(1024) __attribute__((amdgpu_waves_per_eu(8, 8))) void k_compact(CompactArgs a) {
  __shared__ unsigned long long s_red[16][5], s_tot[5], s_em[COMPACT_CHUNK];
  __shared__ uint32_t           s_ob[COMPACT_CHUNK], s_ib[COMPACT_CHUNK], s_no[COMPACT_CHUNK], s_w[2][16];
  static_assert(COMPACT_CHUNK == 1024, "an edge per thread");
  const int      lane = threadIdx.x & 63, wave = threadIdx.x >> 6;
  const uint32_t chunk = blockIdx.x;
  const uint64_t my_e  = static_cast<uint64_t>(chunk) * COMPACT_CHUNK + threadIdx.x;
  const uint32_t my_no = my_e < a.n_edges ? a.edge_norders[my_e] : 0u, my_ni = my_e < a.n_edges ? a.edge_nids[my_e] : 0u;
  const uint64_t my_em = my_e < a.n_edges ? a.edges[my_e].em_off : 0ull;
  unsigned long long t[5] = {0, 0, 0, 0, 0};
  for (uint32_t c = threadIdx.x; c < a.n_chunks; c += 1024) {
    const unsigned long long w0 = a.chunk_sums[2 * c], w1 = a.chunk_sums[2 * c + 1];
    const unsigned long long no = w0 >> 32, nf = w0 & 0xffffull;
    if (c < chunk) {
      t[0] += no;
      t[1] += w1;
    }
    t[2] += no;
    t[3] += w1;
    t[4] += nf;
  }
#pragma unroll
  for (int k = 0; k < 5; ++k) {
    for (int d = 32; d > 0; d >>= 1) t[k] += __shfl_xor(t[k], d);
    if (lane == 0) s_red[wave][k] = t[k];
  }
  __syncthreads();
  if (wave == 0) {
#pragma unroll
    for (int k = 0; k < 5; ++k) {
      unsigned long long v = lane < 16 ? s_red[lane][k] : 0ull;
      for (int d = 8; d > 0; d >>= 1) v += __shfl_xor(v, d);
      if (lane == 0) s_tot[k] = v;
    }
  }
  __syncthreads();
  const unsigned long long base_o = s_tot[0], base_i = s_tot[1], tot_o = s_tot[2], tot_i = s_tot[3], tot_f = s_tot[4];
  if (chunk == 0 && a.scalars && threadIdx.x < 64) {
    if (lane == 0) {
      a.scalars[SC_TOTAL_A] = tot_o;
      a.scalars[SC_TOTAL_B] = tot_i;
      a.scalars[SC_TOTAL_C] = tot_f;
    }
    publish_to_host(a.pub, lane, lane == SC_TOTAL_A ? tot_o : lane == SC_TOTAL_B ? tot_i : lane == SC_TOTAL_C ? tot_f : lane < SC_COUNT ? a.scalars[lane] : 0ull);
  }
  if (tot_o > a.cap_orders || tot_i > a.cap_ids) return;
  const uint64_t e0 = static_cast<uint64_t>(chunk) * COMPACT_CHUNK;
  if (e0 >= a.n_edges) return;
  {
    const uint32_t no = my_no, ni = my_ni;
    const uint64_t em = my_em;
    const uint32_t io = wave_incl_scan(no), ii = wave_incl_scan(ni);
    if (lane == 63) {
      s_w[0][wave] = io;
      s_w[1][wave] = ii;
    }
    __syncthreads();
    uint32_t bo = io - no, bi = ii - ni;
    for (int w = 0; w < wave; ++w) {
      bo += s_w[0][w];
      bi += s_w[1][w];
    }
    s_ob[threadIdx.x] = bo;
    s_ib[threadIdx.x] = bi;
    s_no[threadIdx.x] = no;
    s_em[threadIdx.x] = em;
  }
  __syncthreads();
  constexpr int ROUNDS = COMPACT_CHUNK / 256;
  const int     sub = lane & 3;
#pragma unroll 1
  for (int round = 0; round < ROUNDS; ++round) {
    const uint32_t le   = round * 256 + wave * 16 + (lane >> 2);
    const uint64_t e    = e0 + le;
    const bool     have = e < a.n_edges;
    const uint32_t no   = have ? s_no[le] : 0u;
    const uint64_t em_off = s_em[le];
    uint64_t       oo = 0, io = 0;
    if (have) {
      oo = base_o + s_ob[le];
      io = base_i + s_ib[le];
      if (sub == 0) {
        a.edges[e].order_off = oo + a.out_order_base;
        a.edges[e].order_cnt = static_cast<uint16_t>(no);
        a.edges[e].em_off    = em_off + a.out_em_base;
      }
    }
    uint32_t max_no = no;
    for (int d = 32; d >= 4; d >>= 1) max_no = max(max_no, static_cast<uint32_t>(__shfl_xor(static_cast<int>(max_no), d)));
    for (uint32_t i = 0; i < max_no; ++i) {
      const bool on = i < no;
      uint4      w  = make_uint4(0, 0, 0, 0);
      if (on) w = reinterpret_cast<const uint4 *>(&a.order_scr[em_off + i])[sub];
      const int      q2  = (lane & ~3) + 2;
      const uint32_t rel = static_cast<uint32_t>(__shfl(static_cast<int>(w.x), q2));
      const uint32_t cnt = static_cast<uint32_t>(__shfl(static_cast<int>(w.z), q2));
      if (sub == 2) {
        const uint64_t gio = io + a.out_ids_base;
        w.x = static_cast<uint32_t>(gio);
        w.y = static_cast<uint32_t>(gio >> 32);
      }
      if (sub == 0) w.x += a.out_edge_base;
      if (on) {
        reinterpret_cast<uint4 *>(&a.orders[oo + i])[sub] = w;
        for (uint32_t q = sub; q < cnt; q += 4) a.ids[io + q] = a.ids_scr[em_off + rel + q];
        io += cnt;
      }
    }
  }
}
// ... 161 lines not shown
  if (i0 < nO) {
    __syncthreads();
    const uint64_t quads = min<uint64_t>(256, nO - i0) * 4;
    uint4         *dst   = reinterpret_cast<uint4 *>(a.orders + i0);
    for (uint32_t q = threadIdx.x; q < quads; q += 256) dst[q] = s_rec[q];
  }
  if (i < nI) {
    uint32_t r = 0;
    while (i >= a.base[r + 1].ids) ++r;
    const uint64_t  k   = i - a.base[r].ids;
    const uint32_t *src = reinterpret_cast<const uint32_t *>(a.gathered + r * a.slab_bytes + a.off_ids);
    uint32_t        id;
    if (IDS3) {
      const uint32_t *w = src + 3 * (k >> 2);
      const uint32_t  j = static_cast<uint32_t>(k & 3);
      id = j == 0 ? (w[0] & 0xffffffu) : j == 1 ? ((w[0] >> 24) | ((w[1] & 0xffffu) << 8))
           : j == 2 ? ((w[1] >> 16) | ((w[2] & 0xffu) << 16)) : (w[2] >> 8);
    } else {
      id = src[k];
    }
    a.ids[i] = id + a.base[r].anchor_id;
  }
}


static inline dim3 grid1(uint64_t n, uint32_t per_block) { return dim3(static_cast<uint32_t>((n + per_block - 1) / per_block)); }

void launch_max_ids(hipStream_t st, const msgpu_row *rows, uint64_t n, uint32_t *max_ids) {
  if (n) {
    uint64_t nb = (n + 255) / 256;
    hipLaunchKernelGGL(k_max_ids, dim3(static_cast<uint32_t>(nb < 2048 ? nb : 2048)), dim3(256), 0, st, rows, n, max_ids);
  }
}
void launch_index_init(hipStream_t st, uint32_t *const zero[4], const uint32_t n_zero[4], uint32_t *const ones[2],
                       const uint32_t n_ones[2]) {
  uint32_t *const z8[8] = {zero[0], zero[1], zero[2], zero[3], nullptr, nullptr, nullptr, nullptr};
  const uint32_t  n8[8] = {n_zero[0], n_zero[1], n_zero[2], n_zero[3], 0, 0, 0, 0};
  launch_index_init8(st, z8, n8, ones, n_ones);
}
void launch_index_init8(hipStream_t st, uint32_t *const zero[8], const uint32_t n_zero[8], uint32_t *const ones[2],
                        const uint32_t n_ones[2]) {
  IndexInitArgs a;
  uint32_t      most = 1;
  for (int k = 0; k < 8; ++k) {
    a.zero[k]   = zero[k];
    a.n_zero[k] = zero[k] ? n_zero[k] : 0;
    most        = a.n_zero[k] > most ? a.n_zero[k] : most;
  }
  for (int k = 0; k < 2; ++k) {
    a.ones[k]   = ones[k];
    a.n_ones[k] = n_ones[k];
    most        = n_ones[k] > most ? n_ones[k] : most;
  }
  uint32_t nb = (most + 255) / 256;
  hipLaunchKernelGGL(k_index_init, dim3(nb < 1024 ? nb : 1024), dim3(256), 0, st, a);
}
void launch_index_pass1(hipStream_t st, const msgpu_row *rows, uint64_t n, uint32_t *cnt_read, uint32_t *anchor_first,
                        uint32_t V, uint32_t A, uint32_t *flags, uint32_t *err, IRow *bkt_row, uint32_t cap,
                        uint2 *spos) {
  if (n)
    hipLaunchKernelGGL(k_index_pass1, grid1(n, 256), dim3(256), 0, st, rows, n, cnt_read, anchor_first, flags, V, A, err,
                       bkt_row, cap, spos);
  hipLaunchKernelGGL(k_check_anchor_first, grid1(static_cast<uint64_t>(A) + 1, 256), dim3(256), 0, st, anchor_first, A,
                     static_cast<uint32_t>(n), flags);
}
void launch_scatter_read(hipStream_t st, const msgpu_row *rows, uint64_t n, const uint32_t *read_off, uint32_t *cursor,
                         IRow *bkt_row) {
  if (n)
    hipLaunchKernelGGL(k_scatter_read, grid1(n, 256), dim3(256), 0, st, rows, n, read_off, cursor, bkt_row);
}
void launch_sort_read(hipStream_t st, const uint32_t *read_off, const uint32_t *cnt_read, uint32_t V, const IRow *bkt_row,
                      IRow *by_read, uint32_t *read_cnt, uint32_t *alive_rank,
                      uint32_t *anchor_cnt, uint8_t *bkt_dead, uint32_t *flags, IRow *by_anchor, uint32_t cap,
                      const msgpu_row *rows, int32_t *read_len, uint32_t *read_first, uint32_t *err,
                      const uint2 *spos, uint4 *vis, uint32_t *visits) {
  if (V)
    hipLaunchKernelGGL(k_sort_read, grid1(V, 4), dim3(256), 0, st, read_off, cnt_read, V, bkt_row, by_read,
                       read_cnt, alive_rank, anchor_cnt, bkt_dead, flags, by_anchor, cap, rows, read_len, read_first, err,
                       spos, vis, visits);
}
void launch_index_finish(hipStream_t st, const uint32_t *read_first, uint32_t V, uint32_t *err, const uint32_t *flags,
                         const uint32_t *fast_off, const uint32_t *gen_off, uint32_t A, uint32_t *anchor_off, uint32_t *d_n_alive,
                         uint32_t n_rows) {
  const uint64_t most = V > static_cast<uint64_t>(A) + 1 ? V : static_cast<uint64_t>(A) + 1;
  hipLaunchKernelGGL(k_index_finish, grid1(most, 256), dim3(256), 0, st, read_first, V, err, flags, fast_off, gen_off, A, anchor_off,
                     d_n_alive, n_rows);
}
void launch_select_anchor_off(hipStream_t st, const uint32_t *flags, const uint32_t *fast_off, const uint32_t *gen_off,
                              uint32_t A, uint32_t *anchor_off, uint32_t *d_n_alive, uint32_t n_rows) {
  hipLaunchKernelGGL(k_select_anchor_off, grid1(static_cast<uint64_t>(A) + 1, 256), dim3(256), 0, st, flags, fast_off,
                     gen_off, A, anchor_off, d_n_alive, n_rows);
}
void launch_scatter_anchor(hipStream_t st, const msgpu_row *rows, uint64_t n, const uint32_t *alive_rank,
                           const uint32_t *anchor_off, uint32_t *cursor, uint32_t *bkt_idx, uint32_t *bkt_line,
                           const uint32_t *flags) {
  if (n)
    hipLaunchKernelGGL(k_scatter_anchor, grid1(n, 256), dim3(256), 0, st, rows, n, alive_rank, anchor_off, cursor,
                       bkt_idx, bkt_line, flags);
}
void launch_rank_anchor(hipStream_t st, const uint32_t *anchor_off, uint64_t n_rows, const uint32_t *d_n_alive,
                        const uint32_t *bkt_idx, const uint32_t *bkt_line, const msgpu_row *rows,
                        const uint32_t *alive_rank, IRow *by_anchor, const uint32_t *flags, const uint32_t *read_off,
                        IRow *by_read, uint4 *vis) {
  if (n_rows)
    hipLaunchKernelGGL(k_rank_anchor, grid1(n_rows, 256), dim3(256), 0, st, anchor_off, d_n_alive, bkt_idx, bkt_line,
                       rows, alive_rank, by_anchor, flags, read_off, by_read, vis);
}
void launch_bound(hipStream_t st, const uint32_t *read_off, const uint32_t *read_cnt, const uint4 *vis, uint32_t V,
                  uint32_t shard, uint32_t nshards, uint32_t lo, uint32_t hi, uint32_t *bound) {
  if (V)
    hipLaunchKernelGGL(k_bound, grid1(V, 16), dim3(256), 0, st, read_off, read_cnt, vis, V, shard, nshards, lo, hi,
                       bound);
}
void launch_classify_reads(hipStream_t st, const uint32_t *read_off, const uint32_t *read_cnt, const uint32_t *bound,
                           const uint64_t *cand_off, uint32_t V, uint32_t shard, uint32_t nshards, uint32_t lo,
                           uint32_t hi, CandDesc *l0, CandDesc *l1, CandDesc *l2, uint32_t *l3, uint32_t *n_lists, const CandZero &z,
                           unsigned long long *own_total) {
  if (V)
    hipLaunchKernelGGL(k_classify_reads, grid1(V, 1024), dim3(1024), 0, st, read_off, read_cnt, bound, cand_off, V, shard,
                       nshards, lo, hi, l0, l1, l2, l3, n_lists, z, own_total);
}
void launch_candidates(hipStream_t st, const CandArgs &a, int cls, const CandDesc *list, uint32_t n_list) {
  if (!n_list) return;
  if (cls == 0)
    hipLaunchKernelGGL((k_candidates<256, 512, 256>), dim3(n_list), dim3(256), 0, st, a, list, n_list);
  else if (cls == 1)
    hipLaunchKernelGGL((k_candidates<256, 1024, 256>), dim3(n_list), dim3(256), 0, st, a, list, n_list);
  else
    hipLaunchKernelGGL((k_candidates<1024, 4096, 256>), dim3(n_list), dim3(256), 0, st, a, list, n_list);
}
void launch_candidates_big(hipStream_t st, const CandArgs &a, const uint32_t *list, uint32_t n_list, uint64_t *big_key,
                           uint32_t *big_t, uint32_t *big_r2s, uint32_t *big_pfx) {
  if (!n_list) return;
  hipLaunchKernelGGL(k_candidates_big, dim3(n_list), dim3(256), 0, st, a, list, n_list, big_key, big_t, big_r2s,
                     big_pfx);
}
void launch_fill_pair_tab(hipStream_t st, uint32_t *tab) {
  hipLaunchKernelGGL(k_fill_pair_tab, dim3((4 * PAIR_TAB_STRIDE + 255) / 256), dim3(256), 0, st, tab);
}
void launch_chain(hipStream_t st, const ChainArgs &a, const uint32_t *list, uint32_t n_list) {
  const uint64_t n = list ? n_list : a.n_edges;
  if (n) hipLaunchKernelGGL(k_chain, dim3(static_cast<uint32_t>(n)), dim3(64), CHAIN_LDS_BYTES, st, a, list, n_list);
}
void launch_chain_sub(hipStream_t st, const ChainArgs &a, int width, const uint32_t *list, uint32_t n_list) {
  if (!n_list) return;
  if (width == 8)
    hipLaunchKernelGGL(k_chain_sub<8>, grid1(n_list, 32), dim3(256), 0, st, a, list, n_list);
  else if (width == 16)
    hipLaunchKernelGGL(k_chain_sub<16>, grid1(n_list, 16), dim3(256), 0, st, a, list, n_list);
  else
    hipLaunchKernelGGL(k_chain_sub<32>, grid1(n_list, 8), dim3(256), 0, st, a, list, n_list);
}
void launch_chain_sub_all(hipStream_t st, const ChainArgs &a, const uint32_t *l32, uint32_t n32, const uint32_t *l16, uint32_t n16,
                          const uint32_t *l8, uint32_t n8) {
  ChainSubLists l;
  l.list32 = l32, l.list16 = l16, l.list8 = l8;
  l.n32 = n32, l.n16 = n16, l.n8 = n8;
  l.nb32 = n32 ? grid1(n32, 8).x : 0u, l.nb16 = n16 ? grid1(n16, 16).x : 0u;
  const uint32_t nb8 = n8 ? grid1(n8, 32).x : 0u, nb = l.nb32 + l.nb16 + nb8;
  if (nb) hipLaunchKernelGGL(k_chain_sub_all, dim3(nb), dim3(256), 0, st, a, l);
}
size_t big_elem_bytes() { return sizeof(BigElem); }
size_t big_path_bytes() { return sizeof(BigPath); }
void launch_chain_big(hipStream_t st, const ChainArgs &a, const uint32_t *big_list, const uint64_t *big_off,
                      uint32_t n_big, void *elems, void *paths) {
  if (n_big)
    hipLaunchKernelGGL(k_chain_big, dim3(n_big), dim3(64), 0, st, a, big_list, big_off, n_big,
                       static_cast<BigElem *>(elems), static_cast<BigPath *>(paths));
}
void launch_merge_gathered(hipStream_t st, const MergeArgs &a) {
  uint64_t n = a.base[a.world].edges;
  if (a.base[a.world].orders > n) n = a.base[a.world].orders;
  if (a.base[a.world].ids > n) n = a.base[a.world].ids;
  if (n) hipLaunchKernelGGL(k_merge_gathered, grid1(n, 256), dim3(256), 0, st, a);
}
void launch_merge_wire(hipStream_t st, const MergeArgs &a, bool ids3) {
  uint64_t n = a.base[a.world].edges;
  if (a.base[a.world].orders > n) n = a.base[a.world].orders;
  if (a.base[a.world].ids > n) n = a.base[a.world].ids;
  if (!n) return;
  if (ids3)
    hipLaunchKernelGGL(k_merge_wire<true>, grid1(n, 256), dim3(256), 0, st, a);
  else
    hipLaunchKernelGGL(k_merge_wire<false>, grid1(n, 256), dim3(256), 0, st, a);
}
void launch_pack_wire(hipStream_t st, const PackWireArgs &a) {
  uint64_t n = a.n_edges > a.n_orders ? a.n_edges : a.n_orders;
  if (a.ids && (a.n_ids + 3) / 4 > n) n = (a.n_ids + 3) / 4;
  if (!n) n = 1;
  hipLaunchKernelGGL(k_pack_wire, grid1(n, 256), dim3(256), 0, st, a);
}
void launch_compact(hipStream_t st, const CompactArgs &a) {
  hipLaunchKernelGGL(k_compact, dim3(a.n_chunks ? a.n_chunks : 1), dim3(1024), 0, st, a);
}

}
```

Before: 436.9 million overlap-pairs/s.

## Repack chain-sub LDS into split arrays and raise occupancy to eight waves

```diff
diff --git a/muchsalsa_amd/csrc/msgpu_api.hip b/muchsalsa_amd/csrc/msgpu_api.hip
--- a/muchsalsa_amd/csrc/msgpu_api.hip
+++ b/muchsalsa_amd/csrc/msgpu_api.hip
@@ -250,10 +250,11 @@
   bool   use_fork  = true;
   bool   use_prologue = true;
   bool   chain_serial = false;
+  bool   sub_waves7   = false;
   uint32_t n_cls[4] = {0, 0, 0, 0};
   uint64_t n_edges_fast = 0;
   uint64_t chain_E = 0;
-  DevBuf ems, order_scr, ids_scr, edge_norders, edge_nids, orders, ids, big_list, cls_list, big_elems,
+  DevBuf ems, order_scr, ids_scr, edge_norders, edge_nids, orders, ids, big_list, cls_list, cls_rec, big_elems,
       big_paths;
   DevBuf g_deg, g_off, g_adj, g_cand, g_sane, g_out;
   DevBuf sel_idx, sel_cnt, sel_off, sel_ems;
@@ -388,7 +389,7 @@
                    &c->bound, &c->cand_off, &c->cand_j, &c->cand_t, &c->scr_v2, &c->scr_start, &c->n_cand, &c->n_edge,
                    &c->lists, &c->edges, &c->edge_cand,
                    &c->big_key, &c->big_t, &c->big_r2s, &c->big_pfx, &c->pair_tab, &c->chain_chunks, &c->big_off, &c->cand_sums, &c->bucket_visits, &c->ems, &c->order_scr, &c->ids_scr,
-                   &c->edge_norders, &c->edge_nids, &c->orders, &c->ids, &c->big_list, &c->cls_list, &c->big_elems, &c->big_paths, &c->alt_edges, &c->alt_ems, &c->alt_orders, &c->alt_ids, &c->vis16, &c->visits,
+                   &c->edge_norders, &c->edge_nids, &c->orders, &c->ids, &c->big_list, &c->cls_list, &c->cls_rec, &c->big_elems, &c->big_paths, &c->alt_edges, &c->alt_ems, &c->alt_orders, &c->alt_ids, &c->vis16, &c->visits,
                    &c->spos2, &c->bin_cursor, &c->bin_start, &c->wire_dev[0], &c->wire_dev[1], &c->win_cuts};
   for (DevBuf *b : all) b->release();
 }
@@ -764,6 +765,10 @@
     c->use_prologue = !getenv("MSGPU_NO_PROLOGUE");
     c->use_fork     = !getenv("MSGPU_NO_FORK");
     c->chain_serial = getenv("MSGPU_CHAIN_SERIAL") != nullptr;
+    {
+      const char *w = getenv("MSGPU_SUB_WAVES");
+      c->sub_waves7 = w && strcmp(w, "7") == 0;
+    }
   }
   for (auto &ev : c->ev)
     if (hipEventCreate(&ev) != hipSuccess) {
@@ -1073,6 +1078,7 @@
     uint64_t ce = c->edges.room() / sizeof(msgpu_edge);
     if (c->edge_cand.cap / 8 < ce) ce = c->edge_cand.cap / 8;
     if (c->cls_list.cap / 4 < ce) ce = c->cls_list.cap / 4;
+    if (c->cls_rec.cap / sizeof(SubRec) < ce) ce = c->cls_rec.cap / sizeof(SubRec);
     uint64_t cb = c->big_list.cap / 4;
     if (c->big_off.cap / 8 < cb) cb = c->big_off.cap / 8;
     if (c->chain_chunks.cap / 8 < chunk_words(ce)) ce = 0;
@@ -1093,6 +1099,7 @@
     k.edges          = c->edges.as<msgpu_edge>();
     k.edge_cand      = c->edge_cand.as<uint64_t>();
     k.list           = c->cls_list.as<uint32_t>();
+    k.list_rec       = c->cls_rec.as<SubRec>();
     k.big_list       = c->big_list.as<uint32_t>();
     k.big_off        = c->big_off.as<uint64_t>();
     k.big_cursor     = scalar<unsigned long long>(c, SC_BIGCUR);
@@ -1124,6 +1131,7 @@
     ENSURE(c, edges, (c->n_edges ? c->n_edges : 1) * sizeof(msgpu_edge));
     ENSURE(c, edge_cand, (c->n_edges ? c->n_edges : 1) * 8);
     ENSURE(c, cls_list, (c->n_edges + 1) * 4);
+    ENSURE(c, cls_rec, (c->n_edges + 1) * sizeof(SubRec));
     ENSURE(c, big_list, (c->n_big_edges + 1) * 4);
     ENSURE(c, big_off, (c->n_big_edges + 1) * 8);
     ENSURE(c, chain_chunks, chunk_words(c->edges.room() / sizeof(msgpu_edge)) * 8);
@@ -1183,6 +1191,8 @@
   a.pair_tab     = c->pair_tab.as<uint32_t>();
   a.pair_tab64   = c->pair_tab.as<uint32_t>() + 4 * PAIR_TAB_STRIDE;
   a.pair_tab_sub = c->pair_tab.as<uint32_t>() + 4 * PAIR_TAB_STRIDE + 2 * PAIR_TAB_STRIDE;
+  a.list_base    = c->cls_list.as<uint32_t>();
+  a.list_rec     = c->cls_rec.as<SubRec>();
   if (!c->chain_zeroed)
     HIPCHK(c, hipMemsetAsync(c->chain_chunks.p, 0, chunk_words(E) * 8, st));
   c->chain_zeroed = false;
@@ -1229,7 +1239,7 @@
       launch_chain_sub(st, a, 16, l16, c->n_cls[0]);
       launch_chain_sub(st, a, 8, l8, c->n_cls[3]);
     } else if (any_sub) {
-      launch_chain_sub_all(beside ? c->side_stream2 : st, a, l32, c->n_cls[1], l16, c->n_cls[0], l8, c->n_cls[3]);
+      launch_chain_sub_all(beside ? c->side_stream2 : st, a, l32, c->n_cls[1], l16, c->n_cls[0], l8, c->n_cls[3], c->sub_waves7);
     }
     if (beside) {
       HIPCHK(c, hipEventRecord(c->ev_side2, c->side_stream2));
diff --git a/muchsalsa_amd/csrc/msgpu_internal.h b/muchsalsa_amd/csrc/msgpu_internal.h
--- a/muchsalsa_amd/csrc/msgpu_internal.h
+++ b/muchsalsa_amd/csrc/msgpu_internal.h
@@ -53,6 +53,10 @@
   uint32_t *scalar_words;
   uint32_t  n_scalar_words;
 };
+struct __attribute__((aligned(16))) SubRec {
+  uint32_t e, v1, v2, em_cnt;
+  uint64_t em_off, cand;
+};
 struct EmitArgs {
   const uint32_t *n_edge, *n_cand;
   const uint64_t *cand_off;
@@ -64,6 +68,7 @@
   msgpu_edge     *edges;
   uint64_t       *edge_cand;
   uint32_t       *list;
+  SubRec         *list_rec;
   uint32_t       *big_list;
   uint64_t       *big_off;
   unsigned long long *big_cursor;
@@ -91,6 +96,8 @@
   uint32_t        *err;
   const uint32_t  *pair_tab;
   const uint32_t  *pair_tab64;
+  const uint32_t  *list_base;
+  const SubRec    *list_rec;
   const uint32_t  *pair_tab_sub;
   unsigned long long *chunk_sums;
   int              fast_path;
@@ -265,7 +272,7 @@
   uint32_t        n32, n16, n8, nb32, nb16;
 };
 void launch_chain_sub_all(hipStream_t st, const ChainArgs &a, const uint32_t *l32, uint32_t n32, const uint32_t *l16, uint32_t n16,
-                          const uint32_t *l8, uint32_t n8);
+                          const uint32_t *l8, uint32_t n8, bool seven_waves);
 size_t big_elem_bytes();
 size_t big_path_bytes();
 void launch_chain_big(hipStream_t st, const ChainArgs &a, const uint32_t *big_list, const uint64_t *big_off,
diff --git a/muchsalsa_amd/csrc/msgpu_kernels.hip b/muchsalsa_amd/csrc/msgpu_kernels.hip
--- a/muchsalsa_amd/csrc/msgpu_kernels.hip
+++ b/muchsalsa_amd/csrc/msgpu_kernels.hip
@@ -1309,7 +1309,16 @@
         a.big_list[i] = static_cast<uint32_t>(eb + e);
         a.big_off[i]  = atomicAdd(&a.big_cursor[1], static_cast<unsigned long long>(ed.em_cnt));
       } else if (ed.em_cnt) {
-        a.list[atomicAdd(&s_pos[ed.em_cnt - 1], 1u)] = static_cast<uint32_t>(eb + e);
+        const uint32_t pos = atomicAdd(&s_pos[ed.em_cnt - 1], 1u);
+        a.list[pos]        = static_cast<uint32_t>(eb + e);
+#ifdef MSGPU_LIST_REC
+        if (ed.em_cnt <= 32) {
+          uint4 *q = reinterpret_cast<uint4 *>(&a.list_rec[pos]);
+          q[0]     = make_uint4(static_cast<uint32_t>(eb + e), ed.v1, ed.v2, ed.em_cnt);
+          q[1]     = make_uint4(static_cast<uint32_t>(ed.em_off), static_cast<uint32_t>(ed.em_off >> 32),
+                                static_cast<uint32_t>(co + st), static_cast<uint32_t>((co + st) >> 32));
+        }
+#endif
       }
     }
   }
@@ -1987,31 +1996,57 @@
   return np;
 }
 
+constexpr uint32_t SUB_LDS_HI   = 0;
+constexpr uint32_t SUB_LDS_RAW  = 1024;
+constexpr uint32_t SUB_LDS_LO   = 2048;
+constexpr uint32_t SUB_LDS_CM   = 3072;
+constexpr uint32_t SUB_LDS_OVR  = 3328;
+constexpr uint32_t SUB_LDS_JQ   = 4352;
+constexpr uint32_t SUB_LDS_GRP  = 4864;
+constexpr uint32_t SUB_LDS_WAVE = 5120;
+static_assert(SUB_LDS_RAW + 1024 >= sizeof(SubPath) * 2 * 64 && SUB_LDS_LO >= sizeof(SubPath) * 2 * 64, "the path lists overlay two arrays");
+static_assert(4 * SUB_LDS_WAVE * 8 <= 160 * 1024, "eight workgroups in a CU");
+
 template <int W>
 __device__ __forceinline__ void chain_sub_body(const ChainArgs &a, const uint32_t *list, uint32_t n_list, uint32_t block,
-                                               unsigned char (*s_wavebuf)[sizeof(ChainElem) * 64], uint32_t (*s_cm)[64],
-                                               double (*s_keep)[64][4], uint32_t (*s_anchor)[64]) {
+                                               unsigned char (*s_sub)[SUB_LDS_WAVE]) {
   constexpr int G = 64 / W;
   static_assert(W == 8 || W == 16 || W == 32, "group width");
-  static_assert(sizeof(ChainElem) * 64 >= sizeof(SubPath) * 2 * 64, "the path lists overlay the element table");
   const int      wave = threadIdx.x >> 6, lane = threadIdx.x & 63;
   const int      g = lane / W, sl = lane % W, gbase = g * W;
   const uint32_t slot    = (block * 4 + wave) * G + g;
   const bool     valid_g = slot < n_list;
   if (__ballot(valid_g) == 0) return;
-  const uint32_t   e  = valid_g ? list[slot] : list[0];
+#ifdef MSGPU_LIST_REC
+  const SubRec     rc = (a.list_rec + (list - a.list_base))[valid_g ? slot : 0u];
+  uint32_t         e  = rc.e;
+  const uint32_t   n  = (valid_g && rc.em_cnt <= static_cast<uint32_t>(W)) ? rc.em_cnt : 0u;
+  const uint64_t   cp = rc.cand;
+  const bool       act = sl < static_cast<int>(n);
+  uint32_t         v1 = rc.v1, v2 = rc.v2;
+  uint64_t         em_off = rc.em_off;
+#else
+  uint32_t         e  = valid_g ? list[slot] : list[0];
   const msgpu_edge ed = a.edges[e];
   const uint32_t   n  = (valid_g && ed.em_cnt <= static_cast<uint32_t>(W)) ? ed.em_cnt : 0u;
   const uint64_t   cp = a.edge_cand[e];
   const bool       act = sl < static_cast<int>(n);
-  const uint32_t   v1 = ed.v1, v2 = ed.v2;
-  const uint32_t   n1 = a.read_cnt[v1], n2 = a.read_cnt[v2];
+  uint32_t         v1 = ed.v1, v2 = ed.v2;
+  uint64_t         em_off = ed.em_off;
+#endif
+  uint32_t         n1 = a.read_cnt[v1], n2 = a.read_cnt[v2];
   const int        len1 = a.read_len[v1], len2 = a.read_len[v2];
-  ChainElem       *el = reinterpret_cast<ChainElem *>(s_wavebuf[wave]);
-  uint32_t        *cm = s_cm[wave];
-
-  uint32_t  j1 = 0, q2 = 0, anchor = 0;
-  double    clo1 = 0, clo2 = 0, ovr1 = 0, ovr2 = 0, em_score = 0;
+  unsigned char   *wb     = s_sub[wave];
+  double2         *el_hi  = reinterpret_cast<double2 *>(wb + SUB_LDS_HI);
+  int4            *el_raw = reinterpret_cast<int4 *>(wb + SUB_LDS_RAW);
+  double2         *el_lo  = reinterpret_cast<double2 *>(wb + SUB_LDS_LO);
+  double2         *s_ovr  = reinterpret_cast<double2 *>(wb + SUB_LDS_OVR);
+  uint2           *s_jq   = reinterpret_cast<uint2 *>(wb + SUB_LDS_JQ);
+  uint4           *s_grp  = reinterpret_cast<uint4 *>(wb + SUB_LDS_GRP) + 2 * g;
+  uint32_t        *cm     = reinterpret_cast<uint32_t *>(wb + SUB_LDS_CM);
+
+  uint32_t  j1 = 0, q2 = 0;
+  double    ovr1 = 0, ovr2 = 0, em_score = 0;
   bool      em_dir = false, em_prim = false;
   ChainElem x{};
   cm[lane] = 0;
@@ -2020,7 +2055,7 @@
     const uint32_t t = a.cand_t[cp + sl];
     const IRow m1 = load_irow(&a.by_read[a.read_off[v1] + j1]);
     const IRow m2 = load_irow(&a.by_anchor[t]);
-    anchor        = m1.other;
+    const uint32_t anchor = m1.other;
     q2            = m2.pf & PF_POS_MASK;
     const int  ov_lo = max(m1.i_lo, m2.i_lo), ov_hi = min(m1.i_hi, m2.i_hi);
     const bool d1 = (m1.pf & PF_DIR) != 0, d2 = (m2.pf & PF_DIR) != 0;
@@ -2035,7 +2070,7 @@
     const double is_ = static_cast<double>(im.score) * cl / il;
     em_score         = os + is_;
     {
-      uint4 *q = reinterpret_cast<uint4 *>(&a.ems[ed.em_off + sl]);
+      uint4 *q = reinterpret_cast<uint4 *>(&a.ems[em_off + sl]);
       q[0]     = make_uint4(static_cast<uint32_t>(ov_lo), static_cast<uint32_t>(ov_hi),
                             static_cast<uint32_t>(__double_as_longlong(em_score)),
                             static_cast<uint32_t>(__double_as_longlong(em_score) >> 32));
@@ -2070,14 +2105,15 @@
       x.chi2 = static_cast<double>(m2.n_hi) - ncr2;
       ovr2   = static_cast<double>(len2 - m2.n_hi) + ncr2;
     }
-    clo1     = x.clo1;
-    clo2     = x.clo2;
-    el[lane] = x;
-  }
-  {
-    double *kp = s_keep[wave][lane];
-    kp[0] = clo1, kp[1] = clo2, kp[2] = ovr1, kp[3] = ovr2;
-    s_anchor[wave][lane] = anchor;
+    el_hi[lane]  = make_double2(x.chi1, x.chi2);
+    el_raw[lane] = make_int4(x.rlo1, x.rhi1, x.rlo2, x.rhi2);
+  }
+  el_lo[lane] = make_double2(x.clo1, x.clo2);
+  s_ovr[lane] = make_double2(ovr1, ovr2);
+  s_jq[lane]  = make_uint2(j1, q2);
+  if (sl == 0) {
+    s_grp[0] = make_uint4(e, v1, v2, n1);
+    s_grp[1] = make_uint4(n2, static_cast<uint32_t>(em_off), static_cast<uint32_t>(em_off >> 32), 0u);
   }
   const uint32_t m_plus  = group_bits<W>(__ballot(act && em_dir), gbase);
   const uint32_t m_minus = group_bits<W>(__ballot(act && !em_dir), gbase);
@@ -2088,7 +2124,14 @@
   {
     const bool      try_clean = (m_plus == 0 || m_minus == 0) && n >= 2 && (a.fast_path & CHAIN_FAST_SHORTCUT);
     const bool      plus      = m_minus == 0;
-    const ChainElem Pv        = el[sl > 0 ? lane - 1 : lane];
+    ChainElem       Pv;
+    {
+      const int     pl = sl > 0 ? lane - 1 : lane;
+      const double2 h = el_hi[pl], c = el_lo[pl];
+      const int4    r = el_raw[pl];
+      Pv.clo1 = c.x, Pv.chi1 = h.x, Pv.clo2 = c.y, Pv.chi2 = h.y;
+      Pv.rlo1 = r.x, Pv.rhi1 = r.y, Pv.rlo2 = r.z, Pv.rhi2 = r.w;
+    }
     bool            good      = true;
     if (act && sl > 0) {
       good = (Pv.clo1 < x.clo1) & (Pv.chi1 < x.chi1) & (Pv.rlo1 < x.rlo1) & (Pv.rhi1 < x.rhi1);
@@ -2120,7 +2163,6 @@
   const int Pmax = nP * (nP - 1) / 2;
   const bool               one_dir = __ballot(m_plus != 0 && m_minus != 0) == 0;
   const unsigned long long KD_one  = __ballot(m_minus == 0);
-  static_assert(sizeof(ChainElem) == 48, "the pair table holds byte offsets of 48-byte elements");
   const __amdgpu_buffer_rsrc_t tab_rsrc = __builtin_amdgcn_make_buffer_rsrc(
       const_cast<uint32_t *>(a.pair_tab_sub) + (W == 32 ? 0 : W == 16 ? 1 : 2) * PAIR_TAB_STRIDE * 2, 0, PAIR_TAB_STRIDE * 8, 0x00020000);
   const uint32_t tab_lane = static_cast<uint32_t>(sl) * 8u;
@@ -2130,13 +2172,13 @@
     return make_uint2(static_cast<uint32_t>(v.x), static_cast<uint32_t>(v.y));
   };
   const int            Pl  = P - sl;
-  const unsigned char *elg = reinterpret_cast<const unsigned char *>(el + gbase);
+  const unsigned char *elg = wb + gbase * 16;
   unsigned char       *cmg = reinterpret_cast<unsigned char *>(cm + gbase);
   double          wiggle  = a.wiggle;
   asm volatile("" : "+v"(wiggle));
   bool wf_lane = true;
   if (act) {
-    const int prev_rlo1 = el[sl > 0 ? lane - 1 : lane].rlo1;
+    const int prev_rlo1 = el_raw[sl > 0 ? lane - 1 : lane].x;
     wf_lane = (x.clo1 <= x.chi1) & (x.clo2 <= x.chi2) & (x.rlo1 <= x.rhi1) & (sl == 0 || prev_rlo1 <= x.rlo1);
   }
   const bool wf = __ballot(!wf_lane) == 0;
@@ -2155,11 +2197,13 @@
         valid &= __ballot(kd == ld);
         KD    = __ballot(kd);
       }
-      const ChainElem K = *reinterpret_cast<const ChainElem *>(elg + (kl.x & 0xffffu));
-      const ChainElem L = *reinterpret_cast<const ChainElem *>(elg + (kl.x >> 16));
-      double          d1, d2;
-      const NanoMasks f1 = nano_check<WFT::value, WFT::value>(K.clo1, K.chi1, L.clo1, L.chi1, K.rlo1, K.rhi1, L.rlo1, L.rhi1, d1);
-      const NanoMasks f2 = nano_check<WFT::value, false>(K.clo2, K.chi2, L.clo2, L.chi2, K.rlo2, K.rhi2, L.rlo2, L.rhi2, d2);
+      const unsigned char *kp = elg + (kl.x & 0xffffu), *lp = elg + (kl.x >> 16);
+      const double2 Kh = *reinterpret_cast<const double2 *>(kp + SUB_LDS_HI), Kc = *reinterpret_cast<const double2 *>(kp + SUB_LDS_LO);
+      const double2 Lh = *reinterpret_cast<const double2 *>(lp + SUB_LDS_HI), Lc = *reinterpret_cast<const double2 *>(lp + SUB_LDS_LO);
+      const int4    Kr = *reinterpret_cast<const int4 *>(kp + SUB_LDS_RAW), Lr = *reinterpret_cast<const int4 *>(lp + SUB_LDS_RAW);
+      double        d1, d2;
+      const NanoMasks f1 = nano_check<WFT::value, WFT::value>(Kc.x, Kh.x, Lc.x, Lh.x, Kr.x, Kr.y, Lr.x, Lr.y, d1);
+      const NanoMasks f2 = nano_check<WFT::value, false>(Kc.y, Kh.y, Lc.y, Lh.y, Kr.z, Kr.w, Lr.z, Lr.w, d2);
       M p2, n2m;
       if (DIR == 0) {
         p2  = f2.pos;
@@ -2257,7 +2301,12 @@
     }
   }
 
-  SubPath *pmn = reinterpret_cast<SubPath *>(s_wavebuf[wave]) + gbase, *ppl = pmn + 64;
+  SubPath *pmn = reinterpret_cast<SubPath *>(wb + SUB_LDS_HI) + gbase, *ppl = pmn + 64;
+  {
+    const uint2 jq = s_jq[lane];
+    j1 = jq.x, q2 = jq.y;
+    n1 = s_grp[0].w, n2 = s_grp[1].x;
+  }
   uint32_t n_m = 0, n_p = 0;
 #pragma clang loop unroll(disable)
   for (int trip = 0; trip < 2; ++trip) {
@@ -2298,6 +2347,17 @@
   if (combined == 1) shadow = !(keep_m ? pmn[__builtin_ctz(keep_m)].primary : ppl[__builtin_ctz(keep_p)].primary);
 
   uint32_t n_orders = 0, n_ids = 0;
+  {
+    const uint4 g0 = s_grp[0], g1 = s_grp[1];
+    e = g0.x, v1 = g0.y, v2 = g0.z;
+    em_off = (static_cast<uint64_t>(g1.z) << 32) | g1.y;
+  }
+  uint32_t anchor = 0;
+  {
+    const msgpu_edgematch *emr = a.ems;
+    asm volatile("" : "+s"(emr));
+    if (act) anchor = emr[em_off + sl].anchor_id;
+  }
   {
     uint32_t km = keep_m, kp = keep_p;
     while (__ballot((km | kp) != 0)) {
@@ -2310,9 +2370,9 @@
       const SubPath  rec  = (dir ? ppl : pmn)[pi];
       const uint32_t mask = (has && rec.mask) ? rec.mask : 1u;
       const int      f = __builtin_ctz(mask), l = 31 - __builtin_clz(mask);
-      const double  *kf = s_keep[wave][gbase + f], *kl = s_keep[wave][gbase + l];
-      const double   L1 = kf[0], R1 = kl[2];
-      const double   L2 = dir ? kf[1] : kf[3], R2 = dir ? kl[3] : kl[1];
+      const double2  cf = el_lo[gbase + f], cl = el_lo[gbase + l], of = s_ovr[gbase + f], ol = s_ovr[gbase + l];
+      const double   L1 = cf.x, R1 = ol.x;
+      const double   L2 = dir ? cf.y : of.y, R2 = dir ? ol.y : cl.y;
       bool     have = false;
       uint32_t fl   = 0;
       double   lo = 0, ro = 0;
@@ -2340,7 +2400,7 @@
       const bool emit = has && have;
       if (emit) {
         const uint32_t cnt = static_cast<uint32_t>(__popc(mask));
-        if ((mask >> sl) & 1u) a.ids_scr[ed.em_off + n_ids + static_cast<uint32_t>(__popc(mask & ((1u << sl) - 1u)))] = s_anchor[wave][lane];
+        if ((mask >> sl) & 1u) a.ids_scr[em_off + n_ids + static_cast<uint32_t>(__popc(mask & ((1u << sl) - 1u)))] = anchor;
         if (sl == 0) {
           msgpu_order o;
           o.edge_idx     = e;
@@ -2355,7 +2415,7 @@
           o.base         = v1;
           o.pad[0]       = 0;
           o.pad[1]       = 0;
-          a.order_scr[ed.em_off + n_orders] = o;
+          a.order_scr[em_off + n_orders] = o;
         }
         ++n_orders;
         n_ids += cnt;
@@ -2372,28 +2432,29 @@
 
 template <int W>
 __global__ __launch_bounds__(256) __attribute__((amdgpu_waves_per_eu(W == 32 ? 7 : 6, W == 32 ? 7 : 6))) void k_chain_sub(ChainArgs a, const uint32_t *list, uint32_t n_list) {
-  __shared__ __attribute__((aligned(16))) unsigned char s_wavebuf[4][sizeof(ChainElem) * 64];
-  __shared__ uint32_t                                  s_cm[4][64];
-  __shared__ __attribute__((aligned(16))) double       s_keep[4][64][4];
-  __shared__ uint32_t                                  s_anchor[4][64];
-  chain_sub_body<W>(a, list, n_list, blockIdx.x, s_wavebuf, s_cm, s_keep, s_anchor);
+  __shared__ __attribute__((aligned(16))) unsigned char s_sub[4][SUB_LDS_WAVE];
+  chain_sub_body<W>(a, list, n_list, blockIdx.x, s_sub);
 }
 #ifndef MSGPU_SUB_WAVES
-#define MSGPU_SUB_WAVES 7
+#define MSGPU_SUB_WAVES 8
 #endif
-__global__ __launch_bounds__(256) __attribute__((amdgpu_waves_per_eu(MSGPU_SUB_WAVES, MSGPU_SUB_WAVES))) void k_chain_sub_all(ChainArgs a, ChainSubLists l) {
-  __shared__ __attribute__((aligned(16))) unsigned char s_wavebuf[4][sizeof(ChainElem) * 64];
-  __shared__ uint32_t                                  s_cm[4][64];
-  __shared__ __attribute__((aligned(16))) double       s_keep[4][64][4];
-  __shared__ uint32_t                                  s_anchor[4][64];
+__device__ __forceinline__ void chain_sub_all_body(const ChainArgs &a, const ChainSubLists &l, unsigned char (*s_sub)[SUB_LDS_WAVE]) {
   uint32_t b = blockIdx.x;
   if (b < l.nb32) {
-    chain_sub_body<32>(a, l.list32, l.n32, b, s_wavebuf, s_cm, s_keep, s_anchor);
+    chain_sub_body<32>(a, l.list32, l.n32, b, s_sub);
   } else if ((b -= l.nb32) < l.nb16) {
-    chain_sub_body<16>(a, l.list16, l.n16, b, s_wavebuf, s_cm, s_keep, s_anchor);
+    chain_sub_body<16>(a, l.list16, l.n16, b, s_sub);
   } else {
-    chain_sub_body<8>(a, l.list8, l.n8, b - l.nb16, s_wavebuf, s_cm, s_keep, s_anchor);
-  }
+    chain_sub_body<8>(a, l.list8, l.n8, b - l.nb16, s_sub);
+  }
+}
+__global__ __launch_bounds__(256) __attribute__((amdgpu_waves_per_eu(MSGPU_SUB_WAVES, MSGPU_SUB_WAVES))) void k_chain_sub_all(ChainArgs a, ChainSubLists l) {
+  __shared__ __attribute__((aligned(16))) unsigned char s_sub[4][SUB_LDS_WAVE];
+  chain_sub_all_body(a, l, s_sub);
+}
+__global__ __launch_bounds__(256) __attribute__((amdgpu_waves_per_eu(7, 7))) void k_chain_sub_all7(ChainArgs a, ChainSubLists l) {
+  __shared__ __attribute__((aligned(16))) unsigned char s_sub[4][SUB_LDS_WAVE];
+  chain_sub_all_body(a, l, s_sub);
 }
 template __global__ void k_chain_sub<8>(ChainArgs, const uint32_t *, uint32_t);
 template __global__ void k_chain_sub<16>(ChainArgs, const uint32_t *, uint32_t);
@@ -2847,7 +2908,7 @@
 }
 __device__ __forceinline__ void tabsub_entry(uint32_t *tab, int t, int p, int k, int l, int run) {
   uint32_t *e = tab + 4 * PAIR_TAB_STRIDE + 2 * PAIR_TAB_STRIDE + (static_cast<size_t>(t - 1) * PAIR_TAB_STRIDE + p) * 2;
-  e[0]        = static_cast<uint32_t>(k * 48) | (static_cast<uint32_t>(l * 48) << 16);
+  e[0]        = static_cast<uint32_t>(k * 16) | (static_cast<uint32_t>(l * 16) << 16);
   e[1]        = static_cast<uint32_t>(k) | (static_cast<uint32_t>(run) << 8) | (static_cast<uint32_t>(l * 4) << 16);
 }
 __device__ __forceinline__ void band64_entry(uint32_t *tab, int p) {
@@ -3315,13 +3376,14 @@
     hipLaunchKernelGGL(k_chain_sub<32>, grid1(n_list, 8), dim3(256), 0, st, a, list, n_list);
 }
 void launch_chain_sub_all(hipStream_t st, const ChainArgs &a, const uint32_t *l32, uint32_t n32, const uint32_t *l16, uint32_t n16,
-                          const uint32_t *l8, uint32_t n8) {
+                          const uint32_t *l8, uint32_t n8, bool seven_waves) {
   ChainSubLists l;
   l.list32 = l32, l.list16 = l16, l.list8 = l8;
   l.n32 = n32, l.n16 = n16, l.n8 = n8;
   l.nb32 = n32 ? grid1(n32, 8).x : 0u, l.nb16 = n16 ? grid1(n16, 16).x : 0u;
   const uint32_t nb8 = n8 ? grid1(n8, 32).x : 0u, nb = l.nb32 + l.nb16 + nb8;
-  if (nb) hipLaunchKernelGGL(k_chain_sub_all, dim3(nb), dim3(256), 0, st, a, l);
+  if (nb && seven_waves) hipLaunchKernelGGL(k_chain_sub_all7, dim3(nb), dim3(256), 0, st, a, l);
+  else if (nb) hipLaunchKernelGGL(k_chain_sub_all, dim3(nb), dim3(256), 0, st, a, l);
 }
 size_t big_elem_bytes() { return sizeof(BigElem); }
 size_t big_path_bytes() { return sizeof(BigPath); }
```

Result: no change. 434.3 million overlap-pairs/s (-0.6%).
